# Xiuyu-Li/q-diffusion

Measured on NVIDIA H100. Metric: images_per_sec, higher is better.
Workload: dtype int8 (W4/W8 codes x A8 codes, int32 accumulate; fp32 norms/softmax)

## Files before the change

q-diffusion_b200/csrc/engine.cu:

```cuda
#include <cuda.h>
#include <cuda_runtime.h>
#include <cudaTypedefs.h>

#include <atomic>
#include <cstdarg>
#include <cstdio>
#include <cstdlib>
#include <cstring>
#include <mutex>
#include <new>
#include <utility>
#include <vector>

#include "../../include/qdiff_b200.h"
#include "attention.cuh"
#include "attention_wg.cuh"
#include "elem.cuh"
#include "gemm_i8.cuh"

namespace {

thread_local char g_err[512] = "";
std::atomic<long long> g_launches{0};
constexpr int kMaxDevices = 64;
std::atomic<int> g_num_sms[kMaxDevices];

int fail(int code, const char* fmt, ...) {
  va_list ap;
  va_start(ap, fmt);
  vsnprintf(g_err, sizeof(g_err), fmt, ap);
  va_end(ap);
  return code;
}

int check_launch(const char* what) {
  cudaError_t e = cudaGetLastError();
  if (e != cudaSuccess) return fail(QD_ERR_CUDA, "%s: %s", what, cudaGetErrorString(e));
  g_launches.fetch_add(1, std::memory_order_relaxed);
  return QD_OK;
}

template <typename... KArgs, typename... Args>
void launch_k(void (*kern)(KArgs...), dim3 grid, dim3 block, size_t smem, cudaStream_t s, Args&&... args) {
  cudaLaunchConfig_t cfg = {};
  cfg.gridDim = grid;
  cfg.blockDim = block;
  cfg.dynamicSmemBytes = smem;
  cfg.stream = s;
  cudaLaunchKernelEx(&cfg, kern, KArgs(std::forward<Args>(args))...);
}

int current_device() {
  int dev = -1;
  if (cudaGetDevice(&dev) != cudaSuccess) return -1;
  return dev;
}

int num_sms() {
  const int dev = current_device();
  if (dev < 0 || dev >= kMaxDevices) {
    fail(QD_ERR_CUDA, "no CUDA device: qdiff_b200 has no CPU fallback");
    return 0;
  }
  int n = g_num_sms[dev].load(std::memory_order_relaxed);
  if (n == 0) {
    if (cudaDeviceGetAttribute(&n, cudaDevAttrMultiProcessorCount, dev) != cudaSuccess || n <= 0) {
      fail(QD_ERR_CUDA, "no CUDA device: qdiff_b200 has no CPU fallback");
      return 0;
    }
    g_num_sms[dev].store(n, std::memory_order_relaxed);
  }
  return n;
}

template <typename K>
int ensure_smem_optin(K kern, int bytes, std::atomic<unsigned long long>& done, const char* what) {
  const int dev = current_device();
  if (dev < 0 || dev >= kMaxDevices) return fail(QD_ERR_CUDA, "%s: no current CUDA device", what);
  const unsigned long long bit = 1ull << dev;
  if (done.load(std::memory_order_acquire) & bit) return QD_OK;
  cudaError_t e = cudaFuncSetAttribute(kern, cudaFuncAttributeMaxDynamicSharedMemorySize, bytes);
  if (e != cudaSuccess) return fail(QD_ERR_CUDA, "%s: cudaFuncSetAttribute: %s", what, cudaGetErrorString(e));
  done.fetch_or(bit, std::memory_order_release);
  return QD_OK;
}

struct DeviceGuard {
  int prev = -1;
  bool ok = true;
  explicit DeviceGuard(int device) {
    if (cudaGetDevice(&prev) != cudaSuccess) prev = -1;
    if (prev != device) ok = cudaSetDevice(device) == cudaSuccess;
  }
  ~DeviceGuard() { if (prev >= 0) cudaSetDevice(prev); }
};

int grid_for(long long work_items, int threads, int per_sm = 8) {
  const int sms = num_sms();
  long long blocks = (work_items + threads - 1) / threads;
  long long cap = (long long)sms * per_sm;
  if (blocks > cap) blocks = cap;
  if (blocks < 1) blocks = 1;
  return (int)blocks;
}

PFN_cuTensorMapEncodeTiled_v12000 get_encode() {
  static PFN_cuTensorMapEncodeTiled_v12000 fn = nullptr;
  static std::once_flag once;
  std::call_once(once, [] {
    void* p = nullptr;
    cudaDriverEntryPointQueryResult q;
    if (cudaGetDriverEntryPoint("cuTensorMapEncodeTiled", &p, cudaEnableDefault, &q) == cudaSuccess &&
        q == cudaDriverEntryPointSuccess)
      fn = reinterpret_cast<PFN_cuTensorMapEncodeTiled_v12000>(p);
  });
  return fn;
}

int encode_u8_map(CUtensorMap* m, const void* base, int rank, const cuuint64_t* dims, const cuuint64_t* strides_bytes,
                  const cuuint32_t* box, int swizzle_bytes = 128) {
  auto enc = get_encode();
  if (!enc) return fail(QD_ERR_CUDA, "cuTensorMapEncodeTiled entry point not available");
  cuuint32_t estr[5] = {1, 1, 1, 1, 1};
  CUresult r = enc(m, CU_TENSOR_MAP_DATA_TYPE_UINT8, (cuuint32_t)rank, const_cast<void*>(base), dims, strides_bytes,
                   box, estr, CU_TENSOR_MAP_INTERLEAVE_NONE,
                   swizzle_bytes == 0 ? CU_TENSOR_MAP_SWIZZLE_NONE :
                   swizzle_bytes == 32 ? CU_TENSOR_MAP_SWIZZLE_32B : swizzle_bytes == 64 ? CU_TENSOR_MAP_SWIZZLE_64B : CU_TENSOR_MAP_SWIZZLE_128B,
                   CU_TENSOR_MAP_L2_PROMOTION_L2_128B, CU_TENSOR_MAP_FLOAT_OOB_FILL_NONE);
  if (r != CUDA_SUCCESS) return fail(QD_ERR_CUDA, "cuTensorMapEncodeTiled failed (%d)", (int)r);
  return QD_OK;
}

struct GemmPlan {
  CUtensorMap tmA, tmB, tmR;
  qd::GemmArgs args;
  int grid, mode;
};

int pick_bn(int N, int tiles_m, int sms, int hint, int step, long long K) {
  if (hint > 0) return hint;
  static const int wave_model = [] { const char* e = getenv("QDIFF_BN_MODEL"); return (e && !strcmp(e, "wave")) ? 1 : 0; }();
  int best = step;
  double best_cost = -1.0;
  const int n16 = (N + step - 1) / step * step;
  const double kb = (double)((K + 127) / 128);
  for (int bn = step; bn <= qd::GEMM_MAX_BN; bn += step) {
    if (bn > n16) break;
    const long long tiles = (long long)tiles_m * ((N + bn - 1) / bn);
    const long long waves = (tiles + sms - 1) / sms;
    double cost;
    if (wave_model) {
      cost = (double)waves * (bn + 24);
    } else {
      const double main_loop = kb * (2.1 * bn > 3.0 * (128 + bn) ? 2.1 * bn : 3.0 * (128 + bn));
      const double epilogue = 6.0 * bn + 300.0;
      cost = (double)waves * ((main_loop > epilogue ? main_loop : epilogue) + 200.0);
    }
    if (best_cost < 0 || cost < best_cost - 1e-9 || (cost < best_cost + 1e-9 && bn > best)) {
      best_cost = cost;
      best = bn;
    }
  }
  return best;
}

int gemm_mode(const qd::GemmArgs& a);

constexpr size_t kSplitWsBytes = 64u << 20;
int32_t* splitk_workspace() {
  static void* ws[kMaxDevices] = {};
  static std::mutex mu;
  const int dev = current_device();
  if (dev < 0 || dev >= kMaxDevices) return nullptr;
  std::lock_guard<std::mutex> lk(mu);
  if (!ws[dev] && cudaMalloc(&ws[dev], kSplitWsBytes) != cudaSuccess) { ws[dev] = nullptr; cudaGetLastError(); }
  return reinterpret_cast<int32_t*>(ws[dev]);
}

int plan_gemm(const qd_gemm_desc* d, GemmPlan* pl) {
  if (!d || !d->a || !d->w || !d->scale) return fail(QD_ERR_BAD_ARG, "gemm: null operand");
  if (d->taps != 1 && d->taps != 9) return fail(QD_ERR_UNSUPPORTED, "gemm: taps must be 1 or 9 (got %d)", d->taps);
  if (d->C <= 0 || (d->C % 32) != 0) return fail(QD_ERR_UNSUPPORTED, "gemm: C=%d must be a positive multiple of 32", d->C);
  if (d->a_bf16 && (d->corr || d->out_q || d->geglu || d->w_int4_packed || !d->out))
    return fail(QD_ERR_BAD_ARG, "gemm: a_bf16 (weight-only) layers take no corr / out_q / geglu / packed weights and write fp32");
  if (d->M <= 0 || d->N <= 0) return fail(QD_ERR_BAD_ARG, "gemm: bad M/N");
  if (!d->out && !d->out_q) return fail(QD_ERR_BAD_ARG, "gemm: no output");
  const int sms = num_sms();
  if (!sms) return QD_ERR_CUDA;

  qd::GemmArgs& a = pl->args;
  memset(&a, 0, sizeof(a));
  a.M = d->M; a.N = d->N; a.C = d->C; a.taps = d->taps;
  a.kdup = d->k_dup == 2 ? 2 : 1;
  if (d->k_dup != 0 && d->k_dup != 1 && d->k_dup != 2) return fail(QD_ERR_BAD_ARG, "gemm: k_dup must be 0, 1 or 2");
  if (a.kdup == 2 && d->w_int4_packed) return fail(QD_ERR_BAD_ARG, "gemm: k_dup 2 is for 8-bit weights (not packed INT4)");
  a.tiles_m = (d->M + qd::GEMM_BM - 1) / qd::GEMM_BM;
  a.geglu = d->geglu;
  if (d->geglu) {
    if ((d->N & 7) || !d->out_q || d->out || d->rowvec || d->residual || d->out_q_transposed || (d->ldq & 3) || d->taps != 1)
      return fail(QD_ERR_BAD_ARG, "gemm: geglu needs N %% 8 == 0, out_q only, plain GEMM");
  }
  a.BN = pick_bn(d->N, a.tiles_m, sms, d->bn_hint, d->geglu ? 32 : 16, (long long)d->C * d->taps * a.kdup);
  const int bn_default = a.BN;
  static const int splitk_enabled = [] { const char* e = getenv("QDIFF_SPLITK"); return (e && !strcmp(e, "0")) ? 0 : 1; }();
  const int num_kb_all = ((d->C + qd::GEMM_BK - 1) / qd::GEMM_BK) * d->taps * a.kdup;
  const bool splitk_candidate = splitk_enabled && !d->bn_hint && !d->a_bf16 && !d->w_int4_packed && d->out && !d->out_q && !d->geglu &&
                                !(d->N & 3) && !(d->ldo & 3) && (!d->residual || !(d->ldr & 3)) && (!d->rowvec || !(d->ld_rowvec & 3)) &&
                                num_kb_all >= 16;
  if (splitk_candidate) {
    const int bn_wide = d->N >= qd::GEMM_MAX_BN_SPLITK ? qd::GEMM_MAX_BN_SPLITK : (d->N + 15) / 16 * 16;
    if (2 * a.tiles_m * ((d->N + bn_wide - 1) / bn_wide) <= sms) a.BN = bn_wide;
  }
  if (a.BN % 16 || a.BN < 16 || a.BN > qd::GEMM_MAX_BN_SPLITK || (d->bn_hint && a.BN > qd::GEMM_MAX_BN))
    return fail(QD_ERR_BAD_ARG, "gemm: bad BN %d (16 .. %d)", a.BN, qd::GEMM_MAX_BN);
  a.tiles_n = (d->N + a.BN - 1) / a.BN;
  a.a_signed = d->a_signed; a.b_signed = 1;


  cuuint64_t dims[4], strides[3];
  cuuint32_t box[4];
  if (d->taps == 1) {
    if (d->lda % 16) return fail(QD_ERR_UNSUPPORTED, "gemm: lda=%lld must be a multiple of 16", d->lda);
    if (d->lda < d->C) return fail(QD_ERR_BAD_ARG, "gemm: lda < C");
    dims[0] = (cuuint64_t)d->C; dims[1] = (cuuint64_t)d->M; dims[2] = 1; dims[3] = 1;
    strides[0] = (cuuint64_t)d->lda; strides[1] = (cuuint64_t)d->lda * d->M; strides[2] = strides[1];
    box[0] = qd::GEMM_BK; box[1] = qd::GEMM_BM; box[2] = 1; box[3] = 1;
  } else {
    const int H = d->H, W = d->W, B = d->B;
    if (H <= 0 || W <= 0 || B <= 0 || (long long)B * H * W != d->M) return fail(QD_ERR_BAD_ARG, "gemm: conv geometry");
    const int hw = H * W;
    int bh, bn;
    int bw = W;
    if (W > 128) {
      if (W % 128) return fail(QD_ERR_UNSUPPORTED, "gemm: conv W=%d must divide or be a multiple of 128", W);
      bw = 128; bh = 1; bn = 1;
    } else if (hw >= 128) {
      if (128 % W) return fail(QD_ERR_UNSUPPORTED, "gemm: conv W=%d must divide 128", W);
      bh = 128 / W; bn = 1;
      if (H % bh) return fail(QD_ERR_UNSUPPORTED, "gemm: conv H=%d not a multiple of %d", H, bh);
    } else {
      if (128 % hw) return fail(QD_ERR_UNSUPPORTED, "gemm: conv H*W=%d must divide 128", hw);
      bh = H; bn = 128 / hw;
    }
    a.H = H; a.W = W; a.bh = bh; a.bn = bn;
    const cuuint64_t pitch = d->lda > d->C ? (cuuint64_t)d->lda : (cuuint64_t)d->C;
    if (pitch % 16) return fail(QD_ERR_UNSUPPORTED, "gemm: conv pixel pitch %llu must be a multiple of 16", (unsigned long long)pitch);
    dims[0] = (cuuint64_t)d->C; dims[1] = (cuuint64_t)W; dims[2] = (cuuint64_t)H; dims[3] = (cuuint64_t)B;
    strides[0] = pitch; strides[1] = pitch * W; strides[2] = pitch * W * H;
    box[0] = qd::GEMM_BK; box[1] = (cuuint32_t)bw; box[2] = (cuuint32_t)bh; box[3] = (cuuint32_t)bn;
  }
  int rc = encode_u8_map(&pl->tmA, d->a, 4, dims, strides, box);
  if (rc) return rc;
  if (d->w_int4_packed) {
    if (!d->w_zero) return fail(QD_ERR_BAD_ARG, "gemm: packed INT4 weights need w_zero");
    if (((uintptr_t)d->w) & 15) return fail(QD_ERR_BAD_ARG, "gemm: packed weights must be 16-byte aligned");
    a.w4 = 1;
    a.wzero = d->w_zero;
  }
  a.out = d->out; a.ldo = d->ldo;
  a.out_q = reinterpret_cast<int8_t*>(d->out_q); a.ldq = d->ldq;
  a.out_q_transposed = d->out_q_transposed;
  a.rows_per_batch = d->rows_per_batch;
  if ((d->rowvec || d->out_q_transposed) && d->rows_per_batch <= 0) return fail(QD_ERR_BAD_ARG, "gemm: rows_per_batch required");
  a.oq_d = d->out_q_head_dim; a.oq_pitch = d->out_q_head_pitch;
  a.oq_f16 = d->out_q_f16 ? 1 : 0;
  if (a.oq_f16 && (!d->out_q || d->out_q_transposed || d->geglu || (d->ldq & 3) || (((uintptr_t)d->out_q) & 7)))
    return fail(QD_ERR_BAD_ARG, "gemm: out_q_f16 needs a row-major out_q with ldq %% 4 == 0");
  if (a.oq_d > 0 && ((a.oq_d & 3) || (a.oq_pitch & 3) || a.oq_pitch < a.oq_d || d->out_q_transposed || !d->out_q))
    return fail(QD_ERR_BAD_ARG, "gemm: bad out_q head layout");
  if (d->out_q && d->oq.qmax - d->oq.qmin > 255)
    return fail(QD_ERR_UNSUPPORTED, "gemm: the epilogue emits 8-bit codes; quantizer range [%d, %d] is wider", d->oq.qmin, d->oq.qmax);
  a.q_delta = d->oq.delta; a.q_zp = d->oq.zero_point; a.q_lo = d->oq.qmin; a.q_hi = d->oq.qmax;
  a.scale = d->scale; a.bias = d->bias; a.corr = d->corr;
  a.scale_q = d->scale_q; a.bias_q = d->bias_q;
  a.gn_stats = reinterpret_cast<float2*>(d->gn_stats); a.ld_stats = d->ld_stats;
  a.bf16 = d->a_bf16;
  if (d->gn_stats && (!d->out || (d->ld_stats & 1) || (reinterpret_cast<uintptr_t>(d->gn_stats) & 15)))
    return fail(QD_ERR_BAD_ARG, "gemm: gn_stats needs an fp32 output, an even ld_stats and 16-byte alignment");
  if ((d->scale_q == nullptr) != (d->bias_q == nullptr)) return fail(QD_ERR_BAD_ARG, "gemm: scale_q and bias_q come together");
  a.rowvec = d->rowvec; a.ld_rowvec = d->ld_rowvec;
  a.residual = d->residual; a.ldr = d->ldr;
  const int tiles = a.tiles_m * a.tiles_n;
  pl->grid = tiles < sms ? tiles : sms;
  pl->mode = gemm_mode(a);
  {
    const int num_kb = num_kb_all;
    const bool eligible = splitk_candidate && pl->mode >= 0 && 2 * tiles <= sms &&
                          (!a.gn_stats || (!(a.M & 31) && !(a.ld_stats & 1)));
    if (eligible) {
      int splits = sms / tiles;
      if (splits > 16) splits = 16;
      if (splits > num_kb / 4) splits = num_kb / 4;
      if (splits >= 2 && (size_t)splits * a.M * a.N * 4 <= kSplitWsBytes) {
        const int per = (num_kb + splits - 1) / splits;
        splits = (num_kb + per - 1) / per;
        int32_t* ws = splitk_workspace();
        if (ws && splits >= 2) {
          a.splits = splits; a.kb_per_split = per; a.ws = ws;
          pl->grid = tiles * splits < sms ? tiles * splits : sms;
        }
      }
    }
  }
  if (a.splits <= 1 && a.BN > qd::GEMM_MAX_BN) {
    a.BN = bn_default;
    a.tiles_n = (d->N + a.BN - 1) / a.BN;
    const int t = a.tiles_m * a.tiles_n;
    pl->grid = t < sms ? t : sms;
  }
  {
    const int w_rows = d->w_rows > 0 ? d->w_rows : d->N;
    if (d->w_int4_packed) {
      cuuint64_t bd[2] = {(cuuint64_t)d->taps * d->C / 2, (cuuint64_t)w_rows};
      cuuint64_t bs[1] = {(cuuint64_t)d->taps * d->C / 2};
      cuuint32_t bb[2] = {qd::GEMM_BK / 2, (cuuint32_t)a.BN};
      rc = encode_u8_map(&pl->tmB, d->w, 2, bd, bs, bb, 0);
    } else {
      cuuint64_t bd[2] = {(cuuint64_t)d->taps * d->C * a.kdup, (cuuint64_t)w_rows};
      cuuint64_t bs[1] = {(cuuint64_t)d->taps * d->C * a.kdup};
      cuuint32_t bb[2] = {qd::GEMM_BK, (cuuint32_t)a.BN};
      rc = encode_u8_map(&pl->tmB, d->w, 2, bd, bs, bb);
    }
    if (rc) return rc;
  }
  if (a.bf16 && pl->mode < 0)
    return fail(QD_ERR_UNSUPPORTED, "gemm: weight-only (a_bf16) layer needs a specialised epilogue (N %% 4 == 0, aligned leading dimensions)");
  memset(&pl->tmR, 0, sizeof(pl->tmR));
  if (qd::gemm_res_tma(pl->mode)) {
    cuuint64_t rd[2] = {(cuuint64_t)d->N * 4, (cuuint64_t)d->M};
    cuuint64_t rs[1] = {(cuuint64_t)d->ldr * 4};
    cuuint32_t rb[2] = {128, 32};
    rc = encode_u8_map(&pl->tmR, d->residual, 2, rd, rs, rb);
    if (rc) return rc;
  }
  return QD_OK;
}

template <int MODE, bool W4>
int launch_gemm_mode_w(const GemmPlan& pl, cudaStream_t s) {
  static std::atomic<unsigned long long> optin{0};
  if (int rc = ensure_smem_optin(qd::gemm_i8_kernel<MODE, W4>, 227 * 1024, optin, "gemm")) return rc;
  qd::GemmArgs a = pl.args;
  const int stage_bytes = qd::gemm_stage_footprint(a.BN, W4 ? 1 : 0);
  constexpr int res_bytes = qd::gemm_res_bytes(MODE);
  constexpr bool splitk = MODE >= 0 && (MODE & qd::EPI_SPLITK) != 0;
  if (a.BN > qd::gemm_max_bn(MODE)) return fail(QD_ERR_BAD_ARG, "gemm: BN=%d exceeds %d (mode %d)", a.BN, qd::gemm_max_bn(MODE), MODE);
  int stages = (232448 - 512 - qd::gemm_acc_tile_bytes(a.BN, splitk) - res_bytes - 1024 - 1024) / stage_bytes;
  if (stages > qd::GEMM_MAX_STAGES) stages = qd::GEMM_MAX_STAGES;
  if (stages < 2) stages = 2;
  a.stages = stages;
  const int smem = qd::gemm_smem_layout(a.BN, stages, W4 ? 1 : 0, res_bytes, splitk).total;
  if (smem > 232448) return fail(QD_ERR_UNSUPPORTED, "gemm: BN=%d needs %d bytes of shared memory for 2 stages (mode %d, w4 %d)", a.BN, smem, MODE, (int)W4);
  launch_k(qd::gemm_i8_kernel<MODE, W4>, pl.grid, qd::gemm_threads(MODE, W4), smem, s, pl.tmA, pl.tmB, pl.tmR, a);
  return check_launch("gemm_i8_kernel");
}

template <int MODE>
int launch_gemm_mode(const GemmPlan& pl, cudaStream_t s) {
  return pl.args.w4 ? launch_gemm_mode_w<MODE, true>(pl, s) : launch_gemm_mode_w<MODE, false>(pl, s);
}

int gemm_mode(const qd::GemmArgs& a) {
  const bool f = a.out != nullptr, q = a.out_q != nullptr;
  if (a.geglu) return qd::EPI_GEGLU | qd::EPI_OUT_Q | (a.corr ? qd::EPI_CORR : 0);
  if (q && !f && !a.geglu && !a.scale_q) return -1;
  if (a.out_q_transposed && q && !f && !a.rowvec && !a.residual && a.taps == 1 && a.oq_d == 0 &&
      a.rows_per_batch % 32 == 0 && (a.ldq & 15) == 0 && (reinterpret_cast<uintptr_t>(a.out_q) & 15) == 0)
    return qd::EPI_TRANS | qd::EPI_OUT_Q | (a.corr ? qd::EPI_CORR : 0);
  if (f == q || a.out_q_transposed || (a.N & 3)) return -1;
  if (a.rowvec && a.residual) return -1;
  if (q && a.rowvec) return -1;
  if (f && (a.ldo & 3)) return -1;
  if (q && (a.ldq & 3)) return -1;
  if (a.residual && (a.ldr & 3)) return -1;
  if (a.rowvec && (a.ld_rowvec & 3)) return -1;
  if (a.bf16) {
    return qd::EPI_BF16 | qd::EPI_OUT_F32 | ((a.taps == 9) ? qd::EPI_CONV : 0) | (a.rowvec ? qd::EPI_ROWVEC : 0) |
           (a.residual ? qd::EPI_RESIDUAL : 0);
  }
  static const int ring_kb = [] { const char* e = getenv("QDIFF_RES_RING_KB"); return e ? atoi(e) : 5; }();
  const int num_kb = ((a.C + qd::GEMM_BK - 1) / qd::GEMM_BK) * a.taps * a.kdup;
  const bool ring = a.residual && a.taps == 1 && num_kb <= ring_kb && !(reinterpret_cast<uintptr_t>(a.residual) & 15) &&
                    !a.w4;
  return (a.corr ? qd::EPI_CORR : 0) | ((a.taps == 9) ? qd::EPI_CONV : 0) | (a.rowvec ? qd::EPI_ROWVEC : 0) |
         (a.residual ? qd::EPI_RESIDUAL : 0) | (f ? qd::EPI_OUT_F32 : qd::EPI_OUT_Q) | (ring ? qd::EPI_RESTMA : 0);
}

int launch_gemm(const GemmPlan& pl, cudaStream_t s) {
  using namespace qd;
  if (pl.args.splits > 1) {
    if (int rc = launch_gemm_mode_w<EPI_SPLITK, false>(pl, s)) return rc;
    launch_k(qd::splitk_finish_kernel, dim3((pl.args.N + 31) / 32, (pl.args.M + 31) / 32), 256, 0, s, pl.args);
    return check_launch("splitk_finish_kernel");
  }
  switch (pl.mode) {
    case EPI_OUT_F32: return launch_gemm_mode<EPI_OUT_F32>(pl, s);
    case EPI_OUT_F32 | EPI_CORR: return launch_gemm_mode<EPI_OUT_F32 | EPI_CORR>(pl, s);
    case EPI_OUT_F32 | EPI_ROWVEC: return launch_gemm_mode<EPI_OUT_F32 | EPI_ROWVEC>(pl, s);
    case EPI_OUT_F32 | EPI_ROWVEC | EPI_CORR: return launch_gemm_mode<EPI_OUT_F32 | EPI_ROWVEC | EPI_CORR>(pl, s);
    case EPI_OUT_F32 | EPI_RESIDUAL: return launch_gemm_mode<EPI_OUT_F32 | EPI_RESIDUAL>(pl, s);
    case EPI_OUT_F32 | EPI_RESIDUAL | EPI_CORR: return launch_gemm_mode<EPI_OUT_F32 | EPI_RESIDUAL | EPI_CORR>(pl, s);
    case EPI_OUT_F32 | EPI_CORR | EPI_CONV: return launch_gemm_mode<EPI_OUT_F32 | EPI_CORR | EPI_CONV>(pl, s);
    case EPI_OUT_F32 | EPI_ROWVEC | EPI_CORR | EPI_CONV: return launch_gemm_mode<EPI_OUT_F32 | EPI_ROWVEC | EPI_CORR | EPI_CONV>(pl, s);
    case EPI_OUT_F32 | EPI_RESIDUAL | EPI_CORR | EPI_CONV: return launch_gemm_mode<EPI_OUT_F32 | EPI_RESIDUAL | EPI_CORR | EPI_CONV>(pl, s);
    case EPI_OUT_Q | EPI_CORR | EPI_CONV: return launch_gemm_mode<EPI_OUT_Q | EPI_CORR | EPI_CONV>(pl, s);
    case EPI_OUT_F32 | EPI_CONV: return launch_gemm_mode<EPI_OUT_F32 | EPI_CONV>(pl, s);
    case EPI_OUT_F32 | EPI_ROWVEC | EPI_CONV: return launch_gemm_mode<EPI_OUT_F32 | EPI_ROWVEC | EPI_CONV>(pl, s);
    case EPI_OUT_F32 | EPI_RESIDUAL | EPI_CONV: return launch_gemm_mode<EPI_OUT_F32 | EPI_RESIDUAL | EPI_CONV>(pl, s);
    case EPI_OUT_Q | EPI_CONV: return launch_gemm_mode<EPI_OUT_Q | EPI_CONV>(pl, s);
    case EPI_OUT_Q: return launch_gemm_mode<EPI_OUT_Q>(pl, s);
    case EPI_OUT_Q | EPI_CORR: return launch_gemm_mode<EPI_OUT_Q | EPI_CORR>(pl, s);
    case EPI_OUT_Q | EPI_RESIDUAL: return launch_gemm_mode<EPI_OUT_Q | EPI_RESIDUAL>(pl, s);
    case EPI_OUT_Q | EPI_RESIDUAL | EPI_CORR: return launch_gemm_mode<EPI_OUT_Q | EPI_RESIDUAL | EPI_CORR>(pl, s);
    case EPI_OUT_F32 | EPI_RESIDUAL | EPI_RESTMA: return launch_gemm_mode<EPI_OUT_F32 | EPI_RESIDUAL | EPI_RESTMA>(pl, s);
    case EPI_OUT_F32 | EPI_RESIDUAL | EPI_CORR | EPI_RESTMA: return launch_gemm_mode<EPI_OUT_F32 | EPI_RESIDUAL | EPI_CORR | EPI_RESTMA>(pl, s);
    case EPI_OUT_Q | EPI_RESIDUAL | EPI_RESTMA: return launch_gemm_mode<EPI_OUT_Q | EPI_RESIDUAL | EPI_RESTMA>(pl, s);
    case EPI_OUT_Q | EPI_RESIDUAL | EPI_CORR | EPI_RESTMA: return launch_gemm_mode<EPI_OUT_Q | EPI_RESIDUAL | EPI_CORR | EPI_RESTMA>(pl, s);
    case EPI_BF16 | EPI_OUT_F32: return launch_gemm_mode_w<EPI_BF16 | EPI_OUT_F32, false>(pl, s);
    case EPI_BF16 | EPI_OUT_F32 | EPI_ROWVEC: return launch_gemm_mode_w<EPI_BF16 | EPI_OUT_F32 | EPI_ROWVEC, false>(pl, s);
    case EPI_BF16 | EPI_OUT_F32 | EPI_RESIDUAL: return launch_gemm_mode_w<EPI_BF16 | EPI_OUT_F32 | EPI_RESIDUAL, false>(pl, s);
    case EPI_BF16 | EPI_OUT_F32 | EPI_CONV: return launch_gemm_mode_w<EPI_BF16 | EPI_OUT_F32 | EPI_CONV, false>(pl, s);
    case EPI_BF16 | EPI_OUT_F32 | EPI_ROWVEC | EPI_CONV: return launch_gemm_mode_w<EPI_BF16 | EPI_OUT_F32 | EPI_ROWVEC | EPI_CONV, false>(pl, s);
    case EPI_BF16 | EPI_OUT_F32 | EPI_RESIDUAL | EPI_CONV: return launch_gemm_mode_w<EPI_BF16 | EPI_OUT_F32 | EPI_RESIDUAL | EPI_CONV, false>(pl, s);
    case EPI_TRANS | EPI_OUT_Q: return launch_gemm_mode<EPI_TRANS | EPI_OUT_Q>(pl, s);
    case EPI_TRANS | EPI_OUT_Q | EPI_CORR: return launch_gemm_mode<EPI_TRANS | EPI_OUT_Q | EPI_CORR>(pl, s);
    case EPI_GEGLU | EPI_OUT_Q: return launch_gemm_mode<EPI_GEGLU | EPI_OUT_Q>(pl, s);
    case EPI_GEGLU | EPI_OUT_Q | EPI_CORR: return launch_gemm_mode<EPI_GEGLU | EPI_OUT_Q | EPI_CORR>(pl, s);
    default: return launch_gemm_mode<-1>(pl, s);
  }
}

int launch_quantize(const qd_quantize_desc& d, cudaStream_t s) {
  if (!d.src || !d.dst || d.M <= 0 || d.C <= 0) return fail(QD_ERR_BAD_ARG, "quantize: bad args");
  if (d.q0.qmax - d.q0.qmin > 255 || d.q1.qmax - d.q1.qmin > 255)
    return fail(QD_ERR_UNSUPPORTED, "quantize: the engine emits 8-bit codes; quantizer range [%d, %d] is wider", d.q0.qmin, d.q0.qmax);
  const bool vec = (d.C % 4 == 0) && (d.ld_src % 4 == 0) && (d.ld_dst % 4 == 0) && (d.split % 4 == 0);
  if (d.upsample2x && !vec) return fail(QD_ERR_UNSUPPORTED, "quantize: upsample needs C %% 4 == 0");
  if (vec) {
    const long long rows = d.upsample2x ? (long long)d.B * 4 * d.H * d.W : d.M;
    launch_k(qd::quantize_kernel, grid_for(rows * (d.C / 4), 256), 256, 0, s, d);
  } else {
    launch_k(qd::quantize_scalar_kernel, grid_for((long long)d.M * d.C, 256), 256, 0, s, d);
  }
  return check_launch("quantize_kernel");
}

int gn_slab_rows(int B, int HW) {
  int sms = num_sms();
  if (sms <= 0) sms = 132;
  long long r = ((long long)B * HW) / (4LL * sms);
  int slab = 64;
  while (slab > 8 && slab > r) slab >>= 1;
  return slab;
}

long long gn_workspace_floats(int B, int HW, int C, int groups) {
  const int slab = gn_slab_rows(B, HW);
  const long long nslab = (HW + slab - 1) / slab;
  (void)C;
  return (long long)B * nslab * groups * 2 * 2 + (long long)B * groups * 2 + 16;
}

int use_stats_env() {
  static const int v = [] { const char* e = getenv("QDIFF_GN_STATS"); return (e && !strcmp(e, "0")) ? 0 : 1; }();
  return v;
}

int launch_groupnorm(const qd_groupnorm_desc& d, cudaStream_t s) {
  if (!d.x || !d.gamma || !d.beta) return fail(QD_ERR_BAD_ARG, "groupnorm: null arg");
  if (d.groups <= 0 || d.groups > qd::GN_MAX_GROUPS || d.C % 4 || d.C % d.groups || d.ld_x % 4)
    return fail(QD_ERR_UNSUPPORTED, "groupnorm: C=%d groups=%d", d.C, d.groups);
  if (d.n_out < 0 || d.n_out > 3) return fail(QD_ERR_BAD_ARG, "groupnorm: n_out");
  if (d.raw_q && ((d.raw_split & 3) || (d.ld_raw & 3) || d.raw_split < 0))
    return fail(QD_ERR_BAD_ARG, "groupnorm: raw output needs raw_split %% 4 == 0 and ld_raw %% 4 == 0");
  const int cpg = d.C / d.groups;
  {
    bool ok = (cpg % 2 == 0) && cpg <= 128 && (d.ld_x % 2 == 0) && (!d.out_f || d.ld_f % 2 == 0);
    for (int o = 0; o < d.n_out; ++o) ok = ok && (d.ld_q[o] % 2 == 0);
    const long long units = (long long)d.HW * (cpg / 2);
    static const int force = [] {
      const char* e = getenv("QDIFF_GN");
      return !e ? 0 : (!strcmp(e, "fused") ? 1 : (!strcmp(e, "split") ? 2 : 0));
    }();
    const long long limit = force == 1 ? 512LL * qd::GN_NU : (force == 2 ? 0 : 256LL * qd::GN_NU);
    const long long elems = (long long)d.B * d.HW * d.C;
    const bool small_problem = elems <= ((d.stats_in && use_stats_env()) ? (512LL << 10) : (2LL << 20)) && (long long)d.B * d.groups <= 2048;
    if (ok && units <= limit && (force == 1 || small_problem)) {
      int threads = units <= 256LL * qd::GN_NU ? 256 : 512;
      if (units < 256) threads = (int)((units + 31) / 32 * 32);
      if (threads < cpg / 2) threads = (cpg / 2 + 31) / 32 * 32;
      launch_k(qd::gn_fused_small_kernel, dim3(d.groups, d.B), threads, 0, s, d);
      return check_launch("gn_fused_small_kernel");
    }
  }
  if (!d.ws) return fail(QD_ERR_BAD_ARG, "groupnorm: workspace required");
  if ((uintptr_t)d.ws & 7) return fail(QD_ERR_BAD_ARG, "groupnorm: workspace must be 8-byte aligned");
  const int slab = gn_slab_rows(d.B, d.HW);
  const int nslab = (d.HW + slab - 1) / slab;
  double* part = reinterpret_cast<double*>(d.ws);
  float* stats = d.ws + (long long)d.B * nslab * d.groups * 4;
  int threads = d.C / 4;
  threads = (threads + 31) / 32 * 32;
  if (threads > 256) threads = 256;
  if (threads < 2 * d.groups) threads = (2 * d.groups + 31) / 32 * 32;
  int rc;
  const int use_stats = use_stats_env();
  if (d.stats_in && use_stats) {
    if (d.HW % 32) return fail(QD_ERR_BAD_ARG, "groupnorm: stats_in needs HW %% 32 == 0");
    launch_k(qd::gn_finalize_from_stats_kernel, dim3(d.groups, d.B), 128, 0, s, reinterpret_cast<const float2*>(d.stats_in),
                                                                         d.ld_stats_in, d.HW, d.C, d.groups, d.eps, stats);
    rc = check_launch("gn_finalize_from_stats_kernel");
    if (rc) return rc;
  } else {
    launch_k(qd::gn_partial_kernel, dim3(nslab, d.B), threads, 2 * d.C * sizeof(float), s, d.x, d.ld_x, d.HW, d.C, d.groups, slab,
                                                                                     nslab, part);
    rc = check_launch("gn_partial_kernel");
    if (rc) return rc;
    launch_k(qd::gn_finalize_kernel, d.B, 256, 0, s, part, d.HW, d.C, d.groups, nslab, d.eps, stats);
    rc = check_launch("gn_finalize_kernel");
    if (rc) return rc;
  }
  const int cq = d.C / 4;
  const int slabs_x = (cq + 255) / 256;
  const int TX = (cq + slabs_x - 1) / slabs_x;
  int TY = 256 / TX;
  if (TY < 1) TY = 1;
  const int athreads = TX * TY;
  int rows = qd::GN_BATCH * TY;
  while ((long long)((d.HW + rows - 1) / rows) * slabs_x * d.B > 8LL * num_sms() && rows < 8 * qd::GN_BATCH * TY) rows += qd::GN_BATCH * TY;
  const dim3 grid(slabs_x, (d.HW + rows - 1) / rows, d.B);
  const bool raw = d.raw_q != nullptr;
#define QD_GN_APPLY(NOUT, RAW) launch_k(qd::gn_apply_kernel<NOUT, RAW>, grid, athreads, 0, s, d, stats, rows, TX)
  switch (d.n_out * 2 + (raw ? 1 : 0)) {
    case 0: QD_GN_APPLY(0, false); break;
    case 1: QD_GN_APPLY(0, true); break;
    case 2: QD_GN_APPLY(1, false); break;
    case 3: QD_GN_APPLY(1, true); break;
    case 4: QD_GN_APPLY(2, false); break;
    case 5: QD_GN_APPLY(2, true); break;
    case 6: QD_GN_APPLY(3, false); break;
    default: QD_GN_APPLY(3, true); break;
  }
#undef QD_GN_APPLY
  return check_launch("gn_apply_kernel");
}

template <int NVEC>
int launch_layernorm_t(const qd_layernorm_desc& d, cudaStream_t s) {
  const int wpb = 8;
  launch_k(qd::layernorm_quant_kernel<NVEC>, grid_for((long long)d.M * 32, wpb * 32, 8), wpb * 32, 0, s, d);
  return check_launch("layernorm_quant_kernel");
}

int launch_layernorm(const qd_layernorm_desc& d, cudaStream_t s) {
  if (!d.x || !d.gamma || !d.beta) return fail(QD_ERR_BAD_ARG, "layernorm: null arg");
  if (d.C % 4 || d.ld_x % 4) return fail(QD_ERR_UNSUPPORTED, "layernorm: C=%d", d.C);
  if (d.n_out < 0 || d.n_out > 3 || (d.n_out == 0 && !d.out_f)) return fail(QD_ERR_BAD_ARG, "layernorm: n_out");
  if (d.out_f && (d.ld_f & 3)) return fail(QD_ERR_UNSUPPORTED, "layernorm: ld_f");
  const int nvec = (d.C / 4 + 31) / 32;
  switch (nvec) {
    case 1: return launch_layernorm_t<1>(d, s);
    case 2: return launch_layernorm_t<2>(d, s);
    case 3: return launch_layernorm_t<3>(d, s);
    case 4: return launch_layernorm_t<4>(d, s);
    case 5: return launch_layernorm_t<5>(d, s);
    case 6: case 7: case 8: return launch_layernorm_t<8>(d, s);
    case 9: case 10: return launch_layernorm_t<10>(d, s);
    case 11: case 12: case 13: case 14: case 15: case 16: return launch_layernorm_t<16>(d, s);
    default: return fail(QD_ERR_UNSUPPORTED, "layernorm: C=%d exceeds 2048", d.C);
  }
}

int launch_split3(const qd_split_desc& d, cudaStream_t s) {
  if (!d.src || !d.dst || d.M <= 0 || d.C <= 0) return fail(QD_ERR_BAD_ARG, "split: bad args");
  if ((d.Cp & 3) || d.Cp < d.C || d.ld_dst < 3LL * d.Cp || (d.ld_dst & 3))
    return fail(QD_ERR_UNSUPPORTED, "split: Cp=%d must be a multiple of 4, >= C, with ld_dst >= 3*Cp", d.Cp);
  if ((d.C & 3) || (d.ld_src & 3)) {
    if (d.upsample2x) return fail(QD_ERR_UNSUPPORTED, "split: upsample needs C %% 4 == 0");
    launch_k(qd::split_bf16x3_scalar_kernel, grid_for((long long)d.M * d.C, 256), 256, 0, s, d);
    return check_launch("split_bf16x3_scalar_kernel");
  }
  const long long rows = d.upsample2x ? (long long)d.B * 4 * d.H * d.W : d.M;
  launch_k(qd::split_bf16x3_kernel, grid_for(rows * (d.C / 4), 256), 256, 0, s, d);
  return check_launch("split_bf16x3_kernel");
}

int launch_attention_fp(const qd_attention_fp_desc& d, cudaStream_t s) {
  if (!d.q || !d.k || !d.v || !d.out || d.B <= 0 || d.heads <= 0 || d.d <= 0 || d.Tq <= 0 || d.Tk <= 0)
    return fail(QD_ERR_BAD_ARG, "attention_fp32: bad args");
  const size_t smem_rows = (size_t)qd::AFP_R * (d.d + qd::afp_tk_pitch(d.Tk)) * sizeof(float);
  const bool aligned = !(d.d & 3) && !(d.ld_q & 3) && !(d.ld_k & 3) && !(d.q_off & 3) && !(d.k_off & 3) && !(d.head_stride_q & 3) &&
                       !(d.head_stride_k & 3) && !((uintptr_t)d.q & 15) && !((uintptr_t)d.k & 15);
  if (d.Tq >= 256 && smem_rows <= 200 * 1024 && aligned) {
    static std::atomic<unsigned long long> optin{0};
    if (int rc = ensure_smem_optin(qd::attention_fp32_rows_kernel, 200 * 1024, optin, "attention_fp32_rows")) return rc;
    launch_k(qd::attention_fp32_rows_kernel, dim3((d.Tq + qd::AFP_R - 1) / qd::AFP_R, d.B * d.heads), 256, smem_rows, s, d);
    return check_launch("attention_fp32_rows_kernel");
  }
  const size_t smem = (size_t)(d.d + d.Tk) * sizeof(float);
  if (smem > 48 * 1024) return fail(QD_ERR_UNSUPPORTED, "attention_fp32: d + Tk = %d exceeds 12288 floats of shared memory", d.d + d.Tk);
  launch_k(qd::attention_fp32_kernel, dim3(d.Tq, d.B * d.heads), 128, smem, s, d);
  return check_launch("attention_fp32_kernel");
}

int launch_im2col(const qd_im2col_desc& d, cudaStream_t s) {
  if (!d.src || !d.dst) return fail(QD_ERR_BAD_ARG, "im2col: null arg");
  if (d.ld_dst < 9 * d.C) return fail(QD_ERR_BAD_ARG, "im2col: ld_dst too small");
  if ((d.C % 16) == 0 && d.ld_dst == 9 * d.C && (d.ld_dst % 16) == 0) {
    launch_k(qd::im2col_vec_kernel, grid_for((long long)d.B * d.Ho * d.Wo * 9 * (d.C / 16), 256), 256, 0, s, d);
    return check_launch("im2col_vec_kernel");
  }
  const long long total = (long long)d.B * d.Ho * d.Wo * d.ld_dst;
  launch_k(qd::im2col_kernel, grid_for(total, 256), 256, 0, s, d);
  return check_launch("im2col_kernel");
}

template <int DQ, int DV, bool QS, bool VS, bool S16, bool F16>
int launch_attention_inst(const qd_attention_desc& d, cudaStream_t s) {
  constexpr int MINB = (DV <= 48) ? 2 : 1;
  auto kern = qd::qattention_kernel<DQ, DV, QS, VS, S16, MINB, F16>;
  static std::atomic<unsigned long long> optin{0};
  if (int rc = ensure_smem_optin(kern, 200 * 1024, optin, "attention")) return rc;
  const bool zrk = !F16 && d.zq != 0;
  const qd::AttSmemLayout lay = qd::att_smem_layout(DQ, DV, d.Tk, zrk);
  if (lay.total > 200 * 1024) return fail(QD_ERR_UNSUPPORTED, "attention: Tk=%d needs %d B of shared memory", d.Tk, lay.total);
  if (zrk) {
    if (!d.ws) return fail(QD_ERR_BAD_ARG, "attention: workspace required when zq != 0");
    const int tk_pad = qd::att_ws_stride(d.Tk);
    launch_k(qd::att_krowsum_kernel<QS>, grid_for((long long)d.B * d.heads * tk_pad, 256), 256, 0, s, d, tk_pad, 0, 0);
    int rc = check_launch("att_krowsum_kernel");
    if (rc) return rc;
  }
  dim3 grid((d.Tq + qd::ATT_BM - 1) / qd::ATT_BM, d.B * d.heads);
  launch_k(kern, grid, qd::ATT_WARPS * 32, lay.total, s, d);
  return check_launch("qattention_kernel");
}

template <int DQ, int DV, bool F16 = false>
int launch_attention_t(const qd_attention_desc& d, cudaStream_t s) {
  const bool qs = d.q_signed != 0, vs = d.v_signed != 0, s16 = d.sm_bits > 8;
  if (qs && vs && s16) return launch_attention_inst<DQ, DV, true, true, true, F16>(d, s);
  if (qs && vs && !s16) return launch_attention_inst<DQ, DV, true, true, false, F16>(d, s);
  if (!qs && !vs && s16) return launch_attention_inst<DQ, DV, false, false, true, F16>(d, s);
  if (!qs && !vs && !s16) return launch_attention_inst<DQ, DV, false, false, false, F16>(d, s);
  return fail(QD_ERR_UNSUPPORTED, "attention: mixed signedness q=%d v=%d", d.q_signed, d.v_signed);
}

template <int DQ, int DV, bool QS, bool VS, bool S16>
int launch_attention_smallk_inst(const qd_attention_desc& d, cudaStream_t s) {
  constexpr int NKV = 3;
  auto kern = qd::qattention_smallk_kernel<DQ, DV, QS, VS, S16, NKV>;
  const int spw = d.Tq >= 2048 ? 4 : (d.Tq >= 512 ? 2 : 1);
  const int slabs = (d.Tq + 15) / 16;
  dim3 grid((slabs + spw * qd::ATS_WARPS - 1) / (spw * qd::ATS_WARPS), d.B * d.heads);
  launch_k(kern, grid, qd::ATS_WARPS * 32, qd::ats_smem_bytes<DQ, DV, NKV>(), s, d, spw);
  return check_launch("qattention_smallk_kernel");
}

template <int DQ, int DV>
int launch_attention_smallk(const qd_attention_desc& d, cudaStream_t s) {
  const bool qs = d.q_signed != 0, vs = d.v_signed != 0, s16 = d.sm_bits > 8;
  if (qs && vs && s16) return launch_attention_smallk_inst<DQ, DV, true, true, true>(d, s);
  if (qs && vs && !s16) return launch_attention_smallk_inst<DQ, DV, true, true, false>(d, s);
  if (!qs && !vs && s16) return launch_attention_smallk_inst<DQ, DV, false, false, true>(d, s);
  if (!qs && !vs && !s16) return launch_attention_smallk_inst<DQ, DV, false, false, false>(d, s);
  return fail(QD_ERR_UNSUPPORTED, "attention: mixed signedness q=%d v=%d", d.q_signed, d.v_signed);
}

bool attention_wg_eligible(const qd_attention_desc& d) {
  static const int forced_mma = [] { const char* e = getenv("QDIFF_ATTENTION"); return (e && !strcmp(e, "mma")) ? 1 : 0; }();
  if (forced_mma) return false;
  const int P = d.head_stride_q, rb = d.qk_f16 ? 2 * d.d : d.d;
  if (d.d != 16 && d.d != 24 && d.d != 32 && d.d != 40 && d.d != 48 && d.d != 64 && d.d != 80 && d.d != 96) return false;
  if (d.qk_f16 && d.d > 64) return false;
  if (d.qk_f16 && d.d == 48) return false;
  if ((P != 32 && P != 64 && P != 128) || P < rb || d.head_stride_k != P) return false;
  if (d.q_off != 0 || d.k_off != 0 || (d.ld_k & 15) || (((uintptr_t)d.k) & 15) || (((uintptr_t)d.vt) & 15)) return false;
  if (d.v_off != 0 || d.head_stride_v != d.d || d.v_batch_stride != (long long)d.heads * d.d * d.ld_vt) return false;
  if (d.zq != 0 && !d.qk_f16 && !d.ws) return false;
  return true;
}

template <int DQ, int DV, bool QS, bool VS, bool S16, bool F16>
int launch_attention_wg_inst(const qd_attention_desc& d, cudaStream_t s) {
  constexpr int MINB = DV <= 40 ? 2 : 1;
  auto kern = qd::qattention_wg_kernel<DQ, DV, QS, VS, S16, F16, MINB>;
  const int P = d.head_stride_q;
  const qd::AtwSmem lay = qd::atw_smem(P, qd::atw_nv(DV));
  static std::atomic<unsigned long long> optin{0};
  if (int rc = ensure_smem_optin(kern, 227 * 1024, optin, "attention_wg")) return rc;
  CUtensorMap tmK, tmV;
  {
    cuuint64_t dims[2] = {(cuuint64_t)d.ld_k, (cuuint64_t)d.B * d.Tk};
    cuuint64_t strides[1] = {(cuuint64_t)d.ld_k};
    cuuint32_t box[2] = {(cuuint32_t)P, (cuuint32_t)qd::ATT_BN};
    if (int rc = encode_u8_map(&tmK, d.k, 2, dims, strides, box, P)) return rc;
  }
  {
    cuuint64_t dims[2] = {(cuuint64_t)d.ld_vt, (cuuint64_t)d.B * d.heads * d.d};
    cuuint64_t strides[1] = {(cuuint64_t)d.ld_vt};
    cuuint32_t box[2] = {(cuuint32_t)qd::ATT_BN, (cuuint32_t)d.d};
    if (int rc = encode_u8_map(&tmV, d.vt, 2, dims, strides, box, 64)) return rc;
  }
  if (!F16 && d.zq != 0) {
    const int tk_pad = qd::att_ws_stride(d.Tk);
    launch_k(qd::att_krowsum_kernel<QS>, grid_for((long long)d.B * d.heads * tk_pad, 256), 256, 0, s, d, tk_pad, 0, 0);
    if (int rc = check_launch("att_krowsum_kernel")) return rc;
  }
  dim3 grid((d.Tq + qd::ATT_BM - 1) / qd::ATT_BM, d.B * d.heads);
  launch_k(kern, grid, qd::ATW_THREADS, lay.total, s, tmK, tmV, d, P);
  return check_launch("qattention_wg_kernel");
}

template <int DQ, int DV, bool F16>
int launch_attention_wg_t(const qd_attention_desc& d, cudaStream_t s) {
  const bool qs = d.q_signed != 0, vs = d.v_signed != 0, s16 = d.sm_bits > 8;
  if (qs && vs && s16) return launch_attention_wg_inst<DQ, DV, true, true, true, F16>(d, s);
  if (qs && vs && !s16) return launch_attention_wg_inst<DQ, DV, true, true, false, F16>(d, s);
  if (!qs && !vs && s16) return launch_attention_wg_inst<DQ, DV, false, false, true, F16>(d, s);
  if (!qs && !vs && !s16) return launch_attention_wg_inst<DQ, DV, false, false, false, F16>(d, s);
  return fail(QD_ERR_UNSUPPORTED, "attention: mixed signedness q=%d v=%d", d.q_signed, d.v_signed);
}

int launch_attention_wg(const qd_attention_desc& d, cudaStream_t s) {
  if (d.qk_f16) {
    switch (d.d) {
      case 16: return launch_attention_wg_t<32, 16, true>(d, s);
      case 24: return launch_attention_wg_t<64, 24, true>(d, s);
      case 32: return launch_attention_wg_t<64, 32, true>(d, s);
      case 40: return launch_attention_wg_t<96, 40, true>(d, s);
      case 48: return launch_attention_wg_t<96, 48, true>(d, s);
      default: return launch_attention_wg_t<128, 64, true>(d, s);
    }
  }
  switch (d.d) {
    case 16: return launch_attention_wg_t<32, 16, false>(d, s);
    case 24: return launch_attention_wg_t<32, 24, false>(d, s);
    case 32: return launch_attention_wg_t<32, 32, false>(d, s);
    case 40: return launch_attention_wg_t<64, 40, false>(d, s);
    case 48: return launch_attention_wg_t<64, 48, false>(d, s);
    case 64: return launch_attention_wg_t<64, 64, false>(d, s);
    case 80: return launch_attention_wg_t<96, 80, false>(d, s);
    default: return launch_attention_wg_t<96, 96, false>(d, s);
  }
}

int launch_attention(const qd_attention_desc& d, cudaStream_t s) {
  if (!d.q || !d.k || !d.vt || (!d.out && !d.out_q)) return fail(QD_ERR_BAD_ARG, "attention: null arg");
  if (d.out_q && (d.ld_out_q & 1)) return fail(QD_ERR_UNSUPPORTED, "attention: ld_out_q");
  if (d.q_signed != d.k_signed) return fail(QD_ERR_UNSUPPORTED, "attention: q/k signedness differ");
  if (d.zw != 0) return fail(QD_ERR_UNSUPPORTED, "attention: softmax zero point must be 0 (got %d)", d.zw);
  if (d.sm_bits != 8 && d.sm_bits != 16) return fail(QD_ERR_UNSUPPORTED, "attention: sm_bits %d", d.sm_bits);
  if (d.ld_vt % 16 || d.ld_vt < d.Tk) return fail(QD_ERR_BAD_ARG, "attention: ld_vt");
  if ((d.q_off | d.head_stride_q | (int)d.ld_q) & 3) return fail(QD_ERR_UNSUPPORTED, "attention: q needs 4-byte alignment");
  if ((d.k_off | d.head_stride_k | (int)d.ld_k | d.d) & 7) return fail(QD_ERR_UNSUPPORTED, "attention: k rows need 8-byte alignment");
  if (d.out && (d.ld_out % 2)) return fail(QD_ERR_UNSUPPORTED, "attention: ld_out");
  if (d.qk_f16) {
    if (attention_wg_eligible(d)) return launch_attention_wg(d, s);
    switch (d.d) {
      case 16: return launch_attention_t<32, 16, true>(d, s);
      case 24: return launch_attention_t<64, 24, true>(d, s);
      case 32: return launch_attention_t<64, 32, true>(d, s);
      case 40: return launch_attention_t<96, 40, true>(d, s);
      case 48: return launch_attention_t<96, 48, true>(d, s);
      case 64: return launch_attention_t<128, 64, true>(d, s);
      default: return fail(QD_ERR_UNSUPPORTED, "attention: qk_f16 needs d in {16, 24, 32, 40, 48, 64} (got %d)", d.d);
    }
  }
  if (d.Tk <= 96 && (d.d == 40 || d.d == 80)) {
    static const bool off = [] { const char* e = getenv("QDIFF_ATTENTION"); return e && !strcmp(e, "nosmallk"); }();
    if (!off) return d.d == 40 ? launch_attention_smallk<64, 40>(d, s) : launch_attention_smallk<96, 80>(d, s);
  }
  if (attention_wg_eligible(d)) return launch_attention_wg(d, s);
  switch (d.d) {
    case 16: return launch_attention_t<32, 16>(d, s);
    case 24: return launch_attention_t<32, 24>(d, s);
    case 32: return launch_attention_t<32, 32>(d, s);
    case 40: return launch_attention_t<64, 40>(d, s);
    case 48: return launch_attention_t<64, 48>(d, s);
    case 64: return launch_attention_t<64, 64>(d, s);
    case 80: return launch_attention_t<96, 80>(d, s);
    case 96: return launch_attention_t<96, 96>(d, s);
    case 160: return launch_attention_t<160, 160>(d, s);
    case 256: return launch_attention_t<256, 256>(d, s);
    default: return fail(QD_ERR_UNSUPPORTED, "attention: head dim %d not instantiated", d.d);
  }
}

int launch_misc(int kind, const qd_misc_desc& m, cudaStream_t s) {
  switch (kind) {
    case QD_OP_TIMESTEP_EMB:
      if (!m.aux) return fail(QD_ERR_BAD_ARG, "timestep_embedding: missing frequency table");
      launch_k(qd::timestep_embedding_kernel, grid_for((long long)m.a * (m.b / 2), 128), 128, 0, s, m.src, m.aux, m.a, m.b, m.c, m.dst);
      return check_launch("timestep_embedding_kernel");
    case QD_OP_COPY2D:
      if (m.b % 4 || m.ld_src % 4 || m.ld_dst % 4) return fail(QD_ERR_UNSUPPORTED, "copy2d: alignment");
      launch_k(qd::copy2d_kernel, grid_for((long long)m.a * (m.b / 4), 256), 256, 0, s, m.src, m.ld_src, m.dst, m.ld_dst, m.a, m.b);
      return check_launch("copy2d_kernel");
    case QD_OP_NCHW_TO_NHWC:
      launch_k(qd::nchw_to_nhwc_kernel, grid_for((long long)m.a * m.b * m.c, 256), 256, 0, s, m.src, m.dst, m.a, m.b, m.c);
      return check_launch("nchw_to_nhwc_kernel");
    case QD_OP_NHWC_TO_NCHW:
      launch_k(qd::nhwc_to_nchw_kernel, grid_for((long long)m.a * m.b * m.c, 256), 256, 0, s, m.src, m.dst, m.a, m.b, m.c);
      return check_launch("nhwc_to_nchw_kernel");
    case QD_OP_AVGPOOL2X:
      if (m.d % 4) return fail(QD_ERR_UNSUPPORTED, "avgpool: C %% 4");
      launch_k(qd::avgpool2x_kernel, grid_for((long long)m.a * (m.b / 2) * (m.c / 2) * (m.d / 4), 256), 256, 0, s, m.src, m.dst, m.a, m.b, m.c, m.d);
      return check_launch("avgpool2x_kernel");
    case QD_OP_UPSAMPLE2X:
      if (m.d % 4) return fail(QD_ERR_UNSUPPORTED, "upsample: C %% 4");
      launch_k(qd::upsample2x_f32_kernel, grid_for((long long)m.a * m.b * m.c * m.d, 256), 256, 0, s, m.src, m.dst, m.a, m.b, m.c, m.d);
      return check_launch("upsample2x_f32_kernel");
    case QD_OP_SOFTMAX_ROWS:
      if (m.a <= 0 || m.b <= 0 || m.ld_src < m.b || m.src != m.dst) return fail(QD_ERR_BAD_ARG, "softmax_rows: in place, rows=%d cols=%d", m.a, m.b);
      launch_k(qd::softmax_rows_kernel, dim3(m.a), 256, 0, s, m.dst, m.ld_src, m.b);
      return check_launch("softmax_rows_kernel");
    case QD_OP_VQ_LOOKUP:
      if (!m.aux || m.a <= 0 || m.b <= 0 || m.b > qd::VQ_MAX_C || m.c <= 0 || m.ld_src < m.b || m.ld_dst < m.b)
        return fail(QD_ERR_BAD_ARG, "vq_lookup: bad args (rows=%d, C=%d <= %d, n_e=%d)", m.a, m.b, qd::VQ_MAX_C, m.c);
      launch_k(qd::vq_lookup_kernel, grid_for((long long)m.a * 32, 256), 256, 0, s, m.src, m.ld_src, m.aux, m.dst, m.ld_dst, m.a, m.b, m.c);
      return check_launch("vq_lookup_kernel");
    default:
      return fail(QD_ERR_BAD_ARG, "misc: unknown kind %d", kind);
  }
}

struct Op {
  int kind;
  GemmPlan gemm;
  union {
    qd_quantize_desc quant;
    qd_groupnorm_desc gn;
    qd_layernorm_desc ln;
    qd_im2col_desc im2col;
    qd_attention_desc att;
    qd_misc_desc misc;
    qd_split_desc split;
    qd_attention_fp_desc attfp;
  };
  Op() : kind(0) { memset(&gemm, 0, sizeof(gemm)); memset(&gn, 0, sizeof(gn)); }
};

int run_op(const Op& op, cudaStream_t s) {
  switch (op.kind) {
    case QD_OP_GEMM: return launch_gemm(op.gemm, s);
    case QD_OP_QUANTIZE: return launch_quantize(op.quant, s);
    case QD_OP_GROUPNORM: return launch_groupnorm(op.gn, s);
    case QD_OP_LAYERNORM: return launch_layernorm(op.ln, s);
    case QD_OP_IM2COL: return launch_im2col(op.im2col, s);
    case QD_OP_ATTENTION: return launch_attention(op.att, s);
    case QD_OP_SPLIT3: return launch_split3(op.split, s);
    case QD_OP_ATTENTION_FP: return launch_attention_fp(op.attfp, s);
    default: return launch_misc(op.kind, op.misc, s);
  }
}

}

struct qd_engine {
  int device;
  bool finalized;
  std::vector<Op> ops;
};

extern "C" {

const char* qd_last_error(void) { return g_err; }
int qd_num_sms(void) { return num_sms(); }
long long qd_launch_count(void) { return g_launches.load(); }

int qd_qgemm_i8(const qd_gemm_desc* d, qd_stream_t stream) {
  GemmPlan pl;
  int rc = plan_gemm(d, &pl);
  if (rc) return rc;
  return launch_gemm(pl, (cudaStream_t)stream);
}
int qd_quantize(const qd_quantize_desc* d, qd_stream_t s) {
  if (!d) return fail(QD_ERR_BAD_ARG, "null desc");
  return launch_quantize(*d, (cudaStream_t)s);
}
long long qd_groupnorm_workspace_floats(int B, int HW, int C, int groups) {
  if (B <= 0 || HW <= 0 || C <= 0 || groups <= 0) return 0;
  return gn_workspace_floats(B, HW, C, groups);
}

int qd_groupnorm_quant(const qd_groupnorm_desc* d, qd_stream_t s) {
  if (!d) return fail(QD_ERR_BAD_ARG, "null desc");
  return launch_groupnorm(*d, (cudaStream_t)s);
}
int qd_layernorm_quant(const qd_layernorm_desc* d, qd_stream_t s) {
  if (!d) return fail(QD_ERR_BAD_ARG, "null desc");
  return launch_layernorm(*d, (cudaStream_t)s);
}
int qd_im2col_i8(const qd_im2col_desc* d, qd_stream_t s) {
  if (!d) return fail(QD_ERR_BAD_ARG, "null desc");
  return launch_im2col(*d, (cudaStream_t)s);
}
int qd_qattention(const qd_attention_desc* d, qd_stream_t s) {
  if (!d) return fail(QD_ERR_BAD_ARG, "null desc");
  return launch_attention(*d, (cudaStream_t)s);
}
int qd_lincomb3(float* out, float a, const float* x, float b, const float* y, float c, const float* z, long long n,
                qd_stream_t s) {
  if (!out || !x || n <= 0) return fail(QD_ERR_BAD_ARG, "lincomb3: bad args");
  launch_k(qd::lincomb3_kernel, grid_for(n, 256), 256, 0, (cudaStream_t)s, out, a, x, b, y, c, z, n);
  return check_launch("lincomb3_kernel");
}
int qd_split_bf16x3(const qd_split_desc* d, qd_stream_t s) {
  if (!d) return fail(QD_ERR_BAD_ARG, "null desc");
  return launch_split3(*d, (cudaStream_t)s);
}
int qd_attention_fp32(const qd_attention_fp_desc* d, qd_stream_t s) {
  if (!d) return fail(QD_ERR_BAD_ARG, "null desc");
  return launch_attention_fp(*d, (cudaStream_t)s);
}
int qd_timestep_embedding(const float* t, const float* freqs, int32_t B, int32_t dim, int32_t mode, float* out,
                          qd_stream_t s) {
  qd_misc_desc m{t, out, 0, 0, B, dim, mode, 0, freqs};
  return launch_misc(QD_OP_TIMESTEP_EMB, m, (cudaStream_t)s);
}
int qd_copy2d(const float* src, long long ld_src, float* dst, long long ld_dst, int32_t M, int32_t C, qd_stream_t s) {
  qd_misc_desc m{src, dst, ld_src, ld_dst, M, C, 0, 0, nullptr};
  return launch_misc(QD_OP_COPY2D, m, (cudaStream_t)s);
}
int qd_nchw_to_nhwc(const float* src, float* dst, int32_t B, int32_t C, int32_t HW, qd_stream_t s) {
  qd_misc_desc m{src, dst, 0, 0, B, C, HW, 0, nullptr};
  return launch_misc(QD_OP_NCHW_TO_NHWC, m, (cudaStream_t)s);
}
int qd_nhwc_to_nchw(const float* src, float* dst, int32_t B, int32_t C, int32_t HW, qd_stream_t s) {
  qd_misc_desc m{src, dst, 0, 0, B, C, HW, 0, nullptr};
  return launch_misc(QD_OP_NHWC_TO_NCHW, m, (cudaStream_t)s);
}
int qd_avgpool2x(const float* src, float* dst, int32_t B, int32_t H, int32_t W, int32_t C, qd_stream_t s) {
  qd_misc_desc m{src, dst, 0, 0, B, H, W, C, nullptr};
  return launch_misc(QD_OP_AVGPOOL2X, m, (cudaStream_t)s);
}
int qd_upsample2x_f32(const float* src, float* dst, int32_t B, int32_t H, int32_t W, int32_t C, qd_stream_t s) {
  qd_misc_desc m{src, dst, 0, 0, B, H, W, C, nullptr};
  return launch_misc(QD_OP_UPSAMPLE2X, m, (cudaStream_t)s);
}
int qd_softmax_rows(float* x, long long ld, int32_t rows, int32_t cols, qd_stream_t s) {
  qd_misc_desc m{x, x, ld, ld, rows, cols, 0, 0, nullptr};
  return launch_misc(QD_OP_SOFTMAX_ROWS, m, (cudaStream_t)s);
}
int qd_vq_lookup(const float* z, long long ld_z, const float* codebook, float* out, long long ld_out, int32_t rows, int32_t C,
                 int32_t n_e, qd_stream_t s) {
  qd_misc_desc m{z, out, ld_z, ld_out, rows, C, n_e, 0, codebook};
  return launch_misc(QD_OP_VQ_LOOKUP, m, (cudaStream_t)s);
}
int qd_sampler_step(const qd_sampler_desc* d, qd_stream_t s) {
  if (!d || !d->x || !d->eps || !d->x_prev || d->n <= 0) return fail(QD_ERR_BAD_ARG, "sampler: bad args");
  launch_k(qd::sampler_step_kernel, grid_for(d->n, 256), 256, 0, (cudaStream_t)s, *d);
  return check_launch("sampler_step_kernel");
}
int qd_ancestral_step(const qd_ancestral_desc* d, qd_stream_t s) {
  if (!d || !d->x || !d->eps || !d->x_prev || d->n <= 0) return fail(QD_ERR_BAD_ARG, "ancestral: bad args");
  launch_k(qd::ancestral_step_kernel, grid_for(d->n, 256), 256, 0, (cudaStream_t)s, *d);
  return check_launch("ancestral_step_kernel");
}

int qd_engine_create(int device, qd_engine** out) {
  if (!out) return fail(QD_ERR_BAD_ARG, "null out");
  {
    DeviceGuard g(device);
    if (!g.ok) return fail(QD_ERR_CUDA, "cudaSetDevice(%d) failed: no CPU fallback", device);
    if (!num_sms()) return QD_ERR_CUDA;
  }
  qd_engine* e = new (std::nothrow) qd_engine();
  if (!e) return fail(QD_ERR_BAD_ARG, "out of host memory");
  e->device = device;
  e->finalized = false;
  *out = e;
  return QD_OK;
}

int qd_engine_add_op(qd_engine* e, int kind, const void* desc) {
  if (!e || !desc) return fail(QD_ERR_BAD_ARG, "null arg");
  DeviceGuard g(e->device);
  if (!g.ok) return fail(QD_ERR_CUDA, "cudaSetDevice(%d) failed", e->device);
  Op op;
  op.kind = kind;
  switch (kind) {
    case QD_OP_GEMM: {
      int rc = plan_gemm(reinterpret_cast<const qd_gemm_desc*>(desc), &op.gemm);
      if (rc) return rc;
      break;
    }
    case QD_OP_QUANTIZE: op.quant = *reinterpret_cast<const qd_quantize_desc*>(desc); break;
    case QD_OP_GROUPNORM: op.gn = *reinterpret_cast<const qd_groupnorm_desc*>(desc); break;
    case QD_OP_LAYERNORM: op.ln = *reinterpret_cast<const qd_layernorm_desc*>(desc); break;
    case QD_OP_IM2COL: op.im2col = *reinterpret_cast<const qd_im2col_desc*>(desc); break;
    case QD_OP_ATTENTION: op.att = *reinterpret_cast<const qd_attention_desc*>(desc); break;
    case QD_OP_SPLIT3: op.split = *reinterpret_cast<const qd_split_desc*>(desc); break;
    case QD_OP_ATTENTION_FP: op.attfp = *reinterpret_cast<const qd_attention_fp_desc*>(desc); break;
    case QD_OP_TIMESTEP_EMB: case QD_OP_COPY2D: case QD_OP_NCHW_TO_NHWC: case QD_OP_NHWC_TO_NCHW:
    case QD_OP_AVGPOOL2X: case QD_OP_UPSAMPLE2X: case QD_OP_VQ_LOOKUP: case QD_OP_SOFTMAX_ROWS:
      op.misc = *reinterpret_cast<const qd_misc_desc*>(desc);
      break;
    default: return fail(QD_ERR_BAD_ARG, "unknown op kind %d", kind);
  }
  e->ops.push_back(op);
  e->finalized = false;
  return QD_OK;
}

int qd_engine_num_ops(const qd_engine* e) { return e ? (int)e->ops.size() : 0; }

int qd_engine_finalize(qd_engine* e) {
  if (!e) return fail(QD_ERR_BAD_ARG, "null engine");
  e->finalized = true;
  return QD_OK;
}

int qd_engine_run_range(qd_engine* e, int first, int last, qd_stream_t stream) {
  if (!e) return fail(QD_ERR_BAD_ARG, "null engine");
  if (!e->finalized) return fail(QD_ERR_NOT_FINALIZED, "engine not finalized");
  if (first < 0 || last > (int)e->ops.size() || first > last) return fail(QD_ERR_BAD_ARG, "bad op range");
  if (current_device() != e->device)
    return fail(QD_ERR_BAD_ARG, "engine was built for device %d but the current device is %d", e->device, current_device());
  for (int i = first; i < last; ++i) {
    int rc = run_op(e->ops[i], (cudaStream_t)stream);
    if (rc) return rc;
  }
  return QD_OK;
}
int qd_engine_run(qd_engine* e, qd_stream_t stream) {
  if (!e) return fail(QD_ERR_BAD_ARG, "null engine");
  return qd_engine_run_range(e, 0, (int)e->ops.size(), stream);
}
void qd_engine_destroy(qd_engine* e) { delete e; }

}
```

q-diffusion_b200/csrc/gemm_i8.cuh:

```cuda
#pragma once
#include "ptx.cuh"
#include "quant_math.cuh"
#include <cuda_fp16.h>
#include <type_traits>

namespace qd {

constexpr int GEMM_BM = 128;
constexpr int GEMM_BK = 128;
constexpr int GEMM_MAX_BN = 128;
constexpr int GEMM_MAX_BN_SPLITK = 256;
__host__ __device__ constexpr int gemm_epi_warps(int MODE) { return (void)MODE, 8; }
constexpr int GEMM_RES_NBUF = 3;
__host__ __device__ constexpr bool gemm_res_tma(int MODE) { return MODE >= 0 && (MODE & 4) != 0 && (MODE & 256) != 0; }
__host__ __device__ constexpr int gemm_res_bytes(int MODE) {
  return gemm_res_tma(MODE) ? gemm_epi_warps(MODE) * GEMM_RES_NBUF * 4096 : 0;
}
__host__ __device__ constexpr int gemm_threads(int MODE, bool W4 = false) { return (4 + gemm_epi_warps(MODE) + (W4 ? 2 : 0)) * 32; }
constexpr int GEMM_A_STAGE_BYTES = GEMM_BM * GEMM_BK;
constexpr int GEMM_MAX_STAGES = 8;
constexpr int GEMM_EPI_TILE_BYTES = 32 * 128;
__host__ __device__ inline int gemm_acc_tile_bytes(int BN, bool splitk = false) {
  return splitk ? 0 : 4 * ((BN + 31) / 32) * GEMM_EPI_TILE_BYTES;
}

constexpr int EPI_CORR = 1;
constexpr int EPI_ROWVEC = 2;
constexpr int EPI_RESIDUAL = 4;
constexpr int EPI_OUT_F32 = 8;
constexpr int EPI_OUT_Q = 16;
constexpr int EPI_GEGLU = 32;
constexpr int EPI_TRANS = 64;
constexpr int EPI_CONV = 128;
constexpr int EPI_RESTMA = 256;
constexpr int EPI_BF16 = 512;
constexpr int EPI_SPLITK = 1024;
__host__ __device__ constexpr int gemm_max_bn(int MODE) { return (MODE >= 0 && (MODE & EPI_SPLITK) != 0) ? GEMM_MAX_BN_SPLITK : GEMM_MAX_BN; }

struct GemmArgs {
  int M, N;
  int C;
  int taps;
  int kdup;
  int BN;
  int tiles_m, tiles_n;
  int stages;
  int H, W, bh, bn;
  int a_signed, b_signed;
  float* out;
  long long ldo;
  int8_t* out_q;
  long long ldq;
  int out_q_transposed;
  int rows_per_batch;
  float q_delta;
  int q_zp, q_lo, q_hi;
  const float* scale;
  const float* bias;
  const int32_t* corr;
  const float* rowvec;
  long long ld_rowvec;
  const float* residual;
  long long ldr;
  int geglu;
  int oq_d, oq_pitch;
  int oq_f16;
  int w4;
  const int8_t* wzero;
  const float* scale_q;
  const float* bias_q;
  float2* gn_stats;
  long long ld_stats;
  int bf16;
  int splits, kb_per_split;
  int32_t* ws;
};
__host__ __device__ constexpr bool gemm_qpre(int MODE) { return MODE >= 0 && (MODE & 16) != 0 && (MODE & 32) == 0; }

struct GemmSmemLayout {
  int stage_bytes;
  int pack_off;
  int bar_offset;
  int stage_off;
  int res_off;
  int total;
};

__host__ __device__ inline int gemm_stage_footprint(int BN, int w4) {
  return GEMM_A_STAGE_BYTES + BN * GEMM_BK + (w4 ? BN * (GEMM_BK / 2) : 0);
}

__host__ __device__ inline GemmSmemLayout gemm_smem_layout(int BN, int stages, int w4 = 0, int res_bytes = 0, bool splitk = false) {
  GemmSmemLayout l;
  l.stage_bytes = GEMM_A_STAGE_BYTES + BN * GEMM_BK;
  l.pack_off = l.stage_bytes * stages;
  l.bar_offset = l.pack_off + (w4 ? stages * BN * (GEMM_BK / 2) : 0);
  l.stage_off = l.bar_offset + 512;
  l.res_off = (l.stage_off + gemm_acc_tile_bytes(BN, splitk) + 1023) / 1024 * 1024;
  l.total = l.res_off + res_bytes + 1024;
  return l;
}

__device__ __forceinline__ void gemm_row_meta(const GemmArgs& p, int m, int& cls, int& img) {
  cls = 0;
  img = 0;
  if (p.rows_per_batch > 0) img = m / p.rows_per_batch;
  if (p.taps == 9) {
    const int hw = p.H * p.W;
    const int r = m % hw;
    const int h = r / p.W, w = r - h * p.W;
    const int rc = (h == 0) ? 0 : (h == p.H - 1 ? 2 : 1);
    const int cc = (w == 0) ? 0 : (w == p.W - 1 ? 2 : 1);
    cls = rc * 3 + cc;
  }
}


template <int NC>
__device__ __forceinline__ void gemm_acc_row(const uint8_t* chunk, int row, uint32_t (&v)[NC]) {
#pragma unroll
  for (int j = 0; j < NC / 4; ++j) {
    const uint4 u = *reinterpret_cast<const uint4*>(chunk + row * 128 + ((j ^ (row & 7)) << 4));
    v[4 * j] = u.x; v[4 * j + 1] = u.y; v[4 * j + 2] = u.z; v[4 * j + 3] = u.w;
  }
}

template <int NC>
__device__ __forceinline__ void gemm_epilogue_rowwise(const GemmArgs& p, const QuantK& qk, const uint32_t (&acc)[NC],
                                                      int m, int n0, int cls, int img) {
  float y[NC];
  if (((p.N & 3) == 0) && n0 + NC <= p.N && !p.rowvec) {
#pragma unroll
    for (int j = 0; j < NC; j += 4) {
      const int n = n0 + j;
      const float4 s4 = __ldg(reinterpret_cast<const float4*>(p.scale + n));
      float4 b4 = make_float4(0.f, 0.f, 0.f, 0.f);
      if (p.bias) b4 = __ldg(reinterpret_cast<const float4*>(p.bias + n));
      int4 c4 = make_int4(0, 0, 0, 0);
      if (p.corr) c4 = __ldg(reinterpret_cast<const int4*>(p.corr + (long long)cls * p.N + n));
      y[j] = (float)((int)acc[j] - c4.x) * s4.x + b4.x;
      y[j + 1] = (float)((int)acc[j + 1] - c4.y) * s4.y + b4.y;
      y[j + 2] = (float)((int)acc[j + 2] - c4.z) * s4.z + b4.z;
      y[j + 3] = (float)((int)acc[j + 3] - c4.w) * s4.w + b4.w;
    }
    if (p.residual) {
#pragma unroll
      for (int j = 0; j < NC; ++j) y[j] += p.residual[(long long)m * p.ldr + n0 + j];
    }
  } else {
#pragma unroll
    for (int j = 0; j < NC; ++j) {
      int n = n0 + j;
      int a = (int)acc[j];
      if (n < p.N) {
        if (p.corr) a -= __ldg(p.corr + (long long)cls * p.N + n);
        float v = (float)a * __ldg(p.scale + n);
        if (p.bias) v += __ldg(p.bias + n);
        if (p.rowvec) v += __ldg(p.rowvec + (long long)img * p.ld_rowvec + n);
        if (p.residual) v += p.residual[(long long)m * p.ldr + n];
        y[j] = v;
      } else {
        y[j] = 0.f;
      }
    }
  }
  if (p.out) {
    float* o = p.out + (long long)m * p.ldo + n0;
#pragma unroll
    for (int j = 0; j < NC; ++j)
      if (n0 + j < p.N) o[j] = y[j];
  }
  if (p.out_q) {
    const int t_in = m - img * p.rows_per_batch;
    const int t_pos = (t_in & ~15) | (((t_in >> 1) & 3) << 2) | (((t_in >> 3) & 1) << 1) | (t_in & 1);
    int8_t* o = p.out_q + ((long long)img * p.N + n0) * p.ldq + t_pos;
#pragma unroll
    for (int j = 0; j < NC; ++j)
      if (n0 + j < p.N) o[(long long)j * p.ldq] = (int8_t)quant_code(y[j], qk);
  }
}

template <int MODE>
__device__ __forceinline__ void gemm_finalise4(const GemmArgs& p, const QuantK& qk, const bool conv, const uint4 a4,
                                               const float (&sc)[4], const float (&bi)[4], const int4 corr4,
                                               const float4 rpre, float* of, int8_t* oq, const float* res, int n,
                                               int cls, int img, float (&gsum)[4], float (&gsq)[4]) {
  constexpr bool G = MODE < 0;
  const bool has_corr = G ? (p.corr != nullptr) : bool(MODE & EPI_CORR);
  const bool has_rowvec = G ? (p.rowvec != nullptr) : bool(MODE & EPI_ROWVEC);
  const bool has_res = G ? (p.residual != nullptr) : bool(MODE & EPI_RESIDUAL);
  const bool out_f = G ? (p.out != nullptr) : bool(MODE & EPI_OUT_F32);
  const bool out_q = G ? (p.out_q != nullptr) : bool(MODE & EPI_OUT_Q);
  const bool full = G ? (n + 3 < p.N) : true;
  int a[4] = {(int)a4.x, (int)a4.y, (int)a4.z, (int)a4.w};
  if (has_corr) {
    if (G && conv) {
      if (full) {
        const int4 c = __ldg(reinterpret_cast<const int4*>(p.corr + (long long)cls * p.N + n));
        a[0] -= c.x; a[1] -= c.y; a[2] -= c.z; a[3] -= c.w;
      } else {
#pragma unroll
        for (int j = 0; j < 4; ++j)
          if (n + j < p.N) a[j] -= __ldg(p.corr + (long long)cls * p.N + n + j);
      }
    } else {
      a[0] -= corr4.x; a[1] -= corr4.y; a[2] -= corr4.z; a[3] -= corr4.w;
    }
  }
  float y[4];
  if constexpr (MODE >= 0 && (MODE & EPI_BF16) != 0) {
    y[0] = __uint_as_float(a4.x) * sc[0] + bi[0]; y[1] = __uint_as_float(a4.y) * sc[1] + bi[1];
    y[2] = __uint_as_float(a4.z) * sc[2] + bi[2]; y[3] = __uint_as_float(a4.w) * sc[3] + bi[3];
  } else {
#pragma unroll
    for (int j = 0; j < 4; ++j) y[j] = (float)a[j] * sc[j] + bi[j];
  }
  if (has_rowvec) {
    const float* rv = p.rowvec + (long long)img * p.ld_rowvec + n;
    if (full && (G ? ((p.ld_rowvec & 3) == 0) : true)) {
      const float4 r = __ldg(reinterpret_cast<const float4*>(rv));
      y[0] += r.x; y[1] += r.y; y[2] += r.z; y[3] += r.w;
    } else {
#pragma unroll
      for (int j = 0; j < 4; ++j)
        if (n + j < p.N) y[j] += rv[j];
    }
  }
  constexpr bool QPRE = gemm_qpre(MODE);
  if (has_res && !G) {
    if constexpr (QPRE) {
      y[0] = fmaf(rpre.x, qk.rdelta, y[0]); y[1] = fmaf(rpre.y, qk.rdelta, y[1]);
      y[2] = fmaf(rpre.z, qk.rdelta, y[2]); y[3] = fmaf(rpre.w, qk.rdelta, y[3]);
    } else {
      y[0] += rpre.x; y[1] += rpre.y; y[2] += rpre.z; y[3] += rpre.w;
    }
  } else if (has_res) {
    if (full && ((p.ldr & 3) == 0)) {
      const float4 rv = *reinterpret_cast<const float4*>(res);
      y[0] += rv.x; y[1] += rv.y; y[2] += rv.z; y[3] += rv.w;
    } else {
#pragma unroll
      for (int j = 0; j < 4; ++j)
        if (n + j < p.N) y[j] += res[j];
    }
  }
  if (out_f) {
#pragma unroll
    for (int j = 0; j < 4; ++j) { gsum[j] += y[j]; gsq[j] = fmaf(y[j], y[j], gsq[j]); }
    if (full && (G ? ((p.ldo & 3) == 0) : true)) {
      *reinterpret_cast<float4*>(of) = make_float4(y[0], y[1], y[2], y[3]);
    } else {
#pragma unroll
      for (int j = 0; j < 4; ++j)
        if (n + j < p.N) of[j] = y[j];
    }
  }
  if constexpr (QPRE) {
    if (p.oq_f16) {
      const float kz = 12582912.0f + (float)p.q_zp;
      const __half2 h01 = __floats2half2_rn(__uint_as_float(quant_bits_pre(y[0], qk)) - kz, __uint_as_float(quant_bits_pre(y[1], qk)) - kz);
      const __half2 h23 = __floats2half2_rn(__uint_as_float(quant_bits_pre(y[2], qk)) - kz, __uint_as_float(quant_bits_pre(y[3], qk)) - kz);
      *reinterpret_cast<uint2*>(oq) = make_uint2(*reinterpret_cast<const uint32_t*>(&h01), *reinterpret_cast<const uint32_t*>(&h23));
    } else {
      *reinterpret_cast<uint32_t*>(oq) = pack4_low_bytes(quant_bits_pre(y[0], qk), quant_bits_pre(y[1], qk),
                                                         quant_bits_pre(y[2], qk), quant_bits_pre(y[3], qk));
    }
  } else if (out_q && p.oq_f16) {
    float cz[4];
#pragma unroll
    for (int j = 0; j < 4; ++j) cz[j] = quant_centered(y[j], qk);
    if (full) {
      const __half2 h01 = __floats2half2_rn(cz[0], cz[1]), h23 = __floats2half2_rn(cz[2], cz[3]);
      *reinterpret_cast<uint2*>(oq) = make_uint2(*reinterpret_cast<const uint32_t*>(&h01), *reinterpret_cast<const uint32_t*>(&h23));
    } else {
#pragma unroll
      for (int j = 0; j < 4; ++j)
        if (n + j < p.N) reinterpret_cast<__half*>(oq)[j] = __float2half_rn(cz[j]);
    }
  } else if (out_q) {
    const uint32_t q0 = quant_code(y[0], qk), q1 = quant_code(y[1], qk);
    const uint32_t q2 = quant_code(y[2], qk), q3 = quant_code(y[3], qk);
    if (full && (G ? ((p.ldq & 3) == 0) : true)) {
      *reinterpret_cast<uint32_t*>(oq) = q0 | (q1 << 8) | (q2 << 16) | (q3 << 24);
    } else {
      const uint32_t qq[4] = {q0, q1, q2, q3};
#pragma unroll
      for (int j = 0; j < 4; ++j)
        if (n + j < p.N) oq[j] = (int8_t)qq[j];
    }
  }
}

template <bool BF16, bool SIGNED, int NF, int TAIL, int NS, typename T>
__device__ __forceinline__ void gemm_wgmma_kblock(T (&acc)[NS][32], uint64_t da, uint64_t db, uint32_t scale_first) {
#pragma unroll
  for (int j = 0; j < 4; ++j) {
    const uint32_t sd = j ? 1u : scale_first;
    const uint64_t a = da + (uint64_t)(2 * j);
#pragma unroll
    for (int s = 0; s <= NF; ++s) {
      const uint64_t b = db + (uint64_t)((s * 64 * GEMM_BK) >> 4) + (uint64_t)(2 * j);
      if (s < NF) {
        if constexpr (BF16) wgmma_bf16_n64(acc[s < NS ? s : 0], a, b, sd);
        else if constexpr (SIGNED) wgmma_s8s8_n64(acc[s < NS ? s : 0], a, b, sd);
        else wgmma_u8s8_n64(acc[s < NS ? s : 0], a, b, sd);
      } else if constexpr (TAIL != 0) {
        constexpr int t = NF < NS ? NF : 0;
        if constexpr (BF16) {
          if constexpr (TAIL == 48) wgmma_bf16_n48(acc[t], a, b, sd);
          else if constexpr (TAIL == 32) wgmma_bf16_n32(acc[t], a, b, sd);
          else wgmma_bf16_n16(acc[t], a, b, sd);
        } else if constexpr (SIGNED) {
          if constexpr (TAIL == 48) wgmma_s8s8_n48(acc[t], a, b, sd);
          else if constexpr (TAIL == 32) wgmma_s8s8_n32(acc[t], a, b, sd);
          else wgmma_s8s8_n16(acc[t], a, b, sd);
        } else {
          if constexpr (TAIL == 48) wgmma_u8s8_n48(acc[t], a, b, sd);
          else if constexpr (TAIL == 32) wgmma_u8s8_n32(acc[t], a, b, sd);
          else wgmma_u8s8_n16(acc[t], a, b, sd);
        }
      }
    }
  }
}

template <int NF_, int TAIL_, bool SIGNED_>
struct GemmNCfg {
  static constexpr int NF = NF_, TAIL = TAIL_;
  static constexpr bool SIGNED = SIGNED_;
};
template <int NS, bool S, typename F>
__device__ __forceinline__ void gemm_dispatch_bn(int BN, F&& f) {
  switch (BN >> 4) {
    case 1: f(GemmNCfg<0, 16, S>{}); break;
    case 2: f(GemmNCfg<0, 32, S>{}); break;
    case 3: f(GemmNCfg<0, 48, S>{}); break;
    case 4: f(GemmNCfg<1, 0, S>{}); break;
    case 5: f(GemmNCfg<1, 16, S>{}); break;
    case 6: f(GemmNCfg<1, 32, S>{}); break;
    case 7: f(GemmNCfg<1, 48, S>{}); break;
    default:
      if constexpr (NS == 2) {
        f(GemmNCfg<2, 0, S>{});
      } else {
        switch (BN >> 4) {
          case 8: f(GemmNCfg<2, 0, S>{}); break;
          case 9: f(GemmNCfg<2, 16, S>{}); break;
          case 10: f(GemmNCfg<2, 32, S>{}); break;
          case 11: f(GemmNCfg<2, 48, S>{}); break;
          case 12: f(GemmNCfg<3, 0, S>{}); break;
          case 13: f(GemmNCfg<3, 16, S>{}); break;
          case 14: f(GemmNCfg<3, 32, S>{}); break;
          case 15: f(GemmNCfg<3, 48, S>{}); break;
          default: f(GemmNCfg<4, 0, S>{}); break;
        }
      }
  }
}

template <int MODE, bool W4 = false>
__global__ void __launch_bounds__(gemm_threads(MODE, W4), 1)
gemm_i8_kernel(const __grid_constant__ CUtensorMap tmA, const __grid_constant__ CUtensorMap tmB,
               const __grid_constant__ CUtensorMap tmR, const GemmArgs p) {
  extern __shared__ uint8_t smem_raw[];
  const uint32_t raw_addr = smem_u32(smem_raw);
  const uint32_t pad = ((raw_addr + 1023u) & ~1023u) - raw_addr;
  uint8_t* smem = smem_raw + pad;

  constexpr int EPI_WARPS = gemm_epi_warps(MODE);
  constexpr int CSTEP = 32 * (EPI_WARPS / 4);
  constexpr bool RES_TMA = gemm_res_tma(MODE);
  constexpr bool SPLITK = MODE >= 0 && (MODE & EPI_SPLITK) != 0;
  constexpr int NS = gemm_max_bn(MODE) / 64;
  const GemmSmemLayout lay = gemm_smem_layout(p.BN, p.stages, W4 ? 1 : 0, gemm_res_bytes(MODE), SPLITK);
  uint64_t* bars = reinterpret_cast<uint64_t*>(smem + lay.bar_offset);
  uint64_t* full_bar = bars;
  uint64_t* empty_bar = bars + GEMM_MAX_STAGES;
  uint64_t* ready_bar = bars + 2 * GEMM_MAX_STAGES;
  uint64_t* res_bar = bars + 3 * GEMM_MAX_STAGES;

  const int warp = threadIdx.x >> 5;
  const int lane = threadIdx.x & 31;
  const int splits = p.splits > 1 ? p.splits : 1;
  const int num_tiles = p.tiles_m * p.tiles_n * splits;
  const int kb_per_tap = (p.C + GEMM_BK - 1) / GEMM_BK;
  const int num_kb_all = kb_per_tap * p.taps * p.kdup;
  const int kb_slice = splits > 1 ? p.kb_per_split : num_kb_all;

  if (warp == 0 && lane == 0) {
    tma_prefetch_desc(&tmA);
    tma_prefetch_desc(&tmB);
    if constexpr (RES_TMA) tma_prefetch_desc(&tmR);
  }
  if (warp == 1 && lane == 0) {
    for (int s = 0; s < p.stages; ++s) {
      mbar_init(&full_bar[s], 1);
      mbar_init(&empty_bar[s], EPI_WARPS / 4);
      if constexpr (W4) mbar_init(&ready_bar[s], 4);
    }
    if constexpr (RES_TMA)
      for (int s = 0; s < EPI_WARPS * GEMM_RES_NBUF; ++s) mbar_init(&res_bar[s], 1);
    fence_mbar_init();
    fence_proxy_async();
  }
  __syncthreads();

  if (warp == 0) {
    if (lane == 0) {
      int stage = 0;
      uint32_t phase = 0;
      const uint32_t tx_bytes = (uint32_t)(GEMM_A_STAGE_BYTES + (W4 ? p.BN * (GEMM_BK / 2) : p.BN * GEMM_BK));
      for (int item = blockIdx.x; item < num_tiles; item += gridDim.x) {
        const int tile = item / splits;
        const int kb0 = (item - tile * splits) * kb_slice;
        const int kb1 = min(num_kb_all, kb0 + kb_slice);
        const int tm = tile / p.tiles_n;
        const int tn = tile - tm * p.tiles_n;
        const int m0 = tm * GEMM_BM;
        const int n0 = tn * p.BN;
        int b0 = 0, h0 = 0, w0 = 0;
        if (p.taps == 9) {
          const int hw = p.H * p.W;
          b0 = m0 / hw;
          h0 = (m0 - b0 * hw) / p.W;
          w0 = m0 - b0 * hw - h0 * p.W;
        }
        int seg = kb0 / kb_per_tap, kc = kb0 - seg * kb_per_tap;
        for (int kb = kb0; kb < kb1; ++kb) {
          const int tap = seg % p.taps;
          const int ky = tap / 3, kx = tap - ky * 3;
          {
            mbar_wait(&empty_bar[stage], phase ^ 1);
            uint8_t* sa = smem + (size_t)stage * lay.stage_bytes;
            uint8_t* sb = sa + GEMM_A_STAGE_BYTES;
            mbar_arrive_expect_tx(&full_bar[stage], tx_bytes);
            if (p.taps == 9)
              tma_load_4d(sa, &tmA, &full_bar[stage], kc * GEMM_BK, w0 + kx - 1, h0 + ky - 1, b0);
            else
              tma_load_4d(sa, &tmA, &full_bar[stage], kc * GEMM_BK, m0, 0, 0);
            if constexpr (W4)
              tma_load_2d(smem + lay.pack_off + (size_t)stage * p.BN * (GEMM_BK / 2), &tmB, &full_bar[stage],
                          (seg * p.C + kc * GEMM_BK) / 2, n0);
            else
              tma_load_2d(sb, &tmB, &full_bar[stage], seg * p.C + kc * GEMM_BK, n0);
            if (++stage == p.stages) { stage = 0; phase ^= 1; }
          }
          if (++kc == kb_per_tap) { kc = 0; ++seg; }
        }
      }
    }
  } else if (warp == 2 || warp == 3 || warp >= 4 + EPI_WARPS) {
    if constexpr (W4) {
      const int t = warp < 4 ? (int)threadIdx.x - 64 : (int)threadIdx.x - (4 + EPI_WARPS) * 32 + 64;
      const int r32 = t >> 2, piece = t & 3;
      int stage = 0;
      uint32_t phase = 0;
      for (int item = blockIdx.x; item < num_tiles; item += gridDim.x) {
        const int tile = item / splits;
        const int kb0 = (item - tile * splits) * kb_slice;
        const int num_kb = min(num_kb_all, kb0 + kb_slice) - kb0;
        const int tn = tile % p.tiles_n;
        const int n0 = tn * p.BN;
        uint32_t kz[8];
#pragma unroll
        for (int i = 0; i < 8; ++i) {
          const int n = n0 + r32 + 32 * i;
          kz[i] = 0x80808080u - ((r32 + 32 * i < p.BN && n < p.N) ? 0x01010101u * (uint32_t)(uint8_t)__ldg(p.wzero + n) : 0u);
        }
        for (int kb = 0; kb < num_kb; ++kb) {
          mbar_wait(&full_bar[stage], phase);
          const uint8_t* sp = smem + lay.pack_off + (size_t)stage * p.BN * (GEMM_BK / 2);
          uint8_t* sb = smem + (size_t)stage * lay.stage_bytes + GEMM_A_STAGE_BYTES;
#pragma unroll
          for (int i = 0; i < 8; ++i) {
            const int row = r32 + 32 * i;
            if (row < p.BN) {
              const uint4 w = *reinterpret_cast<const uint4*>(sp + row * (GEMM_BK / 2) + piece * 16);
              const uint32_t in[4] = {w.x, w.y, w.z, w.w};
              uint32_t o[8];
#pragma unroll
              for (int q = 0; q < 4; ++q) {
                o[2 * q] = ((in[q] & 0x0F0F0F0Fu) + kz[i]) ^ 0x80808080u;
                o[2 * q + 1] = (((in[q] >> 4) & 0x0F0F0F0Fu) + kz[i]) ^ 0x80808080u;
              }
              uint8_t* dst = sb + row * GEMM_BK;
              *reinterpret_cast<uint4*>(dst + (((2 * piece) ^ (row & 7)) << 4)) = make_uint4(o[0], o[1], o[2], o[3]);
              *reinterpret_cast<uint4*>(dst + (((2 * piece + 1) ^ (row & 7)) << 4)) = make_uint4(o[4], o[5], o[6], o[7]);
            }
          }
          fence_proxy_async();
          __syncwarp();
          if (lane == 0) mbar_arrive(&ready_bar[stage]);
          if (++stage == p.stages) { stage = 0; phase ^= 1; }
        }
      }
    }
  } else if (warp >= 4 && warp < 4 + EPI_WARPS) {
    const int cw = warp - 4;
    const int wg = cw >> 2;
    const bool wg_leader = (threadIdx.x & 127) == 0;
    const int q = cw & 3;
    const int half = cw >> 2;
    const int nch = (p.BN + 31) >> 5;
    uint8_t* const acc_tile = smem + lay.stage_off;
    const uint8_t* stg = acc_tile;
    constexpr bool BF16 = MODE >= 0 && (MODE & EPI_BF16) != 0;
    using AccT = typename std::conditional<BF16, float, uint32_t>::type;
    int stage = 0;
    uint32_t phase = 0;
    const int rsub = lane >> 3;
    const int cq = lane & 7;
    constexpr bool QPRE = gemm_qpre(MODE);
    const QuantK qk = QPRE ? make_quantk_pre(p.q_delta, p.q_lo, p.q_hi) : make_quantk(p.q_delta, p.q_zp, p.q_lo, p.q_hi);
    const float* const ep_scale = QPRE ? p.scale_q : p.scale;
    const float* const ep_bias = QPRE ? p.bias_q : p.bias;
    const bool conv = MODE < 0 ? (p.taps == 9) : ((MODE & EPI_CONV) != 0);
    uint8_t* rring = smem + lay.res_off + (warp - 4) * (GEMM_RES_NBUF * 4096);
    uint64_t* rbar = res_bar + (warp - 4) * GEMM_RES_NBUF;
    int pf_tile = blockIdx.x, pf_c = half * 32, pf_buf = 0;
    int rd_buf = 0;
    uint32_t rd_phase = 0;
    auto res_issue = [&]() {
      if (pf_tile >= num_tiles) return;
      if (lane == 0) {
        const int ptm = pf_tile / p.tiles_n, ptn = pf_tile - ptm * p.tiles_n;
        mbar_arrive_expect_tx(&rbar[pf_buf], 4096u);
        tma_load_2d(rring + pf_buf * 4096, &tmR, &rbar[pf_buf], (ptn * p.BN + pf_c) * 4, ptm * GEMM_BM + q * 32);
      }
      if (++pf_buf == GEMM_RES_NBUF) pf_buf = 0;
      pf_c += CSTEP;
      if (pf_c >= p.BN) { pf_c = half * 32; pf_tile += gridDim.x; }
    };
    if constexpr (RES_TMA) {
      if (half * 32 >= p.BN) pf_tile = num_tiles;
#pragma unroll 1
      for (int i = 0; i < GEMM_RES_NBUF - 1; ++i) res_issue();
    }
    for (int item = blockIdx.x; item < num_tiles; item += gridDim.x) {
      const int tile = item / splits;
      const int zsplit = item - tile * splits;
      const int tm = tile / p.tiles_n;
      const int tn = tile - tm * p.tiles_n;
      const int n_base = tn * p.BN;
      const int m_warp = tm * GEMM_BM + q * 32;
      const bool transposed = (MODE < 0) && p.out_q_transposed;
      constexpr bool kTrans = MODE >= 0 && (MODE & EPI_TRANS) != 0;
      int cls8[8], img8[8];
      if (!transposed && !kTrans) {
#pragma unroll
        for (int it = 0; it < 8; ++it) gemm_row_meta(p, m_warp + it * 4 + rsub, cls8[it], img8[it]);
      }
      {
        AccT accr[NS][32];
#pragma unroll
        for (int s = 0; s < NS; ++s)
#pragma unroll
          for (int i = 0; i < 32; ++i) accr[s][i] = 0;
        const int kb0 = zsplit * kb_slice;
        const int kb1 = min(num_kb_all, kb0 + kb_slice);
        int prev_stage = -1;
        auto mainloop = [&](auto cfg) {
          using Cfg = decltype(cfg);
          for (int kb = kb0; kb < kb1; ++kb) {
            mbar_wait(&full_bar[stage], phase);
            if constexpr (W4) mbar_wait(&ready_bar[stage], phase);
            wgmma_fence();
            const uint32_t sa = smem_u32(smem + (size_t)stage * lay.stage_bytes);
            const uint64_t da = make_smem_desc_sw128(sa + (uint32_t)(wg * 64 * GEMM_BK));
            const uint64_t db = make_smem_desc_sw128(sa + GEMM_A_STAGE_BYTES);
            gemm_wgmma_kblock<BF16, Cfg::SIGNED, Cfg::NF, Cfg::TAIL>(accr, da, db, kb > kb0 ? 1u : 0u);
            wgmma_commit();
            wgmma_wait<1>();
            if (prev_stage >= 0 && wg_leader) mbar_arrive(&empty_bar[prev_stage]);
            prev_stage = stage;
            if (++stage == p.stages) { stage = 0; phase ^= 1; }
          }
          wgmma_wait<0>();
        };
        if constexpr (BF16) gemm_dispatch_bn<NS, true>(p.BN, mainloop);
        else if (p.a_signed) gemm_dispatch_bn<NS, true>(p.BN, mainloop);
        else gemm_dispatch_bn<NS, false>(p.BN, mainloop);
#pragma unroll
        for (int s = 0; s < NS; ++s) wgmma_fence_regs(accr[s]);
        if (prev_stage >= 0 && wg_leader) mbar_arrive(&empty_bar[prev_stage]);
        const int r0 = 64 * wg + 16 * (cw & 3) + (lane >> 2);
        if constexpr (SPLITK) {
          int32_t* wz = p.ws + (long long)zsplit * p.M * p.N;
#pragma unroll
          for (int s = 0; s < NS; ++s)
#pragma unroll
            for (int j = 0; j < 8; ++j) {
              const int n = n_base + 64 * s + 8 * j + 2 * (lane & 3);
              if (64 * s + 8 * j < p.BN && n < p.N) {
#pragma unroll
                for (int h = 0; h < 2; ++h) {
                  const int m = tm * GEMM_BM + r0 + 8 * h;
                  if (m < p.M)
                    *reinterpret_cast<uint2*>(wz + (long long)m * p.N + n) = make_uint2(accr[s][4 * j + 2 * h], accr[s][4 * j + 2 * h + 1]);
                }
              }
            }
          continue;
        }
        named_bar_sync(1, EPI_WARPS * 32);
#pragma unroll
        for (int s = 0; s < NS; ++s)
#pragma unroll
          for (int j = 0; j < 8; ++j) {
            const int col = 64 * s + 8 * j + 2 * (lane & 3);
            if (col < p.BN) {
#pragma unroll
              for (int h = 0; h < 2; ++h) {
                const int row = r0 + 8 * h;
                uint8_t* dst = acc_tile + ((row >> 5) * nch + (col >> 5)) * GEMM_EPI_TILE_BYTES + (row & 31) * 128 +
                               ((((col & 31) >> 2) ^ (row & 7)) << 4) + (col & 3) * 4;
                uint32_t lo, hi;
                if constexpr (BF16) { lo = __float_as_uint(accr[s][4 * j + 2 * h]); hi = __float_as_uint(accr[s][4 * j + 2 * h + 1]); }
                else { lo = accr[s][4 * j + 2 * h]; hi = accr[s][4 * j + 2 * h + 1]; }
                *reinterpret_cast<uint2*>(dst) = make_uint2(lo, hi);
              }
            }
          }
      }
      named_bar_sync(1, EPI_WARPS * 32);
      if constexpr (kTrans) {
        const int img = m_warp / p.rows_per_batch;
        const int tok0 = m_warp - img * p.rows_per_batch;
        for (int c = half * 32; c < p.BN; c += CSTEP) {
          const int ncols = (p.BN - c) >= 32 ? 32 : 16;
          stg = acc_tile + (q * nch + (c >> 5)) * GEMM_EPI_TILE_BYTES;
          const int col = ncols == 32 ? lane : (lane & 15);
          const int n = n_base + c + col;
          if (m_warp < p.M && n < p.N) {
            const float sc1 = __ldg(ep_scale + n);
            const float bi1 = ep_bias ? __ldg(ep_bias + n) : 0.f;
            int cr = 0;
            if constexpr ((MODE & EPI_CORR) != 0) cr = __ldg(p.corr + n);
            int8_t* o = p.out_q + ((long long)img * p.N + n) * p.ldq + tok0;
            const uint8_t* src = stg + (col & 3) * 4;
            const int cj = col >> 2;
            const int g0 = ncols == 32 ? 0 : (lane >> 4), g1 = ncols == 32 ? 2 : g0 + 1;
            for (int g = g0; g < g1; ++g) {
              uint32_t w4[4];
#pragma unroll
              for (int k = 0; k < 16; ++k) {
                const int r7 = (((k >> 1) & 1) << 3) | (((k >> 2) & 3) << 1) | (k & 1);
                const int a = *reinterpret_cast<const int*>(src + (g * 16 + r7) * 128 + ((cj ^ (r7 & 7)) << 4));
                const uint32_t qv = QPRE ? (quant_bits_pre(fmaf((float)(a - cr), sc1, bi1), qk) & 0xFFu)
                                         : quant_code((float)(a - cr) * sc1 + bi1, qk);
                w4[k >> 2] = (k & 3) ? (w4[k >> 2] | (qv << (8 * (k & 3)))) : qv;
              }
              *reinterpret_cast<uint4*>(o + g * 16) = make_uint4(w4[0], w4[1], w4[2], w4[3]);
            }
          }
          __syncwarp();
        }
      } else if constexpr (MODE >= 0 && (MODE & EPI_GEGLU) != 0) {
        const int r8 = lane >> 2, pq = lane & 3;
        for (int c = half * 32; c < p.BN; c += CSTEP) {
          stg = acc_tile + (q * nch + (c >> 5)) * GEMM_EPI_TILE_BYTES;
          const int nx = n_base + c + 8 * pq;
          if (nx < p.N) {
            const float4 sx = __ldg(reinterpret_cast<const float4*>(p.scale + nx));
            const float4 sg = __ldg(reinterpret_cast<const float4*>(p.scale + nx + 4));
            float4 bx = make_float4(0.f, 0.f, 0.f, 0.f), bg = bx;
            if (p.bias) {
              bx = __ldg(reinterpret_cast<const float4*>(p.bias + nx));
              bg = __ldg(reinterpret_cast<const float4*>(p.bias + nx + 4));
            }
            int4 cx = make_int4(0, 0, 0, 0), cg = cx;
            if constexpr ((MODE & EPI_CORR) != 0) {
              cx = __ldg(reinterpret_cast<const int4*>(p.corr + nx));
              cg = __ldg(reinterpret_cast<const int4*>(p.corr + nx + 4));
            }
#pragma unroll
            for (int it = 0; it < 4; ++it) {
              const int row = it * 8 + r8;
              const int m = m_warp + row;
              if (m < p.M) {
                const uint4 ax = *reinterpret_cast<const uint4*>(stg + row * 128 + (((2 * pq) ^ (row & 7)) << 4));
                const uint4 ag = *reinterpret_cast<const uint4*>(stg + row * 128 + (((2 * pq + 1) ^ (row & 7)) << 4));
                const float x0 = (float)((int)ax.x - cx.x) * sx.x + bx.x, g0 = (float)((int)ag.x - cg.x) * sg.x + bg.x;
                const float x1 = (float)((int)ax.y - cx.y) * sx.y + bx.y, g1 = (float)((int)ag.y - cg.y) * sg.y + bg.y;
                const float x2 = (float)((int)ax.z - cx.z) * sx.z + bx.z, g2 = (float)((int)ag.z - cg.z) * sg.z + bg.z;
                const float x3 = (float)((int)ax.w - cx.w) * sx.w + bx.w, g3 = (float)((int)ag.w - cg.w) * sg.w + bg.w;
                const uint32_t code = quant_code_fast(x0 * gelu_fast(g0), qk) | (quant_code_fast(x1 * gelu_fast(g1), qk) << 8) |
                                      (quant_code_fast(x2 * gelu_fast(g2), qk) << 16) | (quant_code_fast(x3 * gelu_fast(g3), qk) << 24);
                *reinterpret_cast<uint32_t*>(p.out_q + (long long)m * p.ldq + (nx >> 1)) = code;
              }
            }
          }
          __syncwarp();
        }
      } else if (transposed) {
        const int m = m_warp + lane;
        int cls, img;
        gemm_row_meta(p, m, cls, img);
        for (int c = half * 32; c < p.BN; c += CSTEP) {
          if (p.BN - c >= 32) {
            uint32_t v[32];
            gemm_acc_row(acc_tile + (q * nch + (c >> 5)) * GEMM_EPI_TILE_BYTES, lane, v);
            if (m < p.M && n_base + c < p.N) gemm_epilogue_rowwise<32>(p, qk, v, m, n_base + c, cls, img);
          } else {
            uint32_t v[16];
            gemm_acc_row(acc_tile + (q * nch + (c >> 5)) * GEMM_EPI_TILE_BYTES, lane, v);
            if (m < p.M && n_base + c < p.N) gemm_epilogue_rowwise<16>(p, qk, v, m, n_base + c, cls, img);
          }
        }
      } else {
        for (int c = half * 32; c < p.BN; c += CSTEP) {
          const int ncols = (p.BN - c) >= 32 ? 32 : 16;
          stg = acc_tile + (q * nch + (c >> 5)) * GEMM_EPI_TILE_BYTES;
          const uint8_t* rbuf = nullptr;
          if constexpr (RES_TMA) {
            res_issue();
            mbar_wait(&rbar[rd_buf], rd_phase);
            rbuf = rring + rd_buf * 4096;
          }
          const int n = n_base + c + cq * 4;
          const bool col_ok = cq * 4 < ncols && n < p.N;
          const unsigned cmask = __ballot_sync(0xffffffffu, col_ok);
          if (col_ok) {
            float sc[4], bi[4];
            int4 corr4 = make_int4(0, 0, 0, 0);
            if (MODE >= 0 || n + 3 < p.N) {
              const float4 s4 = *reinterpret_cast<const float4*>(ep_scale + n);
              sc[0] = s4.x; sc[1] = s4.y; sc[2] = s4.z; sc[3] = s4.w;
              if (ep_bias) {
                const float4 b4 = *reinterpret_cast<const float4*>(ep_bias + n);
                bi[0] = b4.x; bi[1] = b4.y; bi[2] = b4.z; bi[3] = b4.w;
              } else {
                bi[0] = bi[1] = bi[2] = bi[3] = 0.f;
              }
              if (p.corr && !conv) corr4 = *reinterpret_cast<const int4*>(p.corr + n);
            } else {
              int cc[4] = {0, 0, 0, 0};
#pragma unroll
              for (int j = 0; j < 4; ++j) {
                const bool ok = n + j < p.N;
                sc[j] = ok ? __ldg(p.scale + n + j) : 0.f;
                bi[j] = (ok && p.bias) ? __ldg(p.bias + n + j) : 0.f;
                cc[j] = (ok && p.corr && !conv) ? __ldg(p.corr + n + j) : 0;
              }
              corr4 = make_int4(cc[0], cc[1], cc[2], cc[3]);
            }
            int nq = n;
            if (p.oq_d > 0) { const int hq = n / p.oq_d; nq = hq * p.oq_pitch + (n - hq * p.oq_d); }
            const long long mrow = m_warp + rsub;
            float* of0 = p.out ? p.out + mrow * p.ldo + n : nullptr;
            const int oq_es = p.oq_f16 ? 2 : 1;
            int8_t* oq0 = p.out_q ? p.out_q + (mrow * p.ldq + nq) * oq_es : nullptr;
            const float* res0 = p.residual ? p.residual + mrow * p.ldr + n : nullptr;
            const long long of_step = 4 * p.ldo, oq_step = 4 * p.ldq * oq_es, res_step = 4 * p.ldr;
            float gsum[4] = {0.f, 0.f, 0.f, 0.f}, gsq[4] = {0.f, 0.f, 0.f, 0.f};
            auto rows = [&](auto full_tag) {
              constexpr bool FULL = decltype(full_tag)::value;
#pragma unroll
              for (int h4 = 0; h4 < 8; h4 += 4) {
                float4 rpre[4];
                int4 cpre[4];
#pragma unroll
                for (int i = 0; i < 4; ++i) {
                  const int it = h4 + i;
                  [[maybe_unused]] const int m = m_warp + it * 4 + rsub;
                  rpre[i] = make_float4(0.f, 0.f, 0.f, 0.f);
                  cpre[i] = corr4;
                  if constexpr (RES_TMA) {
                    const int row = it * 4 + rsub;
                    rpre[i] = *reinterpret_cast<const float4*>(rbuf + row * 128 + ((cq ^ (row & 7)) << 4));
                  } else if constexpr (MODE >= 0 && (MODE & EPI_RESIDUAL) != 0) {
                    if (FULL || m < p.M) rpre[i] = *reinterpret_cast<const float4*>(res0 + it * res_step);
                  }
                  if constexpr (MODE >= 0 && (MODE & EPI_CORR) != 0 && (MODE & EPI_CONV) != 0)
                    cpre[i] = __ldg(reinterpret_cast<const int4*>(p.corr + (long long)cls8[it] * p.N + n));
                }
#pragma unroll
                for (int i = 0; i < 4; ++i) {
                  const int it = h4 + i;
                  const int row = it * 4 + rsub;
                  const int m = m_warp + row;
                  if (FULL || m < p.M) {
                    const uint4 a4 = *reinterpret_cast<const uint4*>(stg + row * 128 + ((cq ^ (row & 7)) << 4));
                    gemm_finalise4<MODE>(p, qk, conv, a4, sc, bi, cpre[i], rpre[i], of0 + it * of_step, oq0 + it * oq_step,
                                         res0 + it * res_step, n, cls8[it], img8[it], gsum, gsq);
                  }
                }
              }
            };
            if (m_warp + 32 <= p.M) rows(std::true_type{}); else rows(std::false_type{});
            if ((MODE < 0 || (MODE & EPI_OUT_F32) != 0) && p.gn_stats != nullptr) {
#pragma unroll
              for (int j = 0; j < 4; ++j) {
                gsum[j] += __shfl_xor_sync(cmask, gsum[j], 8);
                gsq[j] += __shfl_xor_sync(cmask, gsq[j], 8);
                gsum[j] += __shfl_xor_sync(cmask, gsum[j], 16);
                gsq[j] += __shfl_xor_sync(cmask, gsq[j], 16);
              }
              if (rsub == 0) {
                float2* st = p.gn_stats + (long long)(m_warp >> 5) * p.ld_stats + n;
                if (MODE >= 0 || n + 3 < p.N) {
                  *reinterpret_cast<float4*>(st) = make_float4(gsum[0], gsq[0], gsum[1], gsq[1]);
                  *reinterpret_cast<float4*>(st + 2) = make_float4(gsum[2], gsq[2], gsum[3], gsq[3]);
                } else {
#pragma unroll
                  for (int j = 0; j < 4; ++j)
                    if (n + j < p.N) st[j] = make_float2(gsum[j], gsq[j]);
                }
              }
            }
          }
          if constexpr (RES_TMA) {
            fence_proxy_async();
            if (++rd_buf == GEMM_RES_NBUF) { rd_buf = 0; rd_phase ^= 1; }
          }
          __syncwarp();
        }
      }
    }
  }
}

__global__ void __launch_bounds__(256) splitk_finish_kernel(const GemmArgs p) {
  __shared__ float sy[32][33], sq[32][33];
  const int r = threadIdx.x >> 3, q = threadIdx.x & 7;
  const int m = blockIdx.y * 32 + r;
  const int n = blockIdx.x * 32 + q * 4;
  const bool ok = m < p.M && n < p.N;
  float4 y = make_float4(0.f, 0.f, 0.f, 0.f);
  if (ok) {
    const long long slice = (long long)p.M * p.N;
    const int32_t* w = p.ws + (long long)m * p.N + n;
    int4 a = *reinterpret_cast<const int4*>(w);
#pragma unroll 4
    for (int z = 1; z < p.splits; ++z) {
      const int4 v = *reinterpret_cast<const int4*>(w + z * slice);
      a.x += v.x; a.y += v.y; a.z += v.z; a.w += v.w;
    }
    int cls, img;
    gemm_row_meta(p, m, cls, img);
    if (p.corr) {
      const int4 c = __ldg(reinterpret_cast<const int4*>(p.corr + (p.taps == 9 ? (long long)cls * p.N : 0) + n));
      a.x -= c.x; a.y -= c.y; a.z -= c.z; a.w -= c.w;
    }
    const float4 sc = __ldg(reinterpret_cast<const float4*>(p.scale + n));
    float4 bi = make_float4(0.f, 0.f, 0.f, 0.f);
    if (p.bias) bi = __ldg(reinterpret_cast<const float4*>(p.bias + n));
    y = make_float4((float)a.x * sc.x + bi.x, (float)a.y * sc.y + bi.y, (float)a.z * sc.z + bi.z, (float)a.w * sc.w + bi.w);
    if (p.rowvec) {
      const float4 rv = __ldg(reinterpret_cast<const float4*>(p.rowvec + (long long)img * p.ld_rowvec + n));
      y.x += rv.x; y.y += rv.y; y.z += rv.z; y.w += rv.w;
    }
    if (p.residual) {
      const float4 rs = *reinterpret_cast<const float4*>(p.residual + (long long)m * p.ldr + n);
      y.x += rs.x; y.y += rs.y; y.z += rs.z; y.w += rs.w;
    }
    *reinterpret_cast<float4*>(p.out + (long long)m * p.ldo + n) = y;
  }
  if (p.gn_stats) {
    sy[r][4 * q] = y.x; sy[r][4 * q + 1] = y.y; sy[r][4 * q + 2] = y.z; sy[r][4 * q + 3] = y.w;
    sq[r][4 * q] = y.x * y.x; sq[r][4 * q + 1] = y.y * y.y; sq[r][4 * q + 2] = y.z * y.z; sq[r][4 * q + 3] = y.w * y.w;
    __syncthreads();
    if (threadIdx.x < 32) {
      const int col = blockIdx.x * 32 + threadIdx.x;
      if (col < p.N) {
        float s0 = 0.f, s1 = 0.f;
#pragma unroll
        for (int i = 0; i < 32; ++i) { s0 += sy[i][threadIdx.x]; s1 += sq[i][threadIdx.x]; }
        p.gn_stats[(long long)blockIdx.y * p.ld_stats + col] = make_float2(s0, s1);
      }
    }
  }
}

}
```

q-diffusion_b200/csrc/ptx.cuh:

```cuda
#pragma once
#include <cuda.h>
#include <cuda_runtime.h>
#include <stdint.h>
#include <stdio.h>
#include <type_traits>

namespace qd {

__device__ __forceinline__ uint32_t smem_u32(const void* p) {
  return static_cast<uint32_t>(__cvta_generic_to_shared(p));
}

__device__ __forceinline__ bool elect_one() {
  uint32_t pred = 0;
  asm volatile(
      "{\n\t"
      ".reg .pred P;\n\t"
      "elect.sync _|P, 0xffffffff;\n\t"
      "selp.u32 %0, 1, 0, P;\n\t"
      "}\n"
      : "=r"(pred));
  return pred != 0;
}

__device__ __forceinline__ void mbar_init(uint64_t* bar, uint32_t count) {
  asm volatile("mbarrier.init.shared::cta.b64 [%0], %1;" ::"r"(smem_u32(bar)), "r"(count) : "memory");
}
__device__ __forceinline__ void fence_mbar_init() {
  asm volatile("fence.mbarrier_init.release.cluster;" ::: "memory");
}
__device__ __forceinline__ void fence_proxy_async() {
  asm volatile("fence.proxy.async.shared::cta;" ::: "memory");
}
__device__ __forceinline__ void mbar_arrive_expect_tx(uint64_t* bar, uint32_t bytes) {
  asm volatile("mbarrier.arrive.expect_tx.shared::cta.b64 _, [%0], %1;" ::"r"(smem_u32(bar)), "r"(bytes)
               : "memory");
}
__device__ __forceinline__ void mbar_arrive(uint64_t* bar) {
  asm volatile("mbarrier.arrive.shared::cta.b64 _, [%0];" ::"r"(smem_u32(bar)) : "memory");
}
__device__ __forceinline__ bool mbar_try_wait(uint64_t* bar, uint32_t parity) {
  uint32_t ok;
  asm volatile(
      "{\n\t"
      ".reg .pred P;\n\t"
      "mbarrier.try_wait.parity.shared::cta.b64 P, [%1], %2;\n\t"
      "selp.u32 %0, 1, 0, P;\n\t"
      "}\n"
      : "=r"(ok)
      : "r"(smem_u32(bar)), "r"(parity)
      : "memory");
  return ok != 0;
}
__device__ __forceinline__ uint64_t globaltimer_ns() {
  uint64_t t;
  asm volatile("mov.u64 %0, %%globaltimer;" : "=l"(t));
  return t;
}
__device__ __forceinline__ void mbar_wait(uint64_t* bar, uint32_t parity) {
  if (mbar_try_wait(bar, parity)) return;
  const uint64_t t0 = globaltimer_ns();
  uint32_t spins = 0;
  while (!mbar_try_wait(bar, parity)) {
    if ((++spins & 1023u) == 0 && globaltimer_ns() - t0 > 2000000000ull) {
      __trap();
    }
  }
}

__device__ __forceinline__ void tma_prefetch_desc(const CUtensorMap* m) {
  asm volatile("prefetch.tensormap [%0];" ::"l"(m) : "memory");
}
__device__ __forceinline__ void tma_load_2d(void* smem_dst, const CUtensorMap* m, uint64_t* bar, int c0, int c1) {
  asm volatile(
      "cp.async.bulk.tensor.2d.shared::cluster.global.tile.mbarrier::complete_tx::bytes [%0], [%1, {%3, %4}], [%2];"
      ::"r"(smem_u32(smem_dst)), "l"(m), "r"(smem_u32(bar)), "r"(c0), "r"(c1)
      : "memory");
}
__device__ __forceinline__ void tma_load_4d(void* smem_dst, const CUtensorMap* m, uint64_t* bar, int c0, int c1,
                                            int c2, int c3) {
  asm volatile(
      "cp.async.bulk.tensor.4d.shared::cluster.global.tile.mbarrier::complete_tx::bytes [%0], [%1, {%3, %4, %5, "
      "%6}], [%2];" ::"r"(smem_u32(smem_dst)),
      "l"(m), "r"(smem_u32(bar)), "r"(c0), "r"(c1), "r"(c2), "r"(c3)
      : "memory");
}

__device__ __forceinline__ void bulk_load_1d(void* smem_dst, const void* gsrc, uint32_t bytes, uint64_t* bar) {
  asm volatile("cp.async.bulk.shared::cluster.global.mbarrier::complete_tx::bytes [%0], [%1], %2, [%3];" ::"r"(
                   smem_u32(smem_dst)),
               "l"(gsrc), "r"(bytes), "r"(smem_u32(bar))
               : "memory");
}

__device__ __forceinline__ void named_bar_sync(uint32_t id, uint32_t threads) {
  asm volatile("bar.sync %0, %1;" ::"r"(id), "r"(threads) : "memory");
}

__device__ __forceinline__ void wgmma_fence() { asm volatile("wgmma.fence.sync.aligned;" ::: "memory"); }
__device__ __forceinline__ void wgmma_commit() { asm volatile("wgmma.commit_group.sync.aligned;" ::: "memory"); }
template <int N>
__device__ __forceinline__ void wgmma_wait() { asm volatile("wgmma.wait_group.sync.aligned %0;" ::"n"(N) : "memory"); }
template <typename T>
__device__ __forceinline__ void wgmma_fence_regs(T (&d)[32]) {
#pragma unroll
  for (int i = 0; i < 32; ++i) {
    if constexpr (std::is_same<T, float>::value) asm volatile("" : "+f"(d[i])::"memory");
    else asm volatile("" : "+r"(d[i])::"memory");
  }
}

__device__ __forceinline__ uint64_t make_smem_desc_sw128(uint32_t smem_addr) {
  uint64_t d = 0;
  d |= (uint64_t)((smem_addr & 0x3FFFF) >> 4);
  d |= (uint64_t)1 << 16;
  d |= (uint64_t)(1024 >> 4) << 32;
  d |= (uint64_t)1 << 62;
  return d;
}

__device__ __forceinline__ void wgmma_s8s8_n16(uint32_t (&d)[32], uint64_t da, uint64_t db, uint32_t scale_d) {
  asm volatile(
      "{\n\t.reg .pred p;\n\t"
      "setp.ne.b32 p, %10, 0;\n\t"
      "wgmma.mma_async.sync.aligned.m64n16k32.s32.s8.s8 "
      "{%0, %1, %2, %3, %4, %5, %6, %7}, %8, %9, p;\n\t}\n"
      : "+r"(d[0]), "+r"(d[1]), "+r"(d[2]), "+r"(d[3]), "+r"(d[4]), "+r"(d[5]), "+r"(d[6]), "+r"(d[7])
      : "l"(da), "l"(db), "r"(scale_d));
}
__device__ __forceinline__ void wgmma_u8s8_n16(uint32_t (&d)[32], uint64_t da, uint64_t db, uint32_t scale_d) {
  asm volatile(
      "{\n\t.reg .pred p;\n\t"
      "setp.ne.b32 p, %10, 0;\n\t"
      "wgmma.mma_async.sync.aligned.m64n16k32.s32.u8.s8 "
      "{%0, %1, %2, %3, %4, %5, %6, %7}, %8, %9, p;\n\t}\n"
      : "+r"(d[0]), "+r"(d[1]), "+r"(d[2]), "+r"(d[3]), "+r"(d[4]), "+r"(d[5]), "+r"(d[6]), "+r"(d[7])
      : "l"(da), "l"(db), "r"(scale_d));
}
__device__ __forceinline__ void wgmma_bf16_n16(float (&d)[32], uint64_t da, uint64_t db, uint32_t scale_d) {
  asm volatile(
      "{\n\t.reg .pred p;\n\t"
      "setp.ne.b32 p, %10, 0;\n\t"
      "wgmma.mma_async.sync.aligned.m64n16k16.f32.bf16.bf16 "
      "{%0, %1, %2, %3, %4, %5, %6, %7}, %8, %9, p, 1, 1, 0, 0;\n\t}\n"
      : "+f"(d[0]), "+f"(d[1]), "+f"(d[2]), "+f"(d[3]), "+f"(d[4]), "+f"(d[5]), "+f"(d[6]), "+f"(d[7])
      : "l"(da), "l"(db), "r"(scale_d));
}
__device__ __forceinline__ void wgmma_s8s8_n32(uint32_t (&d)[32], uint64_t da, uint64_t db, uint32_t scale_d) {
  asm volatile(
      "{\n\t.reg .pred p;\n\t"
      "setp.ne.b32 p, %18, 0;\n\t"
      "wgmma.mma_async.sync.aligned.m64n32k32.s32.s8.s8 "
      "{%0, %1, %2, %3, %4, %5, %6, %7, %8, %9, %10, %11, %12, %13, %14, %15}, %16, %17, p;\n\t}\n"
      : "+r"(d[0]), "+r"(d[1]), "+r"(d[2]), "+r"(d[3]), "+r"(d[4]), "+r"(d[5]), "+r"(d[6]), "+r"(d[7]), "+r"(d[8]), "+r"(d[9]), "+r"(d[10]), "+r"(d[11]), "+r"(d[12]), "+r"(d[13]), "+r"(d[14]), "+r"(d[15])
      : "l"(da), "l"(db), "r"(scale_d));
}
__device__ __forceinline__ void wgmma_u8s8_n32(uint32_t (&d)[32], uint64_t da, uint64_t db, uint32_t scale_d) {
  asm volatile(
      "{\n\t.reg .pred p;\n\t"
      "setp.ne.b32 p, %18, 0;\n\t"
      "wgmma.mma_async.sync.aligned.m64n32k32.s32.u8.s8 "
      "{%0, %1, %2, %3, %4, %5, %6, %7, %8, %9, %10, %11, %12, %13, %14, %15}, %16, %17, p;\n\t}\n"
      : "+r"(d[0]), "+r"(d[1]), "+r"(d[2]), "+r"(d[3]), "+r"(d[4]), "+r"(d[5]), "+r"(d[6]), "+r"(d[7]), "+r"(d[8]), "+r"(d[9]), "+r"(d[10]), "+r"(d[11]), "+r"(d[12]), "+r"(d[13]), "+r"(d[14]), "+r"(d[15])
      : "l"(da), "l"(db), "r"(scale_d));
}
__device__ __forceinline__ void wgmma_bf16_n32(float (&d)[32], uint64_t da, uint64_t db, uint32_t scale_d) {
  asm volatile(
      "{\n\t.reg .pred p;\n\t"
      "setp.ne.b32 p, %18, 0;\n\t"
      "wgmma.mma_async.sync.aligned.m64n32k16.f32.bf16.bf16 "
      "{%0, %1, %2, %3, %4, %5, %6, %7, %8, %9, %10, %11, %12, %13, %14, %15}, %16, %17, p, 1, 1, 0, 0;\n\t}\n"
      : "+f"(d[0]), "+f"(d[1]), "+f"(d[2]), "+f"(d[3]), "+f"(d[4]), "+f"(d[5]), "+f"(d[6]), "+f"(d[7]), "+f"(d[8]), "+f"(d[9]), "+f"(d[10]), "+f"(d[11]), "+f"(d[12]), "+f"(d[13]), "+f"(d[14]), "+f"(d[15])
      : "l"(da), "l"(db), "r"(scale_d));
}
__device__ __forceinline__ void wgmma_s8s8_n48(uint32_t (&d)[32], uint64_t da, uint64_t db, uint32_t scale_d) {
  asm volatile(
      "{\n\t.reg .pred p;\n\t"
      "setp.ne.b32 p, %26, 0;\n\t"
      "wgmma.mma_async.sync.aligned.m64n48k32.s32.s8.s8 "
      "{%0, %1, %2, %3, %4, %5, %6, %7, %8, %9, %10, %11, %12, %13, %14, %15, %16, %17, %18, %19, %20, %21, %22, %23}, %24, %25, p;\n\t}\n"
      : "+r"(d[0]), "+r"(d[1]), "+r"(d[2]), "+r"(d[3]), "+r"(d[4]), "+r"(d[5]), "+r"(d[6]), "+r"(d[7]), "+r"(d[8]), "+r"(d[9]), "+r"(d[10]), "+r"(d[11]), "+r"(d[12]), "+r"(d[13]), "+r"(d[14]), "+r"(d[15]), "+r"(d[16]), "+r"(d[17]), "+r"(d[18]), "+r"(d[19]), "+r"(d[20]), "+r"(d[21]), "+r"(d[22]), "+r"(d[23])
      : "l"(da), "l"(db), "r"(scale_d));
}
__device__ __forceinline__ void wgmma_u8s8_n48(uint32_t (&d)[32], uint64_t da, uint64_t db, uint32_t scale_d) {
  asm volatile(
      "{\n\t.reg .pred p;\n\t"
      "setp.ne.b32 p, %26, 0;\n\t"
      "wgmma.mma_async.sync.aligned.m64n48k32.s32.u8.s8 "
      "{%0, %1, %2, %3, %4, %5, %6, %7, %8, %9, %10, %11, %12, %13, %14, %15, %16, %17, %18, %19, %20, %21, %22, %23}, %24, %25, p;\n\t}\n"
      : "+r"(d[0]), "+r"(d[1]), "+r"(d[2]), "+r"(d[3]), "+r"(d[4]), "+r"(d[5]), "+r"(d[6]), "+r"(d[7]), "+r"(d[8]), "+r"(d[9]), "+r"(d[10]), "+r"(d[11]), "+r"(d[12]), "+r"(d[13]), "+r"(d[14]), "+r"(d[15]), "+r"(d[16]), "+r"(d[17]), "+r"(d[18]), "+r"(d[19]), "+r"(d[20]), "+r"(d[21]), "+r"(d[22]), "+r"(d[23])
      : "l"(da), "l"(db), "r"(scale_d));
}
__device__ __forceinline__ void wgmma_bf16_n48(float (&d)[32], uint64_t da, uint64_t db, uint32_t scale_d) {
  asm volatile(
      "{\n\t.reg .pred p;\n\t"
      "setp.ne.b32 p, %26, 0;\n\t"
      "wgmma.mma_async.sync.aligned.m64n48k16.f32.bf16.bf16 "
      "{%0, %1, %2, %3, %4, %5, %6, %7, %8, %9, %10, %11, %12, %13, %14, %15, %16, %17, %18, %19, %20, %21, %22, %23}, %24, %25, p, 1, 1, 0, 0;\n\t}\n"
      : "+f"(d[0]), "+f"(d[1]), "+f"(d[2]), "+f"(d[3]), "+f"(d[4]), "+f"(d[5]), "+f"(d[6]), "+f"(d[7]), "+f"(d[8]), "+f"(d[9]), "+f"(d[10]), "+f"(d[11]), "+f"(d[12]), "+f"(d[13]), "+f"(d[14]), "+f"(d[15]), "+f"(d[16]), "+f"(d[17]), "+f"(d[18]), "+f"(d[19]), "+f"(d[20]), "+f"(d[21]), "+f"(d[22]), "+f"(d[23])
      : "l"(da), "l"(db), "r"(scale_d));
}
__device__ __forceinline__ void wgmma_s8s8_n64(uint32_t (&d)[32], uint64_t da, uint64_t db, uint32_t scale_d) {
  asm volatile(
      "{\n\t.reg .pred p;\n\t"
      "setp.ne.b32 p, %34, 0;\n\t"
      "wgmma.mma_async.sync.aligned.m64n64k32.s32.s8.s8 "
      "{%0, %1, %2, %3, %4, %5, %6, %7, %8, %9, %10, %11, %12, %13, %14, %15, %16, %17, %18, %19, %20, %21, %22, %23, %24, %25, %26, %27, %28, %29, %30, %31}, %32, %33, p;\n\t}\n"
      : "+r"(d[0]), "+r"(d[1]), "+r"(d[2]), "+r"(d[3]), "+r"(d[4]), "+r"(d[5]), "+r"(d[6]), "+r"(d[7]), "+r"(d[8]), "+r"(d[9]), "+r"(d[10]), "+r"(d[11]), "+r"(d[12]), "+r"(d[13]), "+r"(d[14]), "+r"(d[15]), "+r"(d[16]), "+r"(d[17]), "+r"(d[18]), "+r"(d[19]), "+r"(d[20]), "+r"(d[21]), "+r"(d[22]), "+r"(d[23]), "+r"(d[24]), "+r"(d[25]), "+r"(d[26]), "+r"(d[27]), "+r"(d[28]), "+r"(d[29]), "+r"(d[30]), "+r"(d[31])
      : "l"(da), "l"(db), "r"(scale_d));
}
__device__ __forceinline__ void wgmma_u8s8_n64(uint32_t (&d)[32], uint64_t da, uint64_t db, uint32_t scale_d) {
  asm volatile(
      "{\n\t.reg .pred p;\n\t"
      "setp.ne.b32 p, %34, 0;\n\t"
      "wgmma.mma_async.sync.aligned.m64n64k32.s32.u8.s8 "
      "{%0, %1, %2, %3, %4, %5, %6, %7, %8, %9, %10, %11, %12, %13, %14, %15, %16, %17, %18, %19, %20, %21, %22, %23, %24, %25, %26, %27, %28, %29, %30, %31}, %32, %33, p;\n\t}\n"
      : "+r"(d[0]), "+r"(d[1]), "+r"(d[2]), "+r"(d[3]), "+r"(d[4]), "+r"(d[5]), "+r"(d[6]), "+r"(d[7]), "+r"(d[8]), "+r"(d[9]), "+r"(d[10]), "+r"(d[11]), "+r"(d[12]), "+r"(d[13]), "+r"(d[14]), "+r"(d[15]), "+r"(d[16]), "+r"(d[17]), "+r"(d[18]), "+r"(d[19]), "+r"(d[20]), "+r"(d[21]), "+r"(d[22]), "+r"(d[23]), "+r"(d[24]), "+r"(d[25]), "+r"(d[26]), "+r"(d[27]), "+r"(d[28]), "+r"(d[29]), "+r"(d[30]), "+r"(d[31])
      : "l"(da), "l"(db), "r"(scale_d));
}
__device__ __forceinline__ void wgmma_bf16_n64(float (&d)[32], uint64_t da, uint64_t db, uint32_t scale_d) {
  asm volatile(
      "{\n\t.reg .pred p;\n\t"
      "setp.ne.b32 p, %34, 0;\n\t"
      "wgmma.mma_async.sync.aligned.m64n64k16.f32.bf16.bf16 "
      "{%0, %1, %2, %3, %4, %5, %6, %7, %8, %9, %10, %11, %12, %13, %14, %15, %16, %17, %18, %19, %20, %21, %22, %23, %24, %25, %26, %27, %28, %29, %30, %31}, %32, %33, p, 1, 1, 0, 0;\n\t}\n"
      : "+f"(d[0]), "+f"(d[1]), "+f"(d[2]), "+f"(d[3]), "+f"(d[4]), "+f"(d[5]), "+f"(d[6]), "+f"(d[7]), "+f"(d[8]), "+f"(d[9]), "+f"(d[10]), "+f"(d[11]), "+f"(d[12]), "+f"(d[13]), "+f"(d[14]), "+f"(d[15]), "+f"(d[16]), "+f"(d[17]), "+f"(d[18]), "+f"(d[19]), "+f"(d[20]), "+f"(d[21]), "+f"(d[22]), "+f"(d[23]), "+f"(d[24]), "+f"(d[25]), "+f"(d[26]), "+f"(d[27]), "+f"(d[28]), "+f"(d[29]), "+f"(d[30]), "+f"(d[31])
      : "l"(da), "l"(db), "r"(scale_d));
}

}
```

Measured before the change: 3.662.

## Use single wide WGMMA instructions up to N=256 with register reallocation and chunked epilogue

Result: faster. 3.742 (median of 6 runs) (+2.2%).

```diff
diff --git a/q-diffusion_b200/csrc/engine.cu b/q-diffusion_b200/csrc/engine.cu
--- a/q-diffusion_b200/csrc/engine.cu
+++ b/q-diffusion_b200/csrc/engine.cu
@@ -137,14 +137,14 @@
   int grid, mode;
 };
 
-int pick_bn(int N, int tiles_m, int sms, int hint, int step, long long K) {
+int pick_bn(int N, int tiles_m, int sms, int hint, int step, int num_kb, int max_bn) {
   if (hint > 0) return hint;
   static const int wave_model = [] { const char* e = getenv("QDIFF_BN_MODEL"); return (e && !strcmp(e, "wave")) ? 1 : 0; }();
   int best = step;
   double best_cost = -1.0;
   const int n16 = (N + step - 1) / step * step;
-  const double kb = (double)((K + 127) / 128);
-  for (int bn = step; bn <= qd::GEMM_MAX_BN; bn += step) {
+  const double kb = (double)num_kb;
+  for (int bn = step; bn <= max_bn; bn += step) {
     if (bn > n16) break;
     const long long tiles = (long long)tiles_m * ((N + bn - 1) / bn);
     const long long waves = (tiles + sms - 1) / sms;
@@ -152,9 +152,7 @@
     if (wave_model) {
       cost = (double)waves * (bn + 24);
     } else {
-      const double main_loop = kb * (2.1 * bn > 3.0 * (128 + bn) ? 2.1 * bn : 3.0 * (128 + bn));
-      const double epilogue = 6.0 * bn + 300.0;
-      cost = (double)waves * ((main_loop > epilogue ? main_loop : epilogue) + 200.0);
+      cost = (double)waves * (kb * (608.0 + 3.16 * bn) + 115.0 * bn);
     }
     if (best_cost < 0 || cost < best_cost - 1e-9 || (cost < best_cost + 1e-9 && bn > best)) {
       best_cost = cost;
@@ -200,22 +198,7 @@
     if ((d->N & 7) || !d->out_q || d->out || d->rowvec || d->residual || d->out_q_transposed || (d->ldq & 3) || d->taps != 1)
       return fail(QD_ERR_BAD_ARG, "gemm: geglu needs N %% 8 == 0, out_q only, plain GEMM");
   }
-  a.BN = pick_bn(d->N, a.tiles_m, sms, d->bn_hint, d->geglu ? 32 : 16, (long long)d->C * d->taps * a.kdup);
-  const int bn_default = a.BN;
-  static const int splitk_enabled = [] { const char* e = getenv("QDIFF_SPLITK"); return (e && !strcmp(e, "0")) ? 0 : 1; }();
-  const int num_kb_all = ((d->C + qd::GEMM_BK - 1) / qd::GEMM_BK) * d->taps * a.kdup;
-  const bool splitk_candidate = splitk_enabled && !d->bn_hint && !d->a_bf16 && !d->w_int4_packed && d->out && !d->out_q && !d->geglu &&
-                                !(d->N & 3) && !(d->ldo & 3) && (!d->residual || !(d->ldr & 3)) && (!d->rowvec || !(d->ld_rowvec & 3)) &&
-                                num_kb_all >= 16;
-  if (splitk_candidate) {
-    const int bn_wide = d->N >= qd::GEMM_MAX_BN_SPLITK ? qd::GEMM_MAX_BN_SPLITK : (d->N + 15) / 16 * 16;
-    if (2 * a.tiles_m * ((d->N + bn_wide - 1) / bn_wide) <= sms) a.BN = bn_wide;
-  }
-  if (a.BN % 16 || a.BN < 16 || a.BN > qd::GEMM_MAX_BN_SPLITK || (d->bn_hint && a.BN > qd::GEMM_MAX_BN))
-    return fail(QD_ERR_BAD_ARG, "gemm: bad BN %d (16 .. %d)", a.BN, qd::GEMM_MAX_BN);
-  a.tiles_n = (d->N + a.BN - 1) / a.BN;
   a.a_signed = d->a_signed; a.b_signed = 1;
-
 
   cuuint64_t dims[4], strides[3];
   cuuint32_t box[4];
@@ -280,9 +263,25 @@
   if ((d->scale_q == nullptr) != (d->bias_q == nullptr)) return fail(QD_ERR_BAD_ARG, "gemm: scale_q and bias_q come together");
   a.rowvec = d->rowvec; a.ld_rowvec = d->ld_rowvec;
   a.residual = d->residual; a.ldr = d->ldr;
+  pl->mode = gemm_mode(a);
+  const int num_kb_all = ((d->C + qd::GEMM_BK - 1) / qd::GEMM_BK) * d->taps * a.kdup;
+  const int max_bn = qd::gemm_max_bn(pl->mode, a.w4);
+  const int auto_max_bn = num_kb_all < 16 && max_bn > qd::GEMM_ACC_TILE_COLS ? qd::GEMM_ACC_TILE_COLS : max_bn;
+  if (d->bn_hint && (d->bn_hint % 16 || d->bn_hint < 16 || d->bn_hint > max_bn))
+    return fail(QD_ERR_BAD_ARG, "gemm: bad bn_hint %d (a multiple of 16, 16 .. %d for this layer)", d->bn_hint, max_bn);
+  a.BN = pick_bn(d->N, a.tiles_m, sms, d->bn_hint, d->geglu ? 32 : 16, num_kb_all, auto_max_bn);
+  const int bn_default = a.BN;
+  static const int splitk_enabled = [] { const char* e = getenv("QDIFF_SPLITK"); return (e && !strcmp(e, "0")) ? 0 : 1; }();
+  const bool splitk_candidate = splitk_enabled && !d->bn_hint && !d->a_bf16 && !d->w_int4_packed && d->out && !d->out_q && !d->geglu &&
+                                !(d->N & 3) && !(d->ldo & 3) && (!d->residual || !(d->ldr & 3)) && (!d->rowvec || !(d->ld_rowvec & 3)) &&
+                                num_kb_all >= 16;
+  if (splitk_candidate) {
+    const int bn_wide = d->N >= qd::GEMM_MAX_BN ? qd::GEMM_MAX_BN : (d->N + 15) / 16 * 16;
+    if (2 * a.tiles_m * ((d->N + bn_wide - 1) / bn_wide) <= sms) a.BN = bn_wide;
+  }
+  a.tiles_n = (d->N + a.BN - 1) / a.BN;
   const int tiles = a.tiles_m * a.tiles_n;
   pl->grid = tiles < sms ? tiles : sms;
-  pl->mode = gemm_mode(a);
   {
     const int num_kb = num_kb_all;
     const bool eligible = splitk_candidate && pl->mode >= 0 && 2 * tiles <= sms &&
@@ -302,7 +301,7 @@
       }
     }
   }
-  if (a.splits <= 1 && a.BN > qd::GEMM_MAX_BN) {
+  if (a.splits <= 1 && a.BN != bn_default) {
     a.BN = bn_default;
     a.tiles_n = (d->N + a.BN - 1) / a.BN;
     const int t = a.tiles_m * a.tiles_n;
@@ -344,7 +343,7 @@
   const int stage_bytes = qd::gemm_stage_footprint(a.BN, W4 ? 1 : 0);
   constexpr int res_bytes = qd::gemm_res_bytes(MODE);
   constexpr bool splitk = MODE >= 0 && (MODE & qd::EPI_SPLITK) != 0;
-  if (a.BN > qd::gemm_max_bn(MODE)) return fail(QD_ERR_BAD_ARG, "gemm: BN=%d exceeds %d (mode %d)", a.BN, qd::gemm_max_bn(MODE), MODE);
+  if (a.BN > qd::gemm_max_bn(MODE, W4)) return fail(QD_ERR_BAD_ARG, "gemm: BN=%d exceeds %d (mode %d, w4 %d)", a.BN, qd::gemm_max_bn(MODE, W4), MODE, (int)W4);
   int stages = (232448 - 512 - qd::gemm_acc_tile_bytes(a.BN, splitk) - res_bytes - 1024 - 1024) / stage_bytes;
   if (stages > qd::GEMM_MAX_STAGES) stages = qd::GEMM_MAX_STAGES;
   if (stages < 2) stages = 2;
diff --git a/q-diffusion_b200/csrc/gemm_i8.cuh b/q-diffusion_b200/csrc/gemm_i8.cuh
--- a/q-diffusion_b200/csrc/gemm_i8.cuh
+++ b/q-diffusion_b200/csrc/gemm_i8.cuh
@@ -8,8 +8,11 @@
 
 constexpr int GEMM_BM = 128;
 constexpr int GEMM_BK = 128;
-constexpr int GEMM_MAX_BN = 128;
-constexpr int GEMM_MAX_BN_SPLITK = 256;
+constexpr int GEMM_MAX_BN = 256;
+constexpr int GEMM_MAX_BN_NARROW = 128;
+constexpr int GEMM_ACC_TILE_COLS = 128;
+constexpr int GEMM_PRODUCER_REGS = 40;
+constexpr int GEMM_CONSUMER_REGS = 232;
 __host__ __device__ constexpr int gemm_epi_warps(int MODE) { return (void)MODE, 8; }
 constexpr int GEMM_RES_NBUF = 3;
 __host__ __device__ constexpr bool gemm_res_tma(int MODE) { return MODE >= 0 && (MODE & 4) != 0 && (MODE & 256) != 0; }
@@ -20,8 +23,9 @@
 constexpr int GEMM_A_STAGE_BYTES = GEMM_BM * GEMM_BK;
 constexpr int GEMM_MAX_STAGES = 8;
 constexpr int GEMM_EPI_TILE_BYTES = 32 * 128;
+__host__ __device__ inline int gemm_acc_tile_cols(int BN) { return BN < GEMM_ACC_TILE_COLS ? BN : GEMM_ACC_TILE_COLS; }
 __host__ __device__ inline int gemm_acc_tile_bytes(int BN, bool splitk = false) {
-  return splitk ? 0 : 4 * ((BN + 31) / 32) * GEMM_EPI_TILE_BYTES;
+  return splitk ? 0 : 4 * ((gemm_acc_tile_cols(BN) + 31) / 32) * GEMM_EPI_TILE_BYTES;
 }
 
 constexpr int EPI_CORR = 1;
@@ -35,7 +39,9 @@
 constexpr int EPI_RESTMA = 256;
 constexpr int EPI_BF16 = 512;
 constexpr int EPI_SPLITK = 1024;
-__host__ __device__ constexpr int gemm_max_bn(int MODE) { return (MODE >= 0 && (MODE & EPI_SPLITK) != 0) ? GEMM_MAX_BN_SPLITK : GEMM_MAX_BN; }
+__host__ __device__ constexpr int gemm_max_bn(int MODE, bool W4) {
+  return (W4 || MODE < 0 || gemm_res_tma(MODE)) ? GEMM_MAX_BN_NARROW : GEMM_MAX_BN;
+}
 
 struct GemmArgs {
   int M, N;
@@ -291,68 +297,49 @@
   }
 }
 
-template <bool BF16, bool SIGNED, int NF, int TAIL, int NS, typename T>
-__device__ __forceinline__ void gemm_wgmma_kblock(T (&acc)[NS][32], uint64_t da, uint64_t db, uint32_t scale_first) {
+template <bool BF16, bool SIGNED, int BN, int R, typename T>
+__device__ __forceinline__ void gemm_wgmma_kblock(T (&acc)[R], uint64_t da, uint64_t db, uint32_t scale_first) {
 #pragma unroll
   for (int j = 0; j < 4; ++j) {
     const uint32_t sd = j ? 1u : scale_first;
     const uint64_t a = da + (uint64_t)(2 * j);
-#pragma unroll
-    for (int s = 0; s <= NF; ++s) {
-      const uint64_t b = db + (uint64_t)((s * 64 * GEMM_BK) >> 4) + (uint64_t)(2 * j);
-      if (s < NF) {
-        if constexpr (BF16) wgmma_bf16_n64(acc[s < NS ? s : 0], a, b, sd);
-        else if constexpr (SIGNED) wgmma_s8s8_n64(acc[s < NS ? s : 0], a, b, sd);
-        else wgmma_u8s8_n64(acc[s < NS ? s : 0], a, b, sd);
-      } else if constexpr (TAIL != 0) {
-        constexpr int t = NF < NS ? NF : 0;
-        if constexpr (BF16) {
-          if constexpr (TAIL == 48) wgmma_bf16_n48(acc[t], a, b, sd);
-          else if constexpr (TAIL == 32) wgmma_bf16_n32(acc[t], a, b, sd);
-          else wgmma_bf16_n16(acc[t], a, b, sd);
-        } else if constexpr (SIGNED) {
-          if constexpr (TAIL == 48) wgmma_s8s8_n48(acc[t], a, b, sd);
-          else if constexpr (TAIL == 32) wgmma_s8s8_n32(acc[t], a, b, sd);
-          else wgmma_s8s8_n16(acc[t], a, b, sd);
-        } else {
-          if constexpr (TAIL == 48) wgmma_u8s8_n48(acc[t], a, b, sd);
-          else if constexpr (TAIL == 32) wgmma_u8s8_n32(acc[t], a, b, sd);
-          else wgmma_u8s8_n16(acc[t], a, b, sd);
-        }
-      }
-    }
-  }
-}
-
-template <int NF_, int TAIL_, bool SIGNED_>
+    const uint64_t b = db + (uint64_t)(2 * j);
+    if constexpr (BF16) wgmma_bf16_n<BN>(acc, a, b, sd);
+    else if constexpr (SIGNED) wgmma_s8s8_n<BN>(acc, a, b, sd);
+    else wgmma_u8s8_n<BN>(acc, a, b, sd);
+  }
+}
+
+template <int BN_, bool SIGNED_>
 struct GemmNCfg {
-  static constexpr int NF = NF_, TAIL = TAIL_;
+  static constexpr int BN = BN_;
   static constexpr bool SIGNED = SIGNED_;
 };
-template <int NS, bool S, typename F>
+template <int BN_MAX, bool S, typename F>
 __device__ __forceinline__ void gemm_dispatch_bn(int BN, F&& f) {
   switch (BN >> 4) {
-    case 1: f(GemmNCfg<0, 16, S>{}); break;
-    case 2: f(GemmNCfg<0, 32, S>{}); break;
-    case 3: f(GemmNCfg<0, 48, S>{}); break;
-    case 4: f(GemmNCfg<1, 0, S>{}); break;
-    case 5: f(GemmNCfg<1, 16, S>{}); break;
-    case 6: f(GemmNCfg<1, 32, S>{}); break;
-    case 7: f(GemmNCfg<1, 48, S>{}); break;
+    case 1: f(GemmNCfg<16, S>{}); break;
+    case 2: f(GemmNCfg<32, S>{}); break;
+    case 3: f(GemmNCfg<48, S>{}); break;
+    case 4: f(GemmNCfg<64, S>{}); break;
+    case 5: f(GemmNCfg<80, S>{}); break;
+    case 6: f(GemmNCfg<96, S>{}); break;
+    case 7: f(GemmNCfg<112, S>{}); break;
     default:
-      if constexpr (NS == 2) {
-        f(GemmNCfg<2, 0, S>{});
+      if constexpr (BN_MAX == 128) {
+        f(GemmNCfg<128, S>{});
       } else {
+        static_assert(BN_MAX == 256, "N tiles up to 128 or 256 columns");
         switch (BN >> 4) {
-          case 8: f(GemmNCfg<2, 0, S>{}); break;
-          case 9: f(GemmNCfg<2, 16, S>{}); break;
-          case 10: f(GemmNCfg<2, 32, S>{}); break;
-          case 11: f(GemmNCfg<2, 48, S>{}); break;
-          case 12: f(GemmNCfg<3, 0, S>{}); break;
-          case 13: f(GemmNCfg<3, 16, S>{}); break;
-          case 14: f(GemmNCfg<3, 32, S>{}); break;
-          case 15: f(GemmNCfg<3, 48, S>{}); break;
-          default: f(GemmNCfg<4, 0, S>{}); break;
+          case 8: f(GemmNCfg<128, S>{}); break;
+          case 9: f(GemmNCfg<144, S>{}); break;
+          case 10: f(GemmNCfg<160, S>{}); break;
+          case 11: f(GemmNCfg<176, S>{}); break;
+          case 12: f(GemmNCfg<192, S>{}); break;
+          case 13: f(GemmNCfg<208, S>{}); break;
+          case 14: f(GemmNCfg<224, S>{}); break;
+          case 15: f(GemmNCfg<240, S>{}); break;
+          default: f(GemmNCfg<256, S>{}); break;
         }
       }
   }
@@ -371,7 +358,7 @@
   constexpr int CSTEP = 32 * (EPI_WARPS / 4);
   constexpr bool RES_TMA = gemm_res_tma(MODE);
   constexpr bool SPLITK = MODE >= 0 && (MODE & EPI_SPLITK) != 0;
-  constexpr int NS = gemm_max_bn(MODE) / 64;
+  constexpr int BN_MAX = gemm_max_bn(MODE, W4);
   const GemmSmemLayout lay = gemm_smem_layout(p.BN, p.stages, W4 ? 1 : 0, gemm_res_bytes(MODE), SPLITK);
   uint64_t* bars = reinterpret_cast<uint64_t*>(smem + lay.bar_offset);
   uint64_t* full_bar = bars;
@@ -406,6 +393,7 @@
   __syncthreads();
 
   if (warp == 0) {
+    if constexpr (!W4) setmaxnreg_dec<GEMM_PRODUCER_REGS>();
     if (lane == 0) {
       int stage = 0;
       uint32_t phase = 0;
@@ -449,8 +437,9 @@
         }
       }
     }
-  } else if (warp == 2 || warp == 3 || warp >= 4 + EPI_WARPS) {
-    if constexpr (W4) {
+  } else if (warp < 4 || warp >= 4 + EPI_WARPS) {
+    if constexpr (!W4) setmaxnreg_dec<GEMM_PRODUCER_REGS>();
+    if (W4 && warp != 1) {
       const int t = warp < 4 ? (int)threadIdx.x - 64 : (int)threadIdx.x - (4 + EPI_WARPS) * 32 + 64;
       const int r32 = t >> 2, piece = t & 3;
       int stage = 0;
@@ -495,13 +484,14 @@
         }
       }
     }
-  } else if (warp >= 4 && warp < 4 + EPI_WARPS) {
+  } else {
+    if constexpr (!W4) setmaxnreg_inc<GEMM_CONSUMER_REGS>();
     const int cw = warp - 4;
     const int wg = cw >> 2;
     const bool wg_leader = (threadIdx.x & 127) == 0;
     const int q = cw & 3;
     const int half = cw >> 2;
-    const int nch = (p.BN + 31) >> 5;
+    const int nch = (gemm_acc_tile_cols(p.BN) + 31) >> 5;
     uint8_t* const acc_tile = smem + lay.stage_off;
     const uint8_t* stg = acc_tile;
     constexpr bool BF16 = MODE >= 0 && (MODE & EPI_BF16) != 0;
@@ -550,12 +540,10 @@
 #pragma unroll
         for (int it = 0; it < 8; ++it) gemm_row_meta(p, m_warp + it * 4 + rsub, cls8[it], img8[it]);
       }
+      AccT accr[BN_MAX / 2];
+#pragma unroll
+      for (int i = 0; i < BN_MAX / 2; ++i) accr[i] = 0;
       {
-        AccT accr[NS][32];
-#pragma unroll
-        for (int s = 0; s < NS; ++s)
-#pragma unroll
-          for (int i = 0; i < 32; ++i) accr[s][i] = 0;
         const int kb0 = zsplit * kb_slice;
         const int kb1 = min(num_kb_all, kb0 + kb_slice);
         int prev_stage = -1;
@@ -568,7 +556,7 @@
             const uint32_t sa = smem_u32(smem + (size_t)stage * lay.stage_bytes);
             const uint64_t da = make_smem_desc_sw128(sa + (uint32_t)(wg * 64 * GEMM_BK));
             const uint64_t db = make_smem_desc_sw128(sa + GEMM_A_STAGE_BYTES);
-            gemm_wgmma_kblock<BF16, Cfg::SIGNED, Cfg::NF, Cfg::TAIL>(accr, da, db, kb > kb0 ? 1u : 0u);
+            gemm_wgmma_kblock<BF16, Cfg::SIGNED, Cfg::BN>(accr, da, db, kb > kb0 ? 1u : 0u);
             wgmma_commit();
             wgmma_wait<1>();
             if (prev_stage >= 0 && wg_leader) mbar_arrive(&empty_bar[prev_stage]);
@@ -577,243 +565,244 @@
           }
           wgmma_wait<0>();
         };
-        if constexpr (BF16) gemm_dispatch_bn<NS, true>(p.BN, mainloop);
-        else if (p.a_signed) gemm_dispatch_bn<NS, true>(p.BN, mainloop);
-        else gemm_dispatch_bn<NS, false>(p.BN, mainloop);
-#pragma unroll
-        for (int s = 0; s < NS; ++s) wgmma_fence_regs(accr[s]);
+        if constexpr (BF16) gemm_dispatch_bn<BN_MAX, true>(p.BN, mainloop);
+        else if (p.a_signed) gemm_dispatch_bn<BN_MAX, true>(p.BN, mainloop);
+        else gemm_dispatch_bn<BN_MAX, false>(p.BN, mainloop);
+        wgmma_fence_regs(accr);
         if (prev_stage >= 0 && wg_leader) mbar_arrive(&empty_bar[prev_stage]);
-        const int r0 = 64 * wg + 16 * (cw & 3) + (lane >> 2);
-        if constexpr (SPLITK) {
-          int32_t* wz = p.ws + (long long)zsplit * p.M * p.N;
-#pragma unroll
-          for (int s = 0; s < NS; ++s)
-#pragma unroll
-            for (int j = 0; j < 8; ++j) {
-              const int n = n_base + 64 * s + 8 * j + 2 * (lane & 3);
-              if (64 * s + 8 * j < p.BN && n < p.N) {
-#pragma unroll
-                for (int h = 0; h < 2; ++h) {
-                  const int m = tm * GEMM_BM + r0 + 8 * h;
-                  if (m < p.M)
-                    *reinterpret_cast<uint2*>(wz + (long long)m * p.N + n) = make_uint2(accr[s][4 * j + 2 * h], accr[s][4 * j + 2 * h + 1]);
+      }
+      const int r0 = 64 * wg + 16 * (cw & 3) + (lane >> 2);
+      if constexpr (SPLITK) {
+        int32_t* wz = p.ws + (long long)zsplit * p.M * p.N;
+#pragma unroll
+        for (int j = 0; j < BN_MAX / 8; ++j) {
+          const int n = n_base + 8 * j + 2 * (lane & 3);
+          if (8 * j < p.BN && n < p.N) {
+#pragma unroll
+            for (int h = 0; h < 2; ++h) {
+              const int m = tm * GEMM_BM + r0 + 8 * h;
+              if (m < p.M)
+                *reinterpret_cast<uint2*>(wz + (long long)m * p.N + n) = make_uint2(accr[4 * j + 2 * h], accr[4 * j + 2 * h + 1]);
+            }
+          }
+        }
+        continue;
+      }
+      constexpr int ACC_PASS = GEMM_ACC_TILE_COLS / 2;
+      for (int c0 = 0; c0 < p.BN && c0 < BN_MAX; c0 += GEMM_ACC_TILE_COLS) {
+        const int c1 = min(p.BN, c0 + GEMM_ACC_TILE_COLS);
+        named_bar_sync(1, EPI_WARPS * 32);
+#pragma unroll
+        for (int j = 0; j < ACC_PASS / 4; ++j) {
+          const int lc = 8 * j + 2 * (lane & 3);
+          if (c0 + lc < c1) {
+#pragma unroll
+            for (int h = 0; h < 2; ++h) {
+              const int row = r0 + 8 * h;
+              uint8_t* dst = acc_tile + ((row >> 5) * nch + (lc >> 5)) * GEMM_EPI_TILE_BYTES + (row & 31) * 128 +
+                             ((((lc & 31) >> 2) ^ (row & 7)) << 4) + (lc & 3) * 4;
+              uint32_t lo, hi;
+              if constexpr (BF16) { lo = __float_as_uint(accr[4 * j + 2 * h]); hi = __float_as_uint(accr[4 * j + 2 * h + 1]); }
+              else { lo = accr[4 * j + 2 * h]; hi = accr[4 * j + 2 * h + 1]; }
+              *reinterpret_cast<uint2*>(dst) = make_uint2(lo, hi);
+            }
+          }
+        }
+#pragma unroll
+        for (int i = 0; i < BN_MAX / 2 - ACC_PASS; ++i) accr[i] = accr[i + ACC_PASS];
+        named_bar_sync(1, EPI_WARPS * 32);
+        if constexpr (kTrans) {
+          const int img = m_warp / p.rows_per_batch;
+          const int tok0 = m_warp - img * p.rows_per_batch;
+          for (int c = c0 + half * 32; c < c1; c += CSTEP) {
+            const int ncols = (p.BN - c) >= 32 ? 32 : 16;
+            stg = acc_tile + (q * nch + ((c - c0) >> 5)) * GEMM_EPI_TILE_BYTES;
+            const int col = ncols == 32 ? lane : (lane & 15);
+            const int n = n_base + c + col;
+            if (m_warp < p.M && n < p.N) {
+              const float sc1 = __ldg(ep_scale + n);
+              const float bi1 = ep_bias ? __ldg(ep_bias + n) : 0.f;
+              int cr = 0;
+              if constexpr ((MODE & EPI_CORR) != 0) cr = __ldg(p.corr + n);
+              int8_t* o = p.out_q + ((long long)img * p.N + n) * p.ldq + tok0;
+              const uint8_t* src = stg + (col & 3) * 4;
+              const int cj = col >> 2;
+              const int g0 = ncols == 32 ? 0 : (lane >> 4), g1 = ncols == 32 ? 2 : g0 + 1;
+              for (int g = g0; g < g1; ++g) {
+                uint32_t w4[4];
+  #pragma unroll
+                for (int k = 0; k < 16; ++k) {
+                  const int r7 = (((k >> 1) & 1) << 3) | (((k >> 2) & 3) << 1) | (k & 1);
+                  const int a = *reinterpret_cast<const int*>(src + (g * 16 + r7) * 128 + ((cj ^ (r7 & 7)) << 4));
+                  const uint32_t qv = QPRE ? (quant_bits_pre(fmaf((float)(a - cr), sc1, bi1), qk) & 0xFFu)
+                                           : quant_code((float)(a - cr) * sc1 + bi1, qk);
+                  w4[k >> 2] = (k & 3) ? (w4[k >> 2] | (qv << (8 * (k & 3)))) : qv;
+                }
+                *reinterpret_cast<uint4*>(o + g * 16) = make_uint4(w4[0], w4[1], w4[2], w4[3]);
+              }
+            }
+            __syncwarp();
+          }
+        } else if constexpr (MODE >= 0 && (MODE & EPI_GEGLU) != 0) {
+          const int r8 = lane >> 2, pq = lane & 3;
+          for (int c = c0 + half * 32; c < c1; c += CSTEP) {
+            stg = acc_tile + (q * nch + ((c - c0) >> 5)) * GEMM_EPI_TILE_BYTES;
+            const int nx = n_base + c + 8 * pq;
+            if (nx < p.N) {
+              const float4 sx = __ldg(reinterpret_cast<const float4*>(p.scale + nx));
+              const float4 sg = __ldg(reinterpret_cast<const float4*>(p.scale + nx + 4));
+              float4 bx = make_float4(0.f, 0.f, 0.f, 0.f), bg = bx;
+              if (p.bias) {
+                bx = __ldg(reinterpret_cast<const float4*>(p.bias + nx));
+                bg = __ldg(reinterpret_cast<const float4*>(p.bias + nx + 4));
+              }
+              int4 cx = make_int4(0, 0, 0, 0), cg = cx;
+              if constexpr ((MODE & EPI_CORR) != 0) {
+                cx = __ldg(reinterpret_cast<const int4*>(p.corr + nx));
+                cg = __ldg(reinterpret_cast<const int4*>(p.corr + nx + 4));
+              }
+  #pragma unroll
+              for (int it = 0; it < 4; ++it) {
+                const int row = it * 8 + r8;
+                const int m = m_warp + row;
+                if (m < p.M) {
+                  const uint4 ax = *reinterpret_cast<const uint4*>(stg + row * 128 + (((2 * pq) ^ (row & 7)) << 4));
+                  const uint4 ag = *reinterpret_cast<const uint4*>(stg + row * 128 + (((2 * pq + 1) ^ (row & 7)) << 4));
+                  const float x0 = (float)((int)ax.x - cx.x) * sx.x + bx.x, g0 = (float)((int)ag.x - cg.x) * sg.x + bg.x;
+                  const float x1 = (float)((int)ax.y - cx.y) * sx.y + bx.y, g1 = (float)((int)ag.y - cg.y) * sg.y + bg.y;
+                  const float x2 = (float)((int)ax.z - cx.z) * sx.z + bx.z, g2 = (float)((int)ag.z - cg.z) * sg.z + bg.z;
+                  const float x3 = (float)((int)ax.w - cx.w) * sx.w + bx.w, g3 = (float)((int)ag.w - cg.w) * sg.w + bg.w;
+                  const uint32_t code = quant_code_fast(x0 * gelu_fast(g0), qk) | (quant_code_fast(x1 * gelu_fast(g1), qk) << 8) |
+                                        (quant_code_fast(x2 * gelu_fast(g2), qk) << 16) | (quant_code_fast(x3 * gelu_fast(g3), qk) << 24);
+                  *reinterpret_cast<uint32_t*>(p.out_q + (long long)m * p.ldq + (nx >> 1)) = code;
                 }
               }
             }
-          continue;
-        }
-        named_bar_sync(1, EPI_WARPS * 32);
-#pragma unroll
-        for (int s = 0; s < NS; ++s)
-#pragma unroll
-          for (int j = 0; j < 8; ++j) {
-            const int col = 64 * s + 8 * j + 2 * (lane & 3);
-            if (col < p.BN) {
-#pragma unroll
-              for (int h = 0; h < 2; ++h) {
-                const int row = r0 + 8 * h;
-                uint8_t* dst = acc_tile + ((row >> 5) * nch + (col >> 5)) * GEMM_EPI_TILE_BYTES + (row & 31) * 128 +
-                               ((((col & 31) >> 2) ^ (row & 7)) << 4) + (col & 3) * 4;
-                uint32_t lo, hi;
-                if constexpr (BF16) { lo = __float_as_uint(accr[s][4 * j + 2 * h]); hi = __float_as_uint(accr[s][4 * j + 2 * h + 1]); }
-                else { lo = accr[s][4 * j + 2 * h]; hi = accr[s][4 * j + 2 * h + 1]; }
-                *reinterpret_cast<uint2*>(dst) = make_uint2(lo, hi);
-              }
+            __syncwarp();
+          }
+        } else if (transposed) {
+          const int m = m_warp + lane;
+          int cls, img;
+          gemm_row_meta(p, m, cls, img);
+          for (int c = c0 + half * 32; c < c1; c += CSTEP) {
+            if (p.BN - c >= 32) {
+              uint32_t v[32];
+              gemm_acc_row(acc_tile + (q * nch + ((c - c0) >> 5)) * GEMM_EPI_TILE_BYTES, lane, v);
+              if (m < p.M && n_base + c < p.N) gemm_epilogue_rowwise<32>(p, qk, v, m, n_base + c, cls, img);
+            } else {
+              uint32_t v[16];
+              gemm_acc_row(acc_tile + (q * nch + ((c - c0) >> 5)) * GEMM_EPI_TILE_BYTES, lane, v);
+              if (m < p.M && n_base + c < p.N) gemm_epilogue_rowwise<16>(p, qk, v, m, n_base + c, cls, img);
             }
           }
-      }
-      named_bar_sync(1, EPI_WARPS * 32);
-      if constexpr (kTrans) {
-        const int img = m_warp / p.rows_per_batch;
-        const int tok0 = m_warp - img * p.rows_per_batch;
-        for (int c = half * 32; c < p.BN; c += CSTEP) {
-          const int ncols = (p.BN - c) >= 32 ? 32 : 16;
-          stg = acc_tile + (q * nch + (c >> 5)) * GEMM_EPI_TILE_BYTES;
-          const int col = ncols == 32 ? lane : (lane & 15);
-          const int n = n_base + c + col;
-          if (m_warp < p.M && n < p.N) {
-            const float sc1 = __ldg(ep_scale + n);
-            const float bi1 = ep_bias ? __ldg(ep_bias + n) : 0.f;
-            int cr = 0;
-            if constexpr ((MODE & EPI_CORR) != 0) cr = __ldg(p.corr + n);
-            int8_t* o = p.out_q + ((long long)img * p.N + n) * p.ldq + tok0;
-            const uint8_t* src = stg + (col & 3) * 4;
-            const int cj = col >> 2;
-            const int g0 = ncols == 32 ? 0 : (lane >> 4), g1 = ncols == 32 ? 2 : g0 + 1;
-            for (int g = g0; g < g1; ++g) {
-              uint32_t w4[4];
-#pragma unroll
-              for (int k = 0; k < 16; ++k) {
-                const int r7 = (((k >> 1) & 1) << 3) | (((k >> 2) & 3) << 1) | (k & 1);
-                const int a = *reinterpret_cast<const int*>(src + (g * 16 + r7) * 128 + ((cj ^ (r7 & 7)) << 4));
-                const uint32_t qv = QPRE ? (quant_bits_pre(fmaf((float)(a - cr), sc1, bi1), qk) & 0xFFu)
-                                         : quant_code((float)(a - cr) * sc1 + bi1, qk);
-                w4[k >> 2] = (k & 3) ? (w4[k >> 2] | (qv << (8 * (k & 3)))) : qv;
+        } else {
+          for (int c = c0 + half * 32; c < c1; c += CSTEP) {
+            const int ncols = (p.BN - c) >= 32 ? 32 : 16;
+            stg = acc_tile + (q * nch + ((c - c0) >> 5)) * GEMM_EPI_TILE_BYTES;
+            const uint8_t* rbuf = nullptr;
+            if constexpr (RES_TMA) {
+              res_issue();
+              mbar_wait(&rbar[rd_buf], rd_phase);
+              rbuf = rring + rd_buf * 4096;
+            }
+            const int n = n_base + c + cq * 4;
+            const bool col_ok = cq * 4 < ncols && n < p.N;
+            const unsigned cmask = __ballot_sync(0xffffffffu, col_ok);
+            if (col_ok) {
+              float sc[4], bi[4];
+              int4 corr4 = make_int4(0, 0, 0, 0);
+              if (MODE >= 0 || n + 3 < p.N) {
+                const float4 s4 = *reinterpret_cast<const float4*>(ep_scale + n);
+                sc[0] = s4.x; sc[1] = s4.y; sc[2] = s4.z; sc[3] = s4.w;
+                if (ep_bias) {
+                  const float4 b4 = *reinterpret_cast<const float4*>(ep_bias + n);
+                  bi[0] = b4.x; bi[1] = b4.y; bi[2] = b4.z; bi[3] = b4.w;
+                } else {
+                  bi[0] = bi[1] = bi[2] = bi[3] = 0.f;
+                }
+                if (p.corr && !conv) corr4 = *reinterpret_cast<const int4*>(p.corr + n);
+              } else {
+                int cc[4] = {0, 0, 0, 0};
+  #pragma unroll
+                for (int j = 0; j < 4; ++j) {
+                  const bool ok = n + j < p.N;
+                  sc[j] = ok ? __ldg(p.scale + n + j) : 0.f;
+                  bi[j] = (ok && p.bias) ? __ldg(p.bias + n + j) : 0.f;
+                  cc[j] = (ok && p.corr && !conv) ? __ldg(p.corr + n + j) : 0;
+                }
+                corr4 = make_int4(cc[0], cc[1], cc[2], cc[3]);
               }
-              *reinterpret_cast<uint4*>(o + g * 16) = make_uint4(w4[0], w4[1], w4[2], w4[3]);
-            }
-          }
-          __syncwarp();
-        }
-      } else if constexpr (MODE >= 0 && (MODE & EPI_GEGLU) != 0) {
-        const int r8 = lane >> 2, pq = lane & 3;
-        for (int c = half * 32; c < p.BN; c += CSTEP) {
-          stg = acc_tile + (q * nch + (c >> 5)) * GEMM_EPI_TILE_BYTES;
-          const int nx = n_base + c + 8 * pq;
-          if (nx < p.N) {
-            const float4 sx = __ldg(reinterpret_cast<const float4*>(p.scale + nx));
-            const float4 sg = __ldg(reinterpret_cast<const float4*>(p.scale + nx + 4));
-            float4 bx = make_float4(0.f, 0.f, 0.f, 0.f), bg = bx;
-            if (p.bias) {
-              bx = __ldg(reinterpret_cast<const float4*>(p.bias + nx));
-              bg = __ldg(reinterpret_cast<const float4*>(p.bias + nx + 4));
-            }
-            int4 cx = make_int4(0, 0, 0, 0), cg = cx;
-            if constexpr ((MODE & EPI_CORR) != 0) {
-              cx = __ldg(reinterpret_cast<const int4*>(p.corr + nx));
-              cg = __ldg(reinterpret_cast<const int4*>(p.corr + nx + 4));
-            }
-#pragma unroll
-            for (int it = 0; it < 4; ++it) {
-              const int row = it * 8 + r8;
-              const int m = m_warp + row;
-              if (m < p.M) {
-                const uint4 ax = *reinterpret_cast<const uint4*>(stg + row * 128 + (((2 * pq) ^ (row & 7)) << 4));
-                const uint4 ag = *reinterpret_cast<const uint4*>(stg + row * 128 + (((2 * pq + 1) ^ (row & 7)) << 4));
-                const float x0 = (float)((int)ax.x - cx.x) * sx.x + bx.x, g0 = (float)((int)ag.x - cg.x) * sg.x + bg.x;
-                const float x1 = (float)((int)ax.y - cx.y) * sx.y + bx.y, g1 = (float)((int)ag.y - cg.y) * sg.y + bg.y;
-                const float x2 = (float)((int)ax.z - cx.z) * sx.z + bx.z, g2 = (float)((int)ag.z - cg.z) * sg.z + bg.z;
-                const float x3 = (float)((int)ax.w - cx.w) * sx.w + bx.w, g3 = (float)((int)ag.w - cg.w) * sg.w + bg.w;
-                const uint32_t code = quant_code_fast(x0 * gelu_fast(g0), qk) | (quant_code_fast(x1 * gelu_fast(g1), qk) << 8) |
-                                      (quant_code_fast(x2 * gelu_fast(g2), qk) << 16) | (quant_code_fast(x3 * gelu_fast(g3), qk) << 24);
-                *reinterpret_cast<uint32_t*>(p.out_q + (long long)m * p.ldq + (nx >> 1)) = code;
-              }
-            }
-          }
-          __syncwarp();
-        }
-      } else if (transposed) {
-        const int m = m_warp + lane;
-        int cls, img;
-        gemm_row_meta(p, m, cls, img);
-        for (int c = half * 32; c < p.BN; c += CSTEP) {
-          if (p.BN - c >= 32) {
-            uint32_t v[32];
-            gemm_acc_row(acc_tile + (q * nch + (c >> 5)) * GEMM_EPI_TILE_BYTES, lane, v);
-            if (m < p.M && n_base + c < p.N) gemm_epilogue_rowwise<32>(p, qk, v, m, n_base + c, cls, img);
-          } else {
-            uint32_t v[16];
-            gemm_acc_row(acc_tile + (q * nch + (c >> 5)) * GEMM_EPI_TILE_BYTES, lane, v);
-            if (m < p.M && n_base + c < p.N) gemm_epilogue_rowwise<16>(p, qk, v, m, n_base + c, cls, img);
-          }
-        }
-      } else {
-        for (int c = half * 32; c < p.BN; c += CSTEP) {
-          const int ncols = (p.BN - c) >= 32 ? 32 : 16;
-          stg = acc_tile + (q * nch + (c >> 5)) * GEMM_EPI_TILE_BYTES;
-          const uint8_t* rbuf = nullptr;
-          if constexpr (RES_TMA) {
-            res_issue();
-            mbar_wait(&rbar[rd_buf], rd_phase);
-            rbuf = rring + rd_buf * 4096;
-          }
-          const int n = n_base + c + cq * 4;
-          const bool col_ok = cq * 4 < ncols && n < p.N;
-          const unsigned cmask = __ballot_sync(0xffffffffu, col_ok);
-          if (col_ok) {
-            float sc[4], bi[4];
-            int4 corr4 = make_int4(0, 0, 0, 0);
-            if (MODE >= 0 || n + 3 < p.N) {
-              const float4 s4 = *reinterpret_cast<const float4*>(ep_scale + n);
-              sc[0] = s4.x; sc[1] = s4.y; sc[2] = s4.z; sc[3] = s4.w;
-              if (ep_bias) {
-                const float4 b4 = *reinterpret_cast<const float4*>(ep_bias + n);
-                bi[0] = b4.x; bi[1] = b4.y; bi[2] = b4.z; bi[3] = b4.w;
-              } else {
-                bi[0] = bi[1] = bi[2] = bi[3] = 0.f;
-              }
-              if (p.corr && !conv) corr4 = *reinterpret_cast<const int4*>(p.corr + n);
-            } else {
-              int cc[4] = {0, 0, 0, 0};
-#pragma unroll
-              for (int j = 0; j < 4; ++j) {
-                const bool ok = n + j < p.N;
-                sc[j] = ok ? __ldg(p.scale + n + j) : 0.f;
-                bi[j] = (ok && p.bias) ? __ldg(p.bias + n + j) : 0.f;
-                cc[j] = (ok && p.corr && !conv) ? __ldg(p.corr + n + j) : 0;
-              }
-              corr4 = make_int4(cc[0], cc[1], cc[2], cc[3]);
-            }
-            int nq = n;
-            if (p.oq_d > 0) { const int hq = n / p.oq_d; nq = hq * p.oq_pitch + (n - hq * p.oq_d); }
-            const long long mrow = m_warp + rsub;
-            float* of0 = p.out ? p.out + mrow * p.ldo + n : nullptr;
-            const int oq_es = p.oq_f16 ? 2 : 1;
-            int8_t* oq0 = p.out_q ? p.out_q + (mrow * p.ldq + nq) * oq_es : nullptr;
-            const float* res0 = p.residual ? p.residual + mrow * p.ldr + n : nullptr;
-            const long long of_step = 4 * p.ldo, oq_step = 4 * p.ldq * oq_es, res_step = 4 * p.ldr;
-            float gsum[4] = {0.f, 0.f, 0.f, 0.f}, gsq[4] = {0.f, 0.f, 0.f, 0.f};
-            auto rows = [&](auto full_tag) {
-              constexpr bool FULL = decltype(full_tag)::value;
-#pragma unroll
-              for (int h4 = 0; h4 < 8; h4 += 4) {
-                float4 rpre[4];
-                int4 cpre[4];
-#pragma unroll
-                for (int i = 0; i < 4; ++i) {
-                  const int it = h4 + i;
-                  [[maybe_unused]] const int m = m_warp + it * 4 + rsub;
-                  rpre[i] = make_float4(0.f, 0.f, 0.f, 0.f);
-                  cpre[i] = corr4;
-                  if constexpr (RES_TMA) {
+              int nq = n;
+              if (p.oq_d > 0) { const int hq = n / p.oq_d; nq = hq * p.oq_pitch + (n - hq * p.oq_d); }
+              const long long mrow = m_warp + rsub;
+              float* of0 = p.out ? p.out + mrow * p.ldo + n : nullptr;
+              const int oq_es = p.oq_f16 ? 2 : 1;
+              int8_t* oq0 = p.out_q ? p.out_q + (mrow * p.ldq + nq) * oq_es : nullptr;
+              const float* res0 = p.residual ? p.residual + mrow * p.ldr + n : nullptr;
+              const long long of_step = 4 * p.ldo, oq_step = 4 * p.ldq * oq_es, res_step = 4 * p.ldr;
+              float gsum[4] = {0.f, 0.f, 0.f, 0.f}, gsq[4] = {0.f, 0.f, 0.f, 0.f};
+              auto rows = [&](auto full_tag) {
+                constexpr bool FULL = decltype(full_tag)::value;
+  #pragma unroll
+                for (int h4 = 0; h4 < 8; h4 += 4) {
+                  float4 rpre[4];
+                  int4 cpre[4];
+  #pragma unroll
+                  for (int i = 0; i < 4; ++i) {
+                    const int it = h4 + i;
+                    [[maybe_unused]] const int m = m_warp + it * 4 + rsub;
+                    rpre[i] = make_float4(0.f, 0.f, 0.f, 0.f);
+                    cpre[i] = corr4;
+                    if constexpr (RES_TMA) {
+                      const int row = it * 4 + rsub;
+                      rpre[i] = *reinterpret_cast<const float4*>(rbuf + row * 128 + ((cq ^ (row & 7)) << 4));
+                    } else if constexpr (MODE >= 0 && (MODE & EPI_RESIDUAL) != 0) {
+                      if (FULL || m < p.M) rpre[i] = *reinterpret_cast<const float4*>(res0 + it * res_step);
+                    }
+                    if constexpr (MODE >= 0 && (MODE & EPI_CORR) != 0 && (MODE & EPI_CONV) != 0)
+                      cpre[i] = __ldg(reinterpret_cast<const int4*>(p.corr + (long long)cls8[it] * p.N + n));
+                  }
+  #pragma unroll
+                  for (int i = 0; i < 4; ++i) {
+                    const int it = h4 + i;
                     const int row = it * 4 + rsub;
-                    rpre[i] = *reinterpret_cast<const float4*>(rbuf + row * 128 + ((cq ^ (row & 7)) << 4));
-                  } else if constexpr (MODE >= 0 && (MODE & EPI_RESIDUAL) != 0) {
-                    if (FULL || m < p.M) rpre[i] = *reinterpret_cast<const float4*>(res0 + it * res_step);
+                    const int m = m_warp + row;
+                    if (FULL || m < p.M) {
+                      const uint4 a4 = *reinterpret_cast<const uint4*>(stg + row * 128 + ((cq ^ (row & 7)) << 4));
+                      gemm_finalise4<MODE>(p, qk, conv, a4, sc, bi, cpre[i], rpre[i], of0 + it * of_step, oq0 + it * oq_step,
+                                           res0 + it * res_step, n, cls8[it], img8[it], gsum, gsq);
+                    }
                   }
-                  if constexpr (MODE >= 0 && (MODE & EPI_CORR) != 0 && (MODE & EPI_CONV) != 0)
-                    cpre[i] = __ldg(reinterpret_cast<const int4*>(p.corr + (long long)cls8[it] * p.N + n));
                 }
-#pragma unroll
-                for (int i = 0; i < 4; ++i) {
-                  const int it = h4 + i;
-                  const int row = it * 4 + rsub;
-                  const int m = m_warp + row;
-                  if (FULL || m < p.M) {
-                    const uint4 a4 = *reinterpret_cast<const uint4*>(stg + row * 128 + ((cq ^ (row & 7)) << 4));
-                    gemm_finalise4<MODE>(p, qk, conv, a4, sc, bi, cpre[i], rpre[i], of0 + it * of_step, oq0 + it * oq_step,
-                                         res0 + it * res_step, n, cls8[it], img8[it], gsum, gsq);
+              };
+              if (m_warp + 32 <= p.M) rows(std::true_type{}); else rows(std::false_type{});
+              if ((MODE < 0 || (MODE & EPI_OUT_F32) != 0) && p.gn_stats != nullptr) {
+  #pragma unroll
+                for (int j = 0; j < 4; ++j) {
+                  gsum[j] += __shfl_xor_sync(cmask, gsum[j], 8);
+                  gsq[j] += __shfl_xor_sync(cmask, gsq[j], 8);
+                  gsum[j] += __shfl_xor_sync(cmask, gsum[j], 16);
+                  gsq[j] += __shfl_xor_sync(cmask, gsq[j], 16);
+                }
+                if (rsub == 0) {
+                  float2* st = p.gn_stats + (long long)(m_warp >> 5) * p.ld_stats + n;
+                  if (MODE >= 0 || n + 3 < p.N) {
+                    *reinterpret_cast<float4*>(st) = make_float4(gsum[0], gsq[0], gsum[1], gsq[1]);
+                    *reinterpret_cast<float4*>(st + 2) = make_float4(gsum[2], gsq[2], gsum[3], gsq[3]);
+                  } else {
+  #pragma unroll
+                    for (int j = 0; j < 4; ++j)
+                      if (n + j < p.N) st[j] = make_float2(gsum[j], gsq[j]);
                   }
                 }
               }
-            };
-            if (m_warp + 32 <= p.M) rows(std::true_type{}); else rows(std::false_type{});
-            if ((MODE < 0 || (MODE & EPI_OUT_F32) != 0) && p.gn_stats != nullptr) {
-#pragma unroll
-              for (int j = 0; j < 4; ++j) {
-                gsum[j] += __shfl_xor_sync(cmask, gsum[j], 8);
-                gsq[j] += __shfl_xor_sync(cmask, gsq[j], 8);
-                gsum[j] += __shfl_xor_sync(cmask, gsum[j], 16);
-                gsq[j] += __shfl_xor_sync(cmask, gsq[j], 16);
-              }
-              if (rsub == 0) {
-                float2* st = p.gn_stats + (long long)(m_warp >> 5) * p.ld_stats + n;
-                if (MODE >= 0 || n + 3 < p.N) {
-                  *reinterpret_cast<float4*>(st) = make_float4(gsum[0], gsq[0], gsum[1], gsq[1]);
-                  *reinterpret_cast<float4*>(st + 2) = make_float4(gsum[2], gsq[2], gsum[3], gsq[3]);
-                } else {
-#pragma unroll
-                  for (int j = 0; j < 4; ++j)
-                    if (n + j < p.N) st[j] = make_float2(gsum[j], gsq[j]);
-                }
-              }
             }
+            if constexpr (RES_TMA) {
+              fence_proxy_async();
+              if (++rd_buf == GEMM_RES_NBUF) { rd_buf = 0; rd_phase ^= 1; }
+            }
+            __syncwarp();
           }
-          if constexpr (RES_TMA) {
-            fence_proxy_async();
-            if (++rd_buf == GEMM_RES_NBUF) { rd_buf = 0; rd_phase ^= 1; }
-          }
-          __syncwarp();
         }
       }
     }
diff --git a/q-diffusion_b200/csrc/ptx.cuh b/q-diffusion_b200/csrc/ptx.cuh
--- a/q-diffusion_b200/csrc/ptx.cuh
+++ b/q-diffusion_b200/csrc/ptx.cuh
@@ -101,10 +101,10 @@
 __device__ __forceinline__ void wgmma_commit() { asm volatile("wgmma.commit_group.sync.aligned;" ::: "memory"); }
 template <int N>
 __device__ __forceinline__ void wgmma_wait() { asm volatile("wgmma.wait_group.sync.aligned %0;" ::"n"(N) : "memory"); }
-template <typename T>
-__device__ __forceinline__ void wgmma_fence_regs(T (&d)[32]) {
+template <typename T, int R>
+__device__ __forceinline__ void wgmma_fence_regs(T (&d)[R]) {
 #pragma unroll
-  for (int i = 0; i < 32; ++i) {
+  for (int i = 0; i < R; ++i) {
     if constexpr (std::is_same<T, float>::value) asm volatile("" : "+f"(d[i])::"memory");
     else asm volatile("" : "+r"(d[i])::"memory");
   }
@@ -119,113 +119,132 @@
   return d;
 }
 
-__device__ __forceinline__ void wgmma_s8s8_n16(uint32_t (&d)[32], uint64_t da, uint64_t db, uint32_t scale_d) {
-  asm volatile(
-      "{\n\t.reg .pred p;\n\t"
-      "setp.ne.b32 p, %10, 0;\n\t"
-      "wgmma.mma_async.sync.aligned.m64n16k32.s32.s8.s8 "
-      "{%0, %1, %2, %3, %4, %5, %6, %7}, %8, %9, p;\n\t}\n"
-      : "+r"(d[0]), "+r"(d[1]), "+r"(d[2]), "+r"(d[3]), "+r"(d[4]), "+r"(d[5]), "+r"(d[6]), "+r"(d[7])
-      : "l"(da), "l"(db), "r"(scale_d));
-}
-__device__ __forceinline__ void wgmma_u8s8_n16(uint32_t (&d)[32], uint64_t da, uint64_t db, uint32_t scale_d) {
-  asm volatile(
-      "{\n\t.reg .pred p;\n\t"
-      "setp.ne.b32 p, %10, 0;\n\t"
-      "wgmma.mma_async.sync.aligned.m64n16k32.s32.u8.s8 "
-      "{%0, %1, %2, %3, %4, %5, %6, %7}, %8, %9, p;\n\t}\n"
-      : "+r"(d[0]), "+r"(d[1]), "+r"(d[2]), "+r"(d[3]), "+r"(d[4]), "+r"(d[5]), "+r"(d[6]), "+r"(d[7])
-      : "l"(da), "l"(db), "r"(scale_d));
-}
-__device__ __forceinline__ void wgmma_bf16_n16(float (&d)[32], uint64_t da, uint64_t db, uint32_t scale_d) {
-  asm volatile(
-      "{\n\t.reg .pred p;\n\t"
-      "setp.ne.b32 p, %10, 0;\n\t"
-      "wgmma.mma_async.sync.aligned.m64n16k16.f32.bf16.bf16 "
-      "{%0, %1, %2, %3, %4, %5, %6, %7}, %8, %9, p, 1, 1, 0, 0;\n\t}\n"
-      : "+f"(d[0]), "+f"(d[1]), "+f"(d[2]), "+f"(d[3]), "+f"(d[4]), "+f"(d[5]), "+f"(d[6]), "+f"(d[7])
-      : "l"(da), "l"(db), "r"(scale_d));
-}
-__device__ __forceinline__ void wgmma_s8s8_n32(uint32_t (&d)[32], uint64_t da, uint64_t db, uint32_t scale_d) {
-  asm volatile(
-      "{\n\t.reg .pred p;\n\t"
-      "setp.ne.b32 p, %18, 0;\n\t"
-      "wgmma.mma_async.sync.aligned.m64n32k32.s32.s8.s8 "
-      "{%0, %1, %2, %3, %4, %5, %6, %7, %8, %9, %10, %11, %12, %13, %14, %15}, %16, %17, p;\n\t}\n"
-      : "+r"(d[0]), "+r"(d[1]), "+r"(d[2]), "+r"(d[3]), "+r"(d[4]), "+r"(d[5]), "+r"(d[6]), "+r"(d[7]), "+r"(d[8]), "+r"(d[9]), "+r"(d[10]), "+r"(d[11]), "+r"(d[12]), "+r"(d[13]), "+r"(d[14]), "+r"(d[15])
-      : "l"(da), "l"(db), "r"(scale_d));
-}
-__device__ __forceinline__ void wgmma_u8s8_n32(uint32_t (&d)[32], uint64_t da, uint64_t db, uint32_t scale_d) {
-  asm volatile(
-      "{\n\t.reg .pred p;\n\t"
-      "setp.ne.b32 p, %18, 0;\n\t"
-      "wgmma.mma_async.sync.aligned.m64n32k32.s32.u8.s8 "
-      "{%0, %1, %2, %3, %4, %5, %6, %7, %8, %9, %10, %11, %12, %13, %14, %15}, %16, %17, p;\n\t}\n"
-      : "+r"(d[0]), "+r"(d[1]), "+r"(d[2]), "+r"(d[3]), "+r"(d[4]), "+r"(d[5]), "+r"(d[6]), "+r"(d[7]), "+r"(d[8]), "+r"(d[9]), "+r"(d[10]), "+r"(d[11]), "+r"(d[12]), "+r"(d[13]), "+r"(d[14]), "+r"(d[15])
-      : "l"(da), "l"(db), "r"(scale_d));
-}
-__device__ __forceinline__ void wgmma_bf16_n32(float (&d)[32], uint64_t da, uint64_t db, uint32_t scale_d) {
-  asm volatile(
-      "{\n\t.reg .pred p;\n\t"
-      "setp.ne.b32 p, %18, 0;\n\t"
-      "wgmma.mma_async.sync.aligned.m64n32k16.f32.bf16.bf16 "
-      "{%0, %1, %2, %3, %4, %5, %6, %7, %8, %9, %10, %11, %12, %13, %14, %15}, %16, %17, p, 1, 1, 0, 0;\n\t}\n"
-      : "+f"(d[0]), "+f"(d[1]), "+f"(d[2]), "+f"(d[3]), "+f"(d[4]), "+f"(d[5]), "+f"(d[6]), "+f"(d[7]), "+f"(d[8]), "+f"(d[9]), "+f"(d[10]), "+f"(d[11]), "+f"(d[12]), "+f"(d[13]), "+f"(d[14]), "+f"(d[15])
-      : "l"(da), "l"(db), "r"(scale_d));
-}
-__device__ __forceinline__ void wgmma_s8s8_n48(uint32_t (&d)[32], uint64_t da, uint64_t db, uint32_t scale_d) {
-  asm volatile(
-      "{\n\t.reg .pred p;\n\t"
-      "setp.ne.b32 p, %26, 0;\n\t"
-      "wgmma.mma_async.sync.aligned.m64n48k32.s32.s8.s8 "
-      "{%0, %1, %2, %3, %4, %5, %6, %7, %8, %9, %10, %11, %12, %13, %14, %15, %16, %17, %18, %19, %20, %21, %22, %23}, %24, %25, p;\n\t}\n"
-      : "+r"(d[0]), "+r"(d[1]), "+r"(d[2]), "+r"(d[3]), "+r"(d[4]), "+r"(d[5]), "+r"(d[6]), "+r"(d[7]), "+r"(d[8]), "+r"(d[9]), "+r"(d[10]), "+r"(d[11]), "+r"(d[12]), "+r"(d[13]), "+r"(d[14]), "+r"(d[15]), "+r"(d[16]), "+r"(d[17]), "+r"(d[18]), "+r"(d[19]), "+r"(d[20]), "+r"(d[21]), "+r"(d[22]), "+r"(d[23])
-      : "l"(da), "l"(db), "r"(scale_d));
-}
-__device__ __forceinline__ void wgmma_u8s8_n48(uint32_t (&d)[32], uint64_t da, uint64_t db, uint32_t scale_d) {
-  asm volatile(
-      "{\n\t.reg .pred p;\n\t"
-      "setp.ne.b32 p, %26, 0;\n\t"
-      "wgmma.mma_async.sync.aligned.m64n48k32.s32.u8.s8 "
-      "{%0, %1, %2, %3, %4, %5, %6, %7, %8, %9, %10, %11, %12, %13, %14, %15, %16, %17, %18, %19, %20, %21, %22, %23}, %24, %25, p;\n\t}\n"
-      : "+r"(d[0]), "+r"(d[1]), "+r"(d[2]), "+r"(d[3]), "+r"(d[4]), "+r"(d[5]), "+r"(d[6]), "+r"(d[7]), "+r"(d[8]), "+r"(d[9]), "+r"(d[10]), "+r"(d[11]), "+r"(d[12]), "+r"(d[13]), "+r"(d[14]), "+r"(d[15]), "+r"(d[16]), "+r"(d[17]), "+r"(d[18]), "+r"(d[19]), "+r"(d[20]), "+r"(d[21]), "+r"(d[22]), "+r"(d[23])
-      : "l"(da), "l"(db), "r"(scale_d));
-}
-__device__ __forceinline__ void wgmma_bf16_n48(float (&d)[32], uint64_t da, uint64_t db, uint32_t scale_d) {
-  asm volatile(
-      "{\n\t.reg .pred p;\n\t"
-      "setp.ne.b32 p, %26, 0;\n\t"
-      "wgmma.mma_async.sync.aligned.m64n48k16.f32.bf16.bf16 "
-      "{%0, %1, %2, %3, %4, %5, %6, %7, %8, %9, %10, %11, %12, %13, %14, %15, %16, %17, %18, %19, %20, %21, %22, %23}, %24, %25, p, 1, 1, 0, 0;\n\t}\n"
-      : "+f"(d[0]), "+f"(d[1]), "+f"(d[2]), "+f"(d[3]), "+f"(d[4]), "+f"(d[5]), "+f"(d[6]), "+f"(d[7]), "+f"(d[8]), "+f"(d[9]), "+f"(d[10]), "+f"(d[11]), "+f"(d[12]), "+f"(d[13]), "+f"(d[14]), "+f"(d[15]), "+f"(d[16]), "+f"(d[17]), "+f"(d[18]), "+f"(d[19]), "+f"(d[20]), "+f"(d[21]), "+f"(d[22]), "+f"(d[23])
-      : "l"(da), "l"(db), "r"(scale_d));
-}
-__device__ __forceinline__ void wgmma_s8s8_n64(uint32_t (&d)[32], uint64_t da, uint64_t db, uint32_t scale_d) {
-  asm volatile(
-      "{\n\t.reg .pred p;\n\t"
-      "setp.ne.b32 p, %34, 0;\n\t"
-      "wgmma.mma_async.sync.aligned.m64n64k32.s32.s8.s8 "
-      "{%0, %1, %2, %3, %4, %5, %6, %7, %8, %9, %10, %11, %12, %13, %14, %15, %16, %17, %18, %19, %20, %21, %22, %23, %24, %25, %26, %27, %28, %29, %30, %31}, %32, %33, p;\n\t}\n"
-      : "+r"(d[0]), "+r"(d[1]), "+r"(d[2]), "+r"(d[3]), "+r"(d[4]), "+r"(d[5]), "+r"(d[6]), "+r"(d[7]), "+r"(d[8]), "+r"(d[9]), "+r"(d[10]), "+r"(d[11]), "+r"(d[12]), "+r"(d[13]), "+r"(d[14]), "+r"(d[15]), "+r"(d[16]), "+r"(d[17]), "+r"(d[18]), "+r"(d[19]), "+r"(d[20]), "+r"(d[21]), "+r"(d[22]), "+r"(d[23]), "+r"(d[24]), "+r"(d[25]), "+r"(d[26]), "+r"(d[27]), "+r"(d[28]), "+r"(d[29]), "+r"(d[30]), "+r"(d[31])
-      : "l"(da), "l"(db), "r"(scale_d));
-}
-__device__ __forceinline__ void wgmma_u8s8_n64(uint32_t (&d)[32], uint64_t da, uint64_t db, uint32_t scale_d) {
-  asm volatile(
-      "{\n\t.reg .pred p;\n\t"
-      "setp.ne.b32 p, %34, 0;\n\t"
-      "wgmma.mma_async.sync.aligned.m64n64k32.s32.u8.s8 "
-      "{%0, %1, %2, %3, %4, %5, %6, %7, %8, %9, %10, %11, %12, %13, %14, %15, %16, %17, %18, %19, %20, %21, %22, %23, %24, %25, %26, %27, %28, %29, %30, %31}, %32, %33, p;\n\t}\n"
-      : "+r"(d[0]), "+r"(d[1]), "+r"(d[2]), "+r"(d[3]), "+r"(d[4]), "+r"(d[5]), "+r"(d[6]), "+r"(d[7]), "+r"(d[8]), "+r"(d[9]), "+r"(d[10]), "+r"(d[11]), "+r"(d[12]), "+r"(d[13]), "+r"(d[14]), "+r"(d[15]), "+r"(d[16]), "+r"(d[17]), "+r"(d[18]), "+r"(d[19]), "+r"(d[20]), "+r"(d[21]), "+r"(d[22]), "+r"(d[23]), "+r"(d[24]), "+r"(d[25]), "+r"(d[26]), "+r"(d[27]), "+r"(d[28]), "+r"(d[29]), "+r"(d[30]), "+r"(d[31])
-      : "l"(da), "l"(db), "r"(scale_d));
-}
-__device__ __forceinline__ void wgmma_bf16_n64(float (&d)[32], uint64_t da, uint64_t db, uint32_t scale_d) {
-  asm volatile(
-      "{\n\t.reg .pred p;\n\t"
-      "setp.ne.b32 p, %34, 0;\n\t"
-      "wgmma.mma_async.sync.aligned.m64n64k16.f32.bf16.bf16 "
-      "{%0, %1, %2, %3, %4, %5, %6, %7, %8, %9, %10, %11, %12, %13, %14, %15, %16, %17, %18, %19, %20, %21, %22, %23, %24, %25, %26, %27, %28, %29, %30, %31}, %32, %33, p, 1, 1, 0, 0;\n\t}\n"
-      : "+f"(d[0]), "+f"(d[1]), "+f"(d[2]), "+f"(d[3]), "+f"(d[4]), "+f"(d[5]), "+f"(d[6]), "+f"(d[7]), "+f"(d[8]), "+f"(d[9]), "+f"(d[10]), "+f"(d[11]), "+f"(d[12]), "+f"(d[13]), "+f"(d[14]), "+f"(d[15]), "+f"(d[16]), "+f"(d[17]), "+f"(d[18]), "+f"(d[19]), "+f"(d[20]), "+f"(d[21]), "+f"(d[22]), "+f"(d[23]), "+f"(d[24]), "+f"(d[25]), "+f"(d[26]), "+f"(d[27]), "+f"(d[28]), "+f"(d[29]), "+f"(d[30]), "+f"(d[31])
-      : "l"(da), "l"(db), "r"(scale_d));
-}
-
-}
+#define QD_WG_R0 "%3, %4, %5, %6, %7, %8, %9, %10"
+#define QD_WG_R1 ", %11, %12, %13, %14, %15, %16, %17, %18"
+#define QD_WG_R2 ", %19, %20, %21, %22, %23, %24, %25, %26"
+#define QD_WG_R3 ", %27, %28, %29, %30, %31, %32, %33, %34"
+#define QD_WG_R4 ", %35, %36, %37, %38, %39, %40, %41, %42"
+#define QD_WG_R5 ", %43, %44, %45, %46, %47, %48, %49, %50"
+#define QD_WG_R6 ", %51, %52, %53, %54, %55, %56, %57, %58"
+#define QD_WG_R7 ", %59, %60, %61, %62, %63, %64, %65, %66"
+#define QD_WG_R8 ", %67, %68, %69, %70, %71, %72, %73, %74"
+#define QD_WG_R9 ", %75, %76, %77, %78, %79, %80, %81, %82"
+#define QD_WG_R10 ", %83, %84, %85, %86, %87, %88, %89, %90"
+#define QD_WG_R11 ", %91, %92, %93, %94, %95, %96, %97, %98"
+#define QD_WG_R12 ", %99, %100, %101, %102, %103, %104, %105, %106"
+#define QD_WG_R13 ", %107, %108, %109, %110, %111, %112, %113, %114"
+#define QD_WG_R14 ", %115, %116, %117, %118, %119, %120, %121, %122"
+#define QD_WG_R15 ", %123, %124, %125, %126, %127, %128, %129, %130"
+#define QD_WG_D0(C) "+" C(d[0]), "+" C(d[1]), "+" C(d[2]), "+" C(d[3]), "+" C(d[4]), "+" C(d[5]), "+" C(d[6]), "+" C(d[7])
+#define QD_WG_D1(C) "+" C(d[8]), "+" C(d[9]), "+" C(d[10]), "+" C(d[11]), "+" C(d[12]), "+" C(d[13]), "+" C(d[14]), "+" C(d[15])
+#define QD_WG_D2(C) "+" C(d[16]), "+" C(d[17]), "+" C(d[18]), "+" C(d[19]), "+" C(d[20]), "+" C(d[21]), "+" C(d[22]), "+" C(d[23])
+#define QD_WG_D3(C) "+" C(d[24]), "+" C(d[25]), "+" C(d[26]), "+" C(d[27]), "+" C(d[28]), "+" C(d[29]), "+" C(d[30]), "+" C(d[31])
+#define QD_WG_D4(C) "+" C(d[32]), "+" C(d[33]), "+" C(d[34]), "+" C(d[35]), "+" C(d[36]), "+" C(d[37]), "+" C(d[38]), "+" C(d[39])
+#define QD_WG_D5(C) "+" C(d[40]), "+" C(d[41]), "+" C(d[42]), "+" C(d[43]), "+" C(d[44]), "+" C(d[45]), "+" C(d[46]), "+" C(d[47])
+#define QD_WG_D6(C) "+" C(d[48]), "+" C(d[49]), "+" C(d[50]), "+" C(d[51]), "+" C(d[52]), "+" C(d[53]), "+" C(d[54]), "+" C(d[55])
+#define QD_WG_D7(C) "+" C(d[56]), "+" C(d[57]), "+" C(d[58]), "+" C(d[59]), "+" C(d[60]), "+" C(d[61]), "+" C(d[62]), "+" C(d[63])
+#define QD_WG_D8(C) "+" C(d[64]), "+" C(d[65]), "+" C(d[66]), "+" C(d[67]), "+" C(d[68]), "+" C(d[69]), "+" C(d[70]), "+" C(d[71])
+#define QD_WG_D9(C) "+" C(d[72]), "+" C(d[73]), "+" C(d[74]), "+" C(d[75]), "+" C(d[76]), "+" C(d[77]), "+" C(d[78]), "+" C(d[79])
+#define QD_WG_D10(C) "+" C(d[80]), "+" C(d[81]), "+" C(d[82]), "+" C(d[83]), "+" C(d[84]), "+" C(d[85]), "+" C(d[86]), "+" C(d[87])
+#define QD_WG_D11(C) "+" C(d[88]), "+" C(d[89]), "+" C(d[90]), "+" C(d[91]), "+" C(d[92]), "+" C(d[93]), "+" C(d[94]), "+" C(d[95])
+#define QD_WG_D12(C) "+" C(d[96]), "+" C(d[97]), "+" C(d[98]), "+" C(d[99]), "+" C(d[100]), "+" C(d[101]), "+" C(d[102]), "+" C(d[103])
+#define QD_WG_D13(C) "+" C(d[104]), "+" C(d[105]), "+" C(d[106]), "+" C(d[107]), "+" C(d[108]), "+" C(d[109]), "+" C(d[110]), "+" C(d[111])
+#define QD_WG_D14(C) "+" C(d[112]), "+" C(d[113]), "+" C(d[114]), "+" C(d[115]), "+" C(d[116]), "+" C(d[117]), "+" C(d[118]), "+" C(d[119])
+#define QD_WG_D15(C) "+" C(d[120]), "+" C(d[121]), "+" C(d[122]), "+" C(d[123]), "+" C(d[124]), "+" C(d[125]), "+" C(d[126]), "+" C(d[127])
+#define QD_WG_REGS1 QD_WG_R0
+#define QD_WG_OPS1(C) QD_WG_D0(C)
+#define QD_WG_REGS2 QD_WG_REGS1 QD_WG_R1
+#define QD_WG_OPS2(C) QD_WG_OPS1(C), QD_WG_D1(C)
+#define QD_WG_REGS3 QD_WG_REGS2 QD_WG_R2
+#define QD_WG_OPS3(C) QD_WG_OPS2(C), QD_WG_D2(C)
+#define QD_WG_REGS4 QD_WG_REGS3 QD_WG_R3
+#define QD_WG_OPS4(C) QD_WG_OPS3(C), QD_WG_D3(C)
+#define QD_WG_REGS5 QD_WG_REGS4 QD_WG_R4
+#define QD_WG_OPS5(C) QD_WG_OPS4(C), QD_WG_D4(C)
+#define QD_WG_REGS6 QD_WG_REGS5 QD_WG_R5
+#define QD_WG_OPS6(C) QD_WG_OPS5(C), QD_WG_D5(C)
+#define QD_WG_REGS7 QD_WG_REGS6 QD_WG_R6
+#define QD_WG_OPS7(C) QD_WG_OPS6(C), QD_WG_D6(C)
+#define QD_WG_REGS8 QD_WG_REGS7 QD_WG_R7
+#define QD_WG_OPS8(C) QD_WG_OPS7(C), QD_WG_D7(C)
+#define QD_WG_REGS9 QD_WG_REGS8 QD_WG_R8
+#define QD_WG_OPS9(C) QD_WG_OPS8(C), QD_WG_D8(C)
+#define QD_WG_REGS10 QD_WG_REGS9 QD_WG_R9
+#define QD_WG_OPS10(C) QD_WG_OPS9(C), QD_WG_D9(C)
+#define QD_WG_REGS11 QD_WG_REGS10 QD_WG_R10
+#define QD_WG_OPS11(C) QD_WG_OPS10(C), QD_WG_D10(C)
+#define QD_WG_REGS12 QD_WG_REGS11 QD_WG_R11
+#define QD_WG_OPS12(C) QD_WG_OPS11(C), QD_WG_D11(C)
+#define QD_WG_REGS13 QD_WG_REGS12 QD_WG_R12
+#define QD_WG_OPS13(C) QD_WG_OPS12(C), QD_WG_D12(C)
+#define QD_WG_REGS14 QD_WG_REGS13 QD_WG_R13
+#define QD_WG_OPS14(C) QD_WG_OPS13(C), QD_WG_D13(C)
+#define QD_WG_REGS15 QD_WG_REGS14 QD_WG_R14
+#define QD_WG_OPS15(C) QD_WG_OPS14(C), QD_WG_D14(C)
+#define QD_WG_REGS16 QD_WG_REGS15 QD_WG_R15
+#define QD_WG_OPS16(C) QD_WG_OPS15(C), QD_WG_D15(C)
+
+template <int N>
+struct Wgmma;
+#define QD_WGMMA_N(NN, G)                                                                                                 \
+  template <>                                                                                                             \
+  struct Wgmma<NN> {                                                                                                      \
+    template <int R>                                                                                                      \
+    __device__ static __forceinline__ void s8s8(uint32_t (&d)[R], uint64_t da, uint64_t db, uint32_t sd) {                \
+      asm volatile("{\n\t.reg .pred p;\n\tsetp.ne.b32 p, %2, 0;\n\t"                                                  \
+                   "wgmma.mma_async.sync.aligned.m64n" #NN "k32.s32.s8.s8 {" QD_WG_REGS##G "}, %0, %1, p;\n\t}\n"         \
+                   : "+l"(da), "+l"(db), "+r"(sd), QD_WG_OPS##G("r"));                                                     \
+    }                                                                                                                     \
+    template <int R>                                                                                                      \
+    __device__ static __forceinline__ void u8s8(uint32_t (&d)[R], uint64_t da, uint64_t db, uint32_t sd) {                \
+      asm volatile("{\n\t.reg .pred p;\n\tsetp.ne.b32 p, %2, 0;\n\t"                                                  \
+                   "wgmma.mma_async.sync.aligned.m64n" #NN "k32.s32.u8.s8 {" QD_WG_REGS##G "}, %0, %1, p;\n\t}\n"         \
+                   : "+l"(da), "+l"(db), "+r"(sd), QD_WG_OPS##G("r"));                                                     \
+    }                                                                                                                     \
+    template <int R>                                                                                                      \
+    __device__ static __forceinline__ void bf16(float (&d)[R], uint64_t da, uint64_t db, uint32_t sd) {                   \
+      asm volatile("{\n\t.reg .pred p;\n\tsetp.ne.b32 p, %2, 0;\n\t"                                                  \
+                   "wgmma.mma_async.sync.aligned.m64n" #NN "k16.f32.bf16.bf16 {" QD_WG_REGS##G "}, %0, %1, p, 1, 1, 0, 0;\n\t}\n" \
+                   : "+l"(da), "+l"(db), "+r"(sd), QD_WG_OPS##G("f"));                                                     \
+    }                                                                                                                     \
+  };
+QD_WGMMA_N(16, 1)
+QD_WGMMA_N(32, 2)
+QD_WGMMA_N(48, 3)
+QD_WGMMA_N(64, 4)
+QD_WGMMA_N(80, 5)
+QD_WGMMA_N(96, 6)
+QD_WGMMA_N(112, 7)
+QD_WGMMA_N(128, 8)
+QD_WGMMA_N(144, 9)
+QD_WGMMA_N(160, 10)
+QD_WGMMA_N(176, 11)
+QD_WGMMA_N(192, 12)
+QD_WGMMA_N(208, 13)
+QD_WGMMA_N(224, 14)
+QD_WGMMA_N(240, 15)
+QD_WGMMA_N(256, 16)
+#undef QD_WGMMA_N
+
+template <int N, int R>
+__device__ __forceinline__ void wgmma_s8s8_n(uint32_t (&d)[R], uint64_t da, uint64_t db, uint32_t scale_d) {
+  static_assert(N / 2 <= R, "accumulator array narrower than the instruction");
+  Wgmma<N>::s8s8(d, da, db, scale_d);
+}
+template <int N, int R>
+__device__ __forceinline__ void wgmma_u8s8_n(uint32_t (&d)[R], uint64_t da, uint64_t db, uint32_t scale_d) {
+  static_assert(N / 2 <= R, "accumulator array narrower than the instruction");
+  Wgmma<N>::u8s8(d, da, db, scale_d);
+}
+template <int N, int R>
+__device__ __forceinline__ void wgmma_bf16_n(float (&d)[R], uint64_t da, uint64_t db, uint32_t scale_d) {
+  static_assert(N / 2 <= R, "accumulator array narrower than the instruction");
+  Wgmma<N>::bf16(d, da, db, scale_d);
+}
+
+template <int R>
+__device__ __forceinline__ void setmaxnreg_dec() { asm volatile("setmaxnreg.dec.sync.aligned.u32 %0;" ::"n"(R)); }
+template <int R>
+__device__ __forceinline__ void setmaxnreg_inc() { asm volatile("setmaxnreg.inc.sync.aligned.u32 %0;" ::"n"(R)); }
+
+}
```
